# CarluerJB/3D_SIFT_CUDA

Measured on AMD Instinct MI355X. Metric: keypoints/s (.key records per second; Gauss-pyramid GB/s vs HBM roofline in `pyramid`/`roofline`), higher is better.
Workload: dtype f32; 1 GPU; 512^3 float32 blob-field volume per GPU, full featExtract path (pyramid + DoG + extrema + keypoints + SIFT-rank descriptor), all octaves; records_per_volume=185421, octaves=8, extrema=43900, keypoints=36792, parallelism=single GPU, tuning=defaults, descriptor_parity=SIFT-rank: pinned against the reference (see DESIGN.md section 2)

## Files before the change

### 3d_sift_cuda_amd/__init__.py

```python
import ctypes as C
import os
import subprocess

import numpy as np

_HERE = os.path.dirname(os.path.abspath(__file__))
CSRC = os.path.join(_HERE, "csrc")
LIB_HIP = os.path.join(CSRC, "_build", "libsift3d_hip.so")
LIB_HOST = os.path.join(CSRC, "_build", "libsift3d_host.so")
FEATEXTRACT = os.path.join(CSRC, "_build", "featExtract")
FEATRESAMPLE = os.path.join(CSRC, "_build", "featResample")
FEATCOMPOSE = os.path.join(CSRC, "_build", "featCompose")
FEATFUSE = os.path.join(CSRC, "_build", "featFuse")
FEATOVERLAP = os.path.join(CSRC, "_build", "featOverlap")

DESC_SIFT, DESC_BRIEF, DESC_RRIEF, DESC_NRRIEF = 0, 1, 2, 3
ABI_VERSION = 6
INFO_MIN0MAX1, INFO_REORIENT = 0x10, 0x20
STAGES = ("blur_x", "blur_y", "blur_z_dog", "subsample", "extrema", "keypoint", "descriptor", "blur_fused", "octave_tiny")

TUNE_BLUR_FUSED, TUNE_FUSED_CHUNKS, TUNE_FUSED_ROWS, TUNE_LAZY_LEVELS, TUNE_TINY_OCTAVE, TUNE_SAMPLER_CAP, TUNE_KP_CHUNKS, TUNE_BANDS_FIRST, TUNE_HOST_RECORDS, TUNE_FUSED_TILE, TUNE_FUSED_SUB, TUNE_SPLIT_TAIL, TUNE_DESC_SEGMENT, TUNE_FUSED_ORDER, TUNE_FUSED_STAGGER = range(15)

EXTREMUM_DTYPE = np.dtype([("x", "<i4"), ("y", "<i4"), ("z", "<i4"), ("value", "<f4")])
FEATURE_DTYPE = np.dtype([("x", "<f4"), ("y", "<f4"), ("z", "<f4"), ("scale", "<f4"), ("ori", "<f4", (9,)),
                          ("eigs", "<f4", (3,)), ("info", "<u4"), ("desc", "<f4", (64,))])
CANDIDATE_DTYPE = np.dtype([("octave", "<i4"), ("level", "<i4"), ("is_max", "<i4"), ("x", "<i4"), ("y", "<i4"),
                            ("z", "<i4"), ("value", "<f4"), ("h_value", "<f4"), ("l_value", "<f4")])


class Sift3DError(RuntimeError):
    pass


class _Timings(C.Structure):
    _fields_ = [("ms", C.c_double * len(STAGES)), ("launches", C.c_int64 * len(STAGES)), ("alg_bytes", C.c_double * len(STAGES)),
                ("n_octaves", C.c_int64), ("n_extrema", C.c_int64), ("n_keypoints", C.c_int64),
                ("n_records", C.c_int64), ("total_ms", C.c_double)]


class LevelDesc(C.Structure):
    _fields_ = [("img", C.c_void_p), ("dogc", C.c_void_p), ("nx", C.c_int64), ("ny", C.c_int64), ("nz_local", C.c_int64),
                ("nz_global", C.c_int64), ("z_offset", C.c_int64), ("sigma_h", C.c_float), ("sigma_c", C.c_float),
                ("sigma_l", C.c_float), ("octave_factor", C.c_float)]


LAUNCH_DTYPE = np.dtype([("stage", "<i4"), ("ntaps", "<i4"), ("nvox", "<i8"), ("alg_bytes", "<f8"), ("ms", "<f8"),
                         ("start_ms", "<f8")])


def build(verbose=False):
    r = subprocess.run(["make", "-C", CSRC, "-j4"], capture_output=True, text=True)
    if verbose or r.returncode != 0:
        print(r.stdout[-4000:])
        print(r.stderr[-4000:])
    if r.returncode != 0:
        raise Sift3DError("building 3d_sift_cuda_amd/csrc failed")


_hip = None
_host = None


def _sig(fn, res, *args):
    fn.restype = res
    fn.argtypes = list(args)


def hip_lib():
    global _hip
    if _hip is not None:
        return _hip
    if not os.path.exists(LIB_HIP):
        raise Sift3DError("%s is missing: run __graft_entry__.build() (there is no CPU fallback)" % LIB_HIP)
    L = C.CDLL(LIB_HIP)
    P, I64, F, I = C.c_void_p, C.c_int64, C.c_float, C.c_int
    _sig(L.sift3d_abi_version, I)
    if L.sift3d_abi_version() != ABI_VERSION:
        raise Sift3DError("%s has ABI version %d, this mirror of include/sift3d.h is version %d: rebuild (__graft_entry__.build())"
                          % (LIB_HIP, L.sift3d_abi_version(), ABI_VERSION))
    _sig(L.sift3d_device_count, I)
    _sig(L.sift3d_create, P, I, I64, I64, I64)
    _sig(L.sift3d_create_slab, P, I, I64, I64, I64)
    _sig(L.sift3d_set_tuning, I, P, I, I)
    _sig(L.sift3d_host_buffer_grows, I64, P)
    _sig(L.sift3d_zslab_set_tuning, I, P, I, I)
    _sig(L.sift3d_destroy, None, P)
    _sig(L.sift3d_last_error, C.c_char_p, P)
    _sig(L.sift3d_set_stream, I, P, P)
    _sig(L.sift3d_sync, I, P)
    _sig(L.sift3d_free, None, P)
    _sig(L.sift3d_gauss_taps, I, F, F, P)
    _sig(L.sift3d_set_libm_variant, I, I)
    _sig(L.sift3d_get_libm_variant, I)
    _sig(L.sift3d_gauss_blur, I, P, P, P, I64, I64, I64, F, F)
    _sig(L.sift3d_gauss_blur_dev, I, P, P, P, I64, I64, I64, F, F)
    _sig(L.sift3d_gauss_blur_dog_dev, I, P, P, P, P, I64, I64, I64, F, F)
    _sig(L.sift3d_gauss_blur_dog_half_dev, I, P, P, P, P, P, I64, I64, I64, F, F, C.POINTER(C.c_int))
    _sig(L.sift3d_blur_window_supported, I, I64, I64, F, F)
    _sig(L.sift3d_gauss_blur_dog_window_dev, I, P, P, P, P, I64, I64, I64, I64, I64, F, F)
    _sig(L.sift3d_dog, I, P, P, P, P, I64)
    _sig(L.sift3d_dog_dev, I, P, P, P, P, I64)
    _sig(L.sift3d_subsample2, I, P, P, I64, I64, I64, P)
    _sig(L.sift3d_subsample2_dev, I, P, P, I64, I64, I64, P)
    _sig(L.sift3d_extrema, I, P, P, P, P, I64, I64, I64, P, I64, P, P, I64, P)
    _sig(L.sift3d_double_size, I, P, P, I64, I64, I64, P)
    _sig(L.sift3d_halve_size, I, P, P, I64, I64, I64, P)
    _sig(L.sift3d_selftest_lds_add, I, P, P, P, I64, P, P)
    _sig(L.sift3d_set_volume, I, P, P, I64, I64, I64)
    _sig(L.sift3d_set_volume_dev, I, P, P, I64, I64, I64)
    _sig(L.sift3d_set_volume_resized, I, P, P, I64, I64, I64, I)
    _sig(L.sift3d_reserve, I, P, I64)
    _sig(L.sift3d_set_volume_begin, I, P, I64, I64, I64, I)
    _sig(L.sift3d_set_volume_planes, I, P, P, I64, I64)
    _sig(L.sift3d_set_volume_end, I, P)
    _sig(L.sift3d_detect, I, P, F, P, P)
    _sig(L.sift3d_extract, I, P, F, I, F, F, P, P)
    _sig(L.sift3d_extract_view, I, P, F, I, F, F, P, P)
    _sig(L.sift3d_enable_timing, I, P, I)
    _sig(L.sift3d_get_timings, I, P, P)
    _sig(L.sift3d_get_launch_log, I, P, P, I64, P)
    _sig(L.sift3d_candidates_reset, I, P)
    _sig(L.sift3d_extrema_append_dev, I, P, P, P, P, I64, I64, I64, I, I64, I64)
    _sig(L.sift3d_lazy_levels_supported, I, I64, I64, I64, F)
    _sig(L.sift3d_extrema_append_lazy_dev, I, P, P, P, P, P, P, P, F, I64, I64, I64, I, I64, I64)
    _sig(L.sift3d_candidates_dev, I, P, P, I, P, P)
    _sig(L.sift3d_describe_dev, I, P, P, I, I, F, F, P, P, P)
    _sig(L.sift3d_describe_dev_counts, I, P, P, I, I, F, F, P, P)
    _sig(L.sift3d_describe_dev_place, I, P, P, P, P, P, P)
    _sig(L.sift3d_host_register, I, P, I64)
    _sig(L.sift3d_host_unregister, I, P)
    _sig(L.sift3d_set_max_octaves, I, P, I)
    _sig(L.sift3d_extract_zslab, I, P, I, P, I64, I64, I64, F, I, F, F, P, P, P, C.c_char_p, I64)
    _sig(L.sift3d_extract_zslab_over, I, I, P, I, P, I64, I64, I64, F, I, F, F, P, P, P, C.c_char_p, I64)
    _sig(L.sift3d_zslab_set_transport_library, None, C.c_char_p)
    _sig(L.sift3d_zslab_create, P, P, I, I64, I64, I64, C.c_char_p, I64)
    _sig(L.sift3d_zslab_extract, I, P, P, F, I, F, F, P, P, P, C.c_char_p, I64)
    _sig(L.sift3d_zslab_destroy, None, P)
    _sig(L.sift3d_zslab_set_volume, I, P, P, C.c_char_p, I64)
    _sig(L.sift3d_zslab_extract_resident, I, P, F, I, F, F, P, P, P, C.c_char_p, I64)
    _sig(L.sift3d_knn64, I, I, P, I64, P, I64, I, P, P, I, P, C.c_char_p, I64)
    _sig(L.sift3d_match_ratio, I, I, P, I64, P, I64, P, P, P, P, P, C.c_char_p, I64)
    _sig(L.sift3d_hough_similarity, I, I, P, P, P, P, P, P, C.c_int32, P, P, P, P, P, C.c_char_p, I64)
    _sig(L.sift3d_match_keys, I, I, P, I64, P, I64, C.c_int32, P, C.c_char_p, I64)
    _sig(L.sift3d_get_level_slice, I, P, I, I, I64, P, P, P)
    _sig(L.sift3d_get_dog_slice, I, P, I, I, I64, P, P, P)
    _sig(L.sift3d_resample_affine, I, I, P, I64, I64, I64, P, I64, I64, I64, P, I, F, P, C.c_char_p, I64)
    _sig(L.sift3d_resample_affine_dev, I, P, P, I64, I64, I64, P, I64, I64, I64, P, I, F)
    _sig(L.sift3d_guided_search_params, I, I, P, I64, P, I64, P, F, P, P, P, P, P, P, P, C.c_char_p, I64)
    _sig(L.sift3d_refine_similarity, I, I, P, I64, P, I64, P, P, P, P, C.c_char_p, I64)
    _sig(L.sift3d_fit_field, I, I, P, P, I64, P, P, P, C.c_char_p, I64)
    _sig(L.sift3d_refine_field, I, I, P, I64, P, I64, P, P, P, P, C.c_char_p, I64)
    _sig(L.sift3d_resample_field, I, I, P, I64, I64, I64, P, I64, I64, I64, P, P, P, P, I, F, P, C.c_char_p, I64)
    _sig(L.sift3d_block_match, I, I, P, P, I64, I64, I64, P, I64, P, I, I, I, P, P, C.c_char_p, I64)
    _sig(L.sift3d_refine_field_intensity, I, I, P, I64, I64, I64, P, I64, I64, I64, P, P, P, P, P, P, P, C.c_char_p, I64)
    _sig(L.sift3d_block_match_ncc, I, I, P, P, I64, I64, I64, P, I64, P, I, I, I, P, P, C.c_char_p, I64)
    _sig(L.sift3d_refine_field_intensity_metric, I, I, P, I64, I64, I64, P, I64, I64, I64, P, P, P, P, P, I, P, P, P, C.c_char_p, I64)
    _sig(L.sift3d_invert_nodes, I, I, P, P, P, P, P, P, P, P, P, C.c_char_p, I64)
    _sig(L.sift3d_invert_field, I, I, P, P, P, P, P, P, C.c_char_p, I64)
    _sig(L.sift3d_jacobian_map, I, I, I64, I64, I64, P, P, P, P, P, I, P, C.c_char_p, I64)
    _sig(L.sift3d_compose_nodes, I, I, P, P, P, P, P, P, P, P, P, P, P, C.c_char_p, I64)
    _sig(L.sift3d_compose_field, I, I, P, P, P, P, P, P, P, P, C.c_char_p, I64)
    _sig(L.sift3d_fuse_weights, I, I, P, P, I64, I64, I64, C.c_int32, C.c_int32, P, C.c_int32, P, P, C.c_char_p, I64)
    _sig(L.sift3d_fuse_vote, I, I, C.c_int32, P, P, I64, C.c_int32, P, P, C.c_char_p, I64)
    _sig(L.sift3d_fuse_labels, I, I, P, I64, I64, I64, P, C.c_int32, P, P, P, P, C.c_char_p, I64)
    _sig(L.sift3d_fuse_search, I, I, P, P, P, I64, I64, I64, C.c_int32, C.c_int32, C.c_int32, P, C.c_int32, P, P, P, P, C.c_char_p, I64)
    _sig(L.sift3d_fuse_labels_search, I, I, P, I64, I64, I64, P, C.c_int32, P, P, C.c_int32, P, P, P, C.c_char_p, I64)
    _sig(L.sift3d_distance_map, I, I, P, I64, I64, I64, P, P, P, C.c_char_p, I64)
    _sig(L.sift3d_surface_distances, I, P, P, I64, I64, I64, P, P, P, P, P, C.c_char_p, I64)
    _hip = L
    return L


def host_lib():
    global _host
    if _host is not None:
        return _host
    if not os.path.exists(LIB_HOST):
        raise Sift3DError("%s is missing: run __graft_entry__.build()" % LIB_HOST)
    L = C.CDLL(LIB_HOST)
    P, I64, F, I = C.c_void_p, C.c_int64, C.c_float, C.c_int
    _sig(L.sift3d_synth_blobs, None, P, I64, I64, I64, C.c_uint32)
    _sig(L.sift3d_synth_blobs_slices, None, P, I64, I64, I64, C.c_uint32, I64, I64)
    _sig(L.nifti_min_read, I, C.c_char_p, P)
    _sig(L.nifti_min_free, None, P)
    _sig(L.nifti_min_write_f32, I, C.c_char_p, P, I, I, I, F, F, F)
    _sig(L.nifti_min_write_f32_ex, I, C.c_char_p, P, I, I, I, F, F, F, P, P)
    _sig(L.sift3d_write_key, I, C.c_char_p, P, I64, F, I, P)
    _sig(L.sift3d_write_key_mode, None, I)
    _sig(L.sift3d_write_key_bin, I, C.c_char_p, P, I64, F)
    _sig(L.sift3d_read_key, I, C.c_char_p, P, P)
    _sig(L.sift3d_read_key_mode, None, I)
    _sig(L.sift3d_write_pgm, I, C.c_char_p, P, I, I)
    _sig(L.sift3d_world_transform, None, P, I64, P)
    _sig(L.sift3d_match_filter, I64, P, I64, I, I)
    _sig(L.sift3d_match_descriptors, I, P, I64, P)
    _sig(L.sift3d_match_votes, I, P, P, I, P, I, P, P, I, P, P)
    _sig(L.sift3d_match_write_votes, I, C.c_char_p, C.c_char_p, C.c_char_p, P, P, I, I, I)
    _sig(L.sift3d_log_ratio_interval, I, C.c_double, P, P)
    _sig(L.sift3d_similarity_invert, None, P, P)
    _sig(L.sift3d_write_similarity, I, C.c_char_p, P)
    _sig(L.sift3d_write_alignment_matches, I, C.c_char_p, C.c_char_p, C.c_char_p, P, I64, P, I64, P)
    _sig(L.sift3d_similarity_matrix, None, P, P)
    _sig(L.sift3d_read_similarity, I, C.c_char_p, P)
    _sig(L.sift3d_resample_map, I, P, P, P, P)
    _sig(L.sift3d_key_vox2key, None, P, P, P)
    _sig(L.sift3d_fit_similarity, I, P, P, I64, P)
    _sig(L.sift3d_refine_defaults, None, P)
    _sig(L.sift3d_field_defaults, None, P)
    _sig(L.sift3d_field_size, I, P, I64, P, P)
    _sig(L.sift3d_field_samples, None, P, P, P, I64, P, P)
    _sig(L.sift3d_field_warp_terms, I, P, P, P, P)
    _sig(L.sift3d_field_eval, None, P, P, I64, P)
    _sig(L.sift3d_field_folds, I64, P, P, P)
    _sig(L.sift3d_write_field, I, C.c_char_p, P)
    _sig(L.sift3d_read_field, I, C.c_char_p, P)
    _sig(L.sift3d_blockmatch_defaults, None, P)
    _sig(L.sift3d_blockmatch_range, I, P, I64, P, P)
    _sig(L.sift3d_blockmatch_lattice, I, I64, I64, I64, P, P, P)
    _sig(L.sift3d_blockmatch_grid, I, I64, I64, I64, P, P, P)
    _sig(L.sift3d_blockmatch_samples, I64, P, I64, I64, I64, P, P, P, P, P, P, P)
    _sig(L.sift3d_blockmatch_folds, I64, P, P, P)
    _sig(L.sift3d_invert_defaults, None, P)
    _sig(L.sift3d_invert_grid, I, I64, I64, I64, P, P, P)
    _sig(L.sift3d_affine_invert, I, P, P)
    _sig(L.sift3d_affine_invert_d, I, P, P)
    _sig(L.sift3d_write_matrix, I, C.c_char_p, P)
    _sig(L.sift3d_jacobian_factor, I, P, P, P)
    _sig(L.sift3d_compose_defaults, None, P)
    _sig(L.sift3d_compose_matrix, I, P, P, P)
    _sig(L.sift3d_compose_spacing, F, P, P, P)
    _sig(L.sift3d_compose_grid, I, I64, I64, I64, P, P, P, P, P)
    _sig(L.sift3d_compose_residual, I64, P, P, P, I64, P, P)
    _sig(L.sift3d_fuse_defaults, None, P)
    _sig(L.sift3d_fuse_similarity, C.c_uint32, C.c_int32, I64, I64, I64, I64, I64, I64)
    _sig(L.sift3d_fuse_check_labels, I64, P, I64)
    _sig(L.sift3d_fuse_shift_code, C.c_uint16, C.c_int32, C.c_int32, C.c_int32, C.c_int32)
    _sig(L.sift3d_fuse_shift_of, I, C.c_int32, C.c_uint32, P)
    _sig(L.sift3d_fuse_shift_stats, I64, C.c_int32, P, I64, P, P)
    _sig(L.sift3d_label_overlap, I64, P, P, I64, P, P, P)
    _sig(L.sift3d_surface_defaults, None, P)
    _sig(L.sift3d_spacing_um, I, F, P)
    _sig(L.sift3d_surface_stats, None, P, I64, P, I64, P)
    L.free_ptr = C.CDLL(None).free
    L.free_ptr.argtypes = [C.c_void_p]
    _host = L
    return L


class ZSlabStats(C.Structure):
    _fields_ = [("n_ranks", C.c_int32), ("sharded_octaves", C.c_int32), ("exchanges", C.c_int64), ("halo_bytes_critical", C.c_int64),
                ("halo_bytes_deferred", C.c_int64), ("gather_bytes", C.c_int64), ("n_extrema", C.c_int64), ("n_keypoints", C.c_int64),
                ("n_records", C.c_int64), ("wall_ms", C.c_double), ("halo_bytes_hidden", C.c_int64), ("transport", C.c_int32),
                ("transport_fell_back", C.c_int32), ("rccl_version", C.c_int32), ("comm_sets", C.c_int32), ("resident_volume", C.c_int32),
                ("list_grown", C.c_int32), ("merge_ms", C.c_double), ("halo_bytes_subsample", C.c_int64), ("enqueue_ms", C.c_double)]


ZSLAB_TRANSPORT, TRANSPORT_PEER_COPY, TRANSPORT_RCCL = 1000, 0, 1
ZSLAB_SERIAL_CHANNELS, ZSLAB_DUPLICATE_RANKS, ZSLAB_POISON_HALO, ZSLAB_PATCH_WAIT, ZSLAB_LIST_ROOM = 1001, 1002, 1003, 1004, 1005


def zslab_set_transport_library(path):
    hip_lib().sift3d_zslab_set_transport_library(None if path is None else os.fsencode(path))


# ... 1195 lines not shown

def write_key(path, feats, eig_thres=140.0, comments=()):
    feats = np.ascontiguousarray(feats, FEATURE_DTYPE)
    arr = (C.c_char_p * max(1, len(comments)))(*[c.encode() for c in comments])
    rc = host_lib().sift3d_write_key(os.fsencode(path), feats.ctypes.data, len(feats), float(eig_thres), len(comments),
                                     C.cast(arr, C.c_void_p))
    if rc != 0:
        raise Sift3DError("could not write %s" % path)


def write_key_bin(path, feats, eig_thres=140.0):
    feats = np.ascontiguousarray(feats, FEATURE_DTYPE)
    if host_lib().sift3d_write_key_bin(os.fsencode(path), feats.ctypes.data, len(feats), float(eig_thres)) != 0:
        raise Sift3DError("could not write %s" % path)


def world_transform(feats, m44):
    out = np.ascontiguousarray(feats, FEATURE_DTYPE).copy()
    m = np.ascontiguousarray(m44, np.float32).reshape(4, 4)
    host_lib().sift3d_world_transform(out.ctypes.data, len(out), m.ctypes.data)
    return out


def write_pgm(path, slice_yx):
    a = _f32(slice_yx)
    if a.ndim != 2 or host_lib().sift3d_write_pgm(os.fsencode(path), a.ctypes.data, a.shape[0], a.shape[1]) != 0:
        raise Sift3DError("could not write %s" % path)


def read_key(path):
    L = host_lib()
    ptr, n = C.c_void_p(), C.c_int64(0)
    rc = L.sift3d_read_key(os.fsencode(path), C.byref(ptr), C.byref(n))
    if rc != 0:
        raise Sift3DError("could not read %s (%d)" % (path, rc))
    out = np.ctypeslib.as_array(C.cast(ptr, C.POINTER(C.c_uint8)), shape=(n.value * FEATURE_DTYPE.itemsize,)).view(FEATURE_DTYPE).copy()
    L.free_ptr(ptr)
    return out


def _f32(a):
    return np.ascontiguousarray(a, dtype=np.float32)


class Context:

    def __init__(self, nx, ny, nz, device=0, slab=False):
        self._L = hip_lib()
        if self._L.sift3d_device_count() <= 0:
            raise Sift3DError("no HIP device visible and there is no CPU fallback")
        make = self._L.sift3d_create_slab if slab else self._L.sift3d_create
        self._h = make(int(device), int(nx), int(ny), int(nz))
        if not self._h:
            raise Sift3DError("sift3d_create%s(device=%d, %d x %d x %d) failed" % ("_slab" if slab else "", device, nx, ny, nz))
        self.device = device
        self._shape = None

    def set_tuning(self, knob, value):
        self._chk(self._L.sift3d_set_tuning(self._h, int(knob), int(value)), "sift3d_set_tuning")

    def host_buffer_grows(self):
        return int(self._L.sift3d_host_buffer_grows(self._h))

    def close(self):
        if getattr(self, "_h", None):
            self._L.sift3d_destroy(self._h)
            self._h = None

    def __enter__(self):
        return self

    def __exit__(self, *a):
        self.close()

    def __del__(self):
        try:
            self.close()
        except Exception:
            pass

    @property
    def handle(self):
        return self._h

    def _chk(self, rc, what):
        if rc != 0:
            raise Sift3DError("%s -> %d: %s" % (what, rc, self._L.sift3d_last_error(self._h).decode()))

    def gauss_blur(self, vol, sigma, min_value=0.01):
        vol = _f32(vol)
        nz, ny, nx = vol.shape
        out = np.empty_like(vol)
        self._chk(self._L.sift3d_gauss_blur(self._h, vol.ctypes.data, out.ctypes.data, nx, ny, nz, float(sigma),
                                            float(min_value)), "sift3d_gauss_blur")
        return out

    def dog(self, a, b):
        a, b = _f32(a), _f32(b)
        out = np.empty_like(a)
        self._chk(self._L.sift3d_dog(self._h, a.ctypes.data, b.ctypes.data, out.ctypes.data, a.size), "sift3d_dog")
        return out

    def subsample2(self, vol):
        vol = _f32(vol)
        nz, ny, nx = vol.shape
        out = np.empty((nz // 2, ny // 2, nx // 2), np.float32)
        self._chk(self._L.sift3d_subsample2(self._h, vol.ctypes.data, nx, ny, nz, out.ctypes.data), "sift3d_subsample2")
        return out

    def double_size(self, vol):
        vol = _f32(vol)
        nz, ny, nx = vol.shape
        out = np.empty((2 * nz, 2 * ny, 2 * nx), np.float32)
        self._chk(self._L.sift3d_double_size(self._h, vol.ctypes.data, nx, ny, nz, out.ctypes.data), "sift3d_double_size")
        return out

    def halve_size(self, vol):
        vol = _f32(vol)
        nz, ny, nx = vol.shape
        out = np.empty((nz // 2, ny // 2, nx // 2), np.float32)
        self._chk(self._L.sift3d_halve_size(self._h, vol.ctypes.data, nx, ny, nz, out.ctypes.data), "sift3d_halve_size")
        return out

    def selftest_lds_add(self, a, b):
        a, b = _f32(a).ravel(), _f32(b).ravel()
        valu, lds = np.empty_like(a), np.empty_like(a)
        self._chk(self._L.sift3d_selftest_lds_add(self._h, a.ctypes.data, b.ctypes.data, a.size, valu.ctypes.data,
                                                  lds.ctypes.data), "sift3d_selftest_lds_add")
        return valu, lds

    def extrema(self, d_prev, d_cur, d_next=None, capacity=None):
        d_prev, d_cur = _f32(d_prev), _f32(d_cur)
        nz, ny, nx = d_cur.shape
        d_next = None if d_next is None else _f32(d_next)
        cap = int(capacity) if capacity is not None else d_cur.size // 8 + 1024
        mins = np.zeros(cap, EXTREMUM_DTYPE)
        maxs = np.zeros(cap, EXTREMUM_DTYPE)
        nmin, nmax = C.c_int64(0), C.c_int64(0)
        rc = self._L.sift3d_extrema(self._h, d_prev.ctypes.data, d_cur.ctypes.data,
                                    None if d_next is None else d_next.ctypes.data, nx, ny, nz, mins.ctypes.data, cap,
                                    C.byref(nmin), maxs.ctypes.data, cap, C.byref(nmax))
        self._chk(rc, "sift3d_extrema")
        return mins[:nmin.value].copy(), maxs[:nmax.value].copy()

    def set_volume(self, vol, resize=0):
        vol = _f32(vol)
        nz, ny, nx = vol.shape
        self._chk(self._L.sift3d_set_volume_resized(self._h, vol.ctypes.data, nx, ny, nz, int(resize)), "sift3d_set_volume_resized")
        self._shape = self._resized((nz, ny, nx), resize)

    def reserve(self, n_extrema):
        self._chk(self._L.sift3d_reserve(self._h, int(n_extrema)), "sift3d_reserve")

    def set_volume_in_runs(self, vol, runs, resize=0):
        vol = _f32(vol)
        nz, ny, nx = vol.shape
        self._chk(self._L.sift3d_set_volume_begin(self._h, nx, ny, nz, int(resize)), "sift3d_set_volume_begin")
        for z0, n in runs:
            part = vol[z0:z0 + n]
            self._chk(self._L.sift3d_set_volume_planes(self._h, part.ctypes.data, int(z0), int(n)), "sift3d_set_volume_planes")
        self._chk(self._L.sift3d_set_volume_end(self._h), "sift3d_set_volume_end")
        self._shape = self._resized((nz, ny, nx), resize)

    def set_volume_dev(self, dev_ptr, nx, ny, nz):
        self._chk(self._L.sift3d_set_volume_dev(self._h, C.c_void_p(int(dev_ptr)), nx, ny, nz), "sift3d_set_volume_dev")
        self._shape = (int(nz), int(ny), int(nx))

    @staticmethod
    def _resized(shape, resize):
        return tuple(2 * d if resize > 0 else d // 2 if resize < 0 else d for d in shape)

    def _slice(self, entry, octave, level, z, shape_yx):
        out = np.empty(shape_yx, np.float32)
        nx, ny = C.c_int64(0), C.c_int64(0)
        self._chk(getattr(self._L, entry)(self._h, int(octave), int(level), int(z), out.ctypes.data, C.byref(nx), C.byref(ny)), entry)
        assert (ny.value, nx.value) == tuple(shape_yx), (entry, octave, (ny.value, nx.value), shape_yx)
        return out

    def level_slice(self, octave, level, z, shape_yx):
        return self._slice("sift3d_get_level_slice", octave, level, z, shape_yx)

    def dog_slice(self, octave, level, z, shape_yx):
        return self._slice("sift3d_get_dog_slice", octave, level, z, shape_yx)

    def pyramid(self):
        out = []
        shape = self._shape
        for o in range(int(self.timings()["n_octaves"])):
            assert min(shape) > 2, (o, shape)
            lv = {"L": [], "D": []}
            for j in range(5):
                lv["L"].append(np.stack([self.level_slice(o, j, z, shape[1:]) for z in range(shape[0])]))
                try:
                    lv["D"].append(np.stack([self.dog_slice(o, j, z, shape[1:]) for z in range(shape[0])]))
                except Sift3DError as e:
                    if "not stored" not in str(e):
                        raise
                    lv["D"].append(None)
            out.append(lv)
            shape = tuple(d // 2 for d in shape)
        return out

    def detect(self, initial_image_scale=1.0):
        out, n = C.c_void_p(), C.c_int64(0)
        self._chk(self._L.sift3d_detect(self._h, float(initial_image_scale), C.byref(out), C.byref(n)), "sift3d_detect")
        try:
            buf = (C.c_char * (n.value * CANDIDATE_DTYPE.itemsize)).from_address(out.value) if n.value else b""
            return np.frombuffer(buf, CANDIDATE_DTYPE, n.value).copy()
        finally:
            self._L.sift3d_free(out)

    def extract(self, initial_image_scale=1.0, desc_mode=DESC_SIFT, eig_thres=140.0, size_factor=1.0, copy=True):
        out, n = C.c_void_p(), C.c_int64(0)
        self._chk(self._L.sift3d_extract_view(self._h, float(initial_image_scale), int(desc_mode), float(eig_thres),
                                              float(size_factor), C.byref(out), C.byref(n)), "sift3d_extract_view")
        if n.value == 0:
            return np.zeros(0, FEATURE_DTYPE)
        buf = (C.c_char * (n.value * FEATURE_DTYPE.itemsize)).from_address(out.value)
        a = np.frombuffer(buf, FEATURE_DTYPE, n.value)
        return a.copy() if copy else a

    def gauss_blur_dog_dev(self, d_in, d_out, d_dog, nx, ny, nz, sigma, min_value=0.01):
        self._chk(self._L.sift3d_gauss_blur_dog_dev(self._h, C.c_void_p(int(d_in)), C.c_void_p(int(d_out)) if d_out else None,
                                                    C.c_void_p(int(d_dog)) if d_dog else None, nx, ny, nz, float(sigma),
                                                    float(min_value)), "sift3d_gauss_blur_dog_dev")

    def gauss_blur_dog_half_dev(self, d_in, d_out, d_dog, d_half, nx, ny, nz, sigma, min_value=0.01):
        one = C.c_int(0)
        self._chk(self._L.sift3d_gauss_blur_dog_half_dev(self._h, C.c_void_p(int(d_in)), C.c_void_p(int(d_out)),
                                                         C.c_void_p(int(d_dog)) if d_dog else None, C.c_void_p(int(d_half)), nx, ny, nz,
                                                         float(sigma), float(min_value), C.byref(one)), "sift3d_gauss_blur_dog_half_dev")
        return bool(one.value)

    def gauss_blur_dev(self, d_in, d_out, nx, ny, nz, sigma, min_value=0.01):
        self._chk(self._L.sift3d_gauss_blur_dev(self._h, C.c_void_p(int(d_in)), C.c_void_p(int(d_out)), nx, ny, nz,
                                                float(sigma), float(min_value)), "sift3d_gauss_blur_dev")

    def blur_window_supported(self, nx, ny, sigma, min_value=0.01):
        return bool(self._L.sift3d_blur_window_supported(nx, ny, float(sigma), float(min_value)))

    def gauss_blur_dog_window_dev(self, d_in, d_out, d_dog, nx, ny, nz, z_lo, z_hi, sigma, min_value=0.01):
        self._chk(self._L.sift3d_gauss_blur_dog_window_dev(self._h, C.c_void_p(int(d_in)), C.c_void_p(int(d_out)) if d_out else None,
                                                           C.c_void_p(int(d_dog)) if d_dog else None, nx, ny, nz, int(z_lo), int(z_hi),
                                                           float(sigma), float(min_value)), "sift3d_gauss_blur_dog_window_dev")

    def dog_dev(self, d_a, d_b, d_out, n):
        self._chk(self._L.sift3d_dog_dev(self._h, C.c_void_p(int(d_a)), C.c_void_p(int(d_b)), C.c_void_p(int(d_out)), n),
                  "sift3d_dog_dev")

    def resample_affine_dev(self, d_src, src_shape, d_dst, out_shape, map, interp="linear", fill=0.0):
        nz, ny, nx = (int(d) for d in src_shape)
        oz, oy, ox = (int(d) for d in out_shape)
        m = _map12(map)
        self._chk(self._L.sift3d_resample_affine_dev(self._h, C.c_void_p(int(d_src)), nx, ny, nz, C.c_void_p(int(d_dst)), ox, oy, oz,
                                                     m.ctypes.data, INTERP[interp], float(fill)), "sift3d_resample_affine_dev")

    def subsample2_dev(self, d_in, nx, ny, nz, d_out):
        self._chk(self._L.sift3d_subsample2_dev(self._h, C.c_void_p(int(d_in)), nx, ny, nz, C.c_void_p(int(d_out))),
                  "sift3d_subsample2_dev")

    def candidates_reset(self):
        self._chk(self._L.sift3d_candidates_reset(self._h), "sift3d_candidates_reset")

    def extrema_append_dev(self, d_prev, d_cur, d_next, nx, ny, nz_local, level_id, z_lo, z_hi):
        self._chk(self._L.sift3d_extrema_append_dev(self._h, C.c_void_p(int(d_prev)), C.c_void_p(int(d_cur)),
                                                    C.c_void_p(int(d_next)), nx, ny, nz_local, int(level_id), int(z_lo),
                                                    int(z_hi)), "sift3d_extrema_append_dev")

    def lazy_levels_supported(self, nx, ny, nz_local, next_sigma):
        return bool(self._L.sift3d_lazy_levels_supported(nx, ny, nz_local, float(next_sigma)))

    def extrema_append_lazy_dev(self, d_prev, g_prev_a, g_prev_b, d_cur, d_next, g_next, next_sigma, nx, ny, nz_local, level_id,
                                z_lo, z_hi):
        vp = lambda v: C.c_void_p(int(v)) if v else None
        self._chk(self._L.sift3d_extrema_append_lazy_dev(self._h, vp(d_prev), vp(g_prev_a), vp(g_prev_b), vp(d_cur), vp(d_next),
                                                         vp(g_next), float(next_sigma), nx, ny, nz_local, int(level_id), int(z_lo),
                                                         int(z_hi)), "sift3d_extrema_append_lazy_dev")

    @staticmethod
    def _level_array(levels):
        arr = (LevelDesc * len(levels))()
        for i, lv in enumerate(levels):
            arr[i] = LevelDesc(int(lv["img"]), int(lv["dogc"]), lv["nx"], lv["ny"], lv["nz_local"], lv["nz_global"],
                               lv["z_offset"], lv["sigma_h"], lv["sigma_c"], lv["sigma_l"], lv["octave_factor"])
        return arr

    def candidates_dev(self, levels):
        arr = self._level_array(levels)
        out, n = C.c_void_p(), C.c_int64(0)
        self._chk(self._L.sift3d_candidates_dev(self._h, arr, len(levels), C.byref(out), C.byref(n)), "sift3d_candidates_dev")
        try:
            buf = (C.c_char * (n.value * CANDIDATE_DTYPE.itemsize)).from_address(out.value) if n.value else b""
            return np.frombuffer(buf, CANDIDATE_DTYPE, n.value).copy()
        finally:
            self._L.sift3d_free(out)

    def describe_dev(self, levels, desc_mode=DESC_SIFT, eig_thres=140.0, size_factor=1.0, copy=True):
        arr = self._level_array(levels)
        view, grp, n = C.c_void_p(), C.c_void_p(), C.c_int64(0)
        self._chk(self._L.sift3d_describe_dev(self._h, arr, len(levels), int(desc_mode), float(eig_thres), float(size_factor),
                                              C.byref(view), C.byref(grp), C.byref(n)), "sift3d_describe_dev")
        if n.value == 0:
            return np.zeros(0, FEATURE_DTYPE), np.zeros(0, np.int32)
        rb = (C.c_char * (n.value * FEATURE_DTYPE.itemsize)).from_address(view.value)
        gb = (C.c_char * (n.value * 4)).from_address(grp.value)
        recs, grp = np.frombuffer(rb, FEATURE_DTYPE, n.value), np.frombuffer(gb, np.int32, n.value)
# ... 51 lines not shown
```

### 3d_sift_cuda_amd/csrc/api_context.hip

```cpp
#include <algorithm>
#include <chrono>
#include <cmath>
#include <cstdarg>
#include <cstdio>
#include <cstdlib>
#include <cstring>
#include <vector>

#include "sift3d_internal.h"

#include "pipeline.h"

int set_err(sift3d_ctx *c, int code, const char *fmt, ...)
{
    if (c) {
        va_list ap;
        va_start(ap, fmt);
        vsnprintf(c->err, sizeof(c->err), fmt, ap);
        va_end(ap);
    }
    return code;
}

extern "C" int sift3d_abi_version(void) { return SIFT3D_ABI_VERSION; }

extern "C" int sift3d_device_count(void)
{
    int n = 0;
    if (hipGetDeviceCount(&n) != hipSuccess) return 0;
    return n;
}

extern "C" void sift3d_free(void *p) { free(p); }

extern "C" const char *sift3d_last_error(const sift3d_ctx *ctx) { return ctx ? ctx->err : "no context"; }

static void free_dev(sift3d_ctx *c)
{
    hipFree(c->vol);
    for (int i = 0; i < 6; i++) hipFree(c->L[i]);
    for (int i = 0; i < 5; i++) hipFree(c->D[i]);
    hipFree(c->D4tiny);
    hipFree(c->T[0]);
    hipFree(c->T[1]);
    hipFree(c->d_taps);
    hipFree(c->keys_a);
    hipFree(c->keys_b);
    hipFree(c->vals_a);
    hipFree(c->vals_b);
    hipFree(c->d_count);
    hipFree(c->surv);
    hipFree(c->surv2);
    hipFree(c->list2[0]);
    hipFree(c->list2[1]);
    hipFree(c->list2_counts);
    hipFree(c->surv_counts);
    hipFree(c->sort_tmp);
    hipFree(c->scan_tmp);
    hipFree(c->d_levels);
    hipFree(c->kps);
    hipFree(c->patch0);
    hipFree(c->sampler_tokens);
    hipFree(c->d_rec_base);
    hipFree(c->nrec);
    hipFree(c->offs);
    hipFree(c->rec_kp);
    hipFree(c->rec_frame);
    if (c->h_recs) hipHostFree(c->h_recs);
    if (c->h_group) hipHostFree(c->h_group);
    hipFree(c->place.d_counts);
    hipFree(c->place.d_shift);
    if (c->place.h_counts) hipHostFree(c->place.h_counts);
}


std::vector<octave_dims> octave_list(int64_t X, int64_t Y, int64_t Z)
{
    std::vector<octave_dims> v;
    int64_t off = 0;
    while (X > 2 && Y > 2 && Z > 2 && v.size() < 32) {
        const int64_t XP = pitch_of(X);
        v.push_back({X, Y, Z, off, XP});
        off += ((XP * Y * Z + 63) / 64) * 64;
        X /= 2; Y /= 2; Z /= 2;
    }
    return v;
}

int alloc_cands(sift3d_ctx *c, int64_t cap)
{
    unsigned long long *ka = nullptr, *kb = nullptr;
    sift3d_cval *va = nullptr, *vb = nullptr;
    void *tmp = nullptr;
    const size_t tmp_bytes = sift3d_sort_temp_bytes(cap) + 256;
    const bool ok = hipMalloc((void **)&ka, sizeof(unsigned long long) * (size_t)cap) == hipSuccess &&
                    hipMalloc((void **)&kb, sizeof(unsigned long long) * (size_t)cap) == hipSuccess &&
                    hipMalloc((void **)&va, sizeof(sift3d_cval) * (size_t)cap) == hipSuccess &&
                    hipMalloc((void **)&vb, sizeof(sift3d_cval) * (size_t)cap) == hipSuccess && hipMalloc(&tmp, tmp_bytes) == hipSuccess;
    if (!ok) {
        (void)hipGetLastError();
        hipFree(ka); hipFree(kb); hipFree(va); hipFree(vb); hipFree(tmp);
        return SIFT3D_ERR_MEMORY;
    }
    hipFree(c->keys_a); hipFree(c->keys_b); hipFree(c->vals_a); hipFree(c->vals_b); hipFree(c->sort_tmp);
    c->keys_a = ka; c->keys_b = kb;
    c->vals_a = va; c->vals_b = vb;
    c->sort_tmp = tmp;
    c->sort_tmp_bytes = tmp_bytes;
    c->cand_cap = cap;
    return SIFT3D_OK;
}

static void destroy_sync_objects(sift3d_ctx *c)
{
    hipStream_t streams[] = {c->ex_stream, c->ex_stream2, c->kp_stream};
    for (hipStream_t st : streams)
        if (st) {
            hipStreamSynchronize(st);
            hipStreamDestroy(st);
        }
    hipEvent_t events[] = {c->ev_ex2[0], c->ev_ex2[1], c->ev_reset, c->ev_desc, c->ev_oct[0], c->ev_oct[1], c->ev_fence[0], c->ev_fence[1],
                           c->ev_split[0], c->ev_split[1], c->ev_split[2]};
    for (hipEvent_t e : events)
        if (e) hipEventDestroy(e);
    for (hipEvent_t e : c->ev_kpc)
        if (e) hipEventDestroy(e);
    if (c->h_cnt0) hipHostFree(c->h_cnt0);
    if (c->own_stream && c->stream) hipStreamDestroy(c->stream);
}

sift3d_ctx *ctx_create(int device, int64_t nx, int64_t ny, int64_t nz, bool lean)
{
    if (nx <= 0 || ny <= 0 || nz <= 0) return nullptr;
    int n = sift3d_device_count();
    if (device < 0 || device >= n) return nullptr;
    if (hipSetDevice(device) != hipSuccess) return nullptr;
    sift3d_ctx *c = new sift3d_ctx();
    c->device = device;
    c->own_stream = true;
    c->lean = lean;
    c->capN = pitch_of(nx) * ny * nz;
    c->surv_div = 64;
    c->tune[SIFT3D_TUNE_BLUR_FUSED] = 1;
    c->tune[SIFT3D_TUNE_LAZY_LEVELS] = 1;
    c->tune[SIFT3D_TUNE_TINY_OCTAVE] = 1;
    c->tune[SIFT3D_TUNE_SAMPLER_CAP] = 4;
    c->tune[SIFT3D_TUNE_BANDS_FIRST] = 1;
    c->tune[SIFT3D_TUNE_HOST_RECORDS] = 5;
    c->tune[SIFT3D_TUNE_FUSED_SUB] = 1;
    c->tune[SIFT3D_TUNE_SPLIT_TAIL] = 1;
    c->tune[SIFT3D_TUNE_DESC_SEGMENT] = 32;
    c->capTot = c->capN + c->capN / 7 + 4 * ny * nz + 64 * 34;
    bool ok = hipStreamCreateWithFlags(&c->stream, hipStreamNonBlocking) == hipSuccess;
    hipStream_t *streams[] = {&c->ex_stream, &c->ex_stream2, &c->kp_stream};
    for (hipStream_t *st : streams) ok = ok && hipStreamCreateWithFlags(st, hipStreamNonBlocking) == hipSuccess;
    hipEvent_t *events[] = {&c->ev_ex2[0], &c->ev_ex2[1], &c->ev_reset, &c->ev_desc, &c->ev_oct[0], &c->ev_oct[1], &c->ev_fence[0], &c->ev_fence[1],
                            &c->ev_split[0], &c->ev_split[1], &c->ev_split[2]};
    for (hipEvent_t *e : events) ok = ok && hipEventCreateWithFlags(e, hipEventDisableTiming) == hipSuccess;
    for (hipEvent_t &e : c->ev_kpc) ok = ok && hipEventCreateWithFlags(&e, hipEventDisableTiming) == hipSuccess;
    ok = ok && hipHostMalloc((void **)&c->h_cnt0, sizeof(unsigned long long) * (16 + SIFT3D_KP_MAX_CHUNKS), hipHostMallocDefault) == hipSuccess;
    const size_t vb = sizeof(float) * (size_t)c->capN;
    const size_t tb = sizeof(float) * (size_t)c->capTot;
    if (!lean) {
        ok = ok && hipMalloc((void **)&c->vol, vb) == hipSuccess && hipMemsetAsync(c->vol, 0, vb, c->stream) == hipSuccess;
        for (int i = 0; i < 5 && ok; i++) ok = hipMalloc((void **)&c->L[i], tb) == hipSuccess && hipMemsetAsync(c->L[i], 0, tb, c->stream) == hipSuccess;
        for (int i = 0; i < 4 && ok; i++) ok = hipMalloc((void **)&c->D[i], tb) == hipSuccess && hipMemsetAsync(c->D[i], 0, tb, c->stream) == hipSuccess;
        ok = ok && hipMalloc((void **)&c->D4tiny, sizeof(float) * SIFT3D_D4TINY_FLOATS) == hipSuccess &&
             hipMemsetAsync(c->D4tiny, 0, sizeof(float) * SIFT3D_D4TINY_FLOATS, c->stream) == hipSuccess;
    }
    if (c->capN <= SIFT3D_EAGER_T_FLOATS)
        for (int i = 0; i < 2 && ok; i++) {
            ok = hipMalloc((void **)&c->T[i], vb) == hipSuccess;
            if (ok) c->capT = c->capN;
        }
    ok = ok && hipMalloc((void **)&c->d_taps, sizeof(float) * SIFT3D_MAX_TAPS) == hipSuccess;
    ok = ok && hipMalloc((void **)&c->d_count, sizeof(unsigned long long) * 8) == hipSuccess;
    ok = ok && hipMalloc((void **)&c->d_levels, sizeof(sift3d_level) * 96) == hipSuccess;
    ok = ok && hipMalloc((void **)&c->sampler_tokens, sizeof(int) * SIFT3D_CU_SLOTS) == hipSuccess &&
         hipMemsetAsync(c->sampler_tokens, 0, sizeof(int) * SIFT3D_CU_SLOTS, c->stream) == hipSuccess;
    ok = ok && hipMalloc((void **)&c->d_rec_base, sizeof(int) * (SIFT3D_KP_MAX_CHUNKS + 1)) == hipSuccess;
    ok = ok && alloc_cands(c, c->capN / 32 + 8192) == SIFT3D_OK;
    c->surv_cap = c->capN / 8 + 65536;
    ok = ok && hipMalloc((void **)&c->surv, sizeof(sift3d_survivor) * (size_t)c->surv_cap) == hipSuccess;
    ok = ok && hipMalloc((void **)&c->surv_counts, sizeof(unsigned long long) * SIFT3D_SURV_COUNTERS * SIFT3D_SURV_SETS) == hipSuccess;
    ok = ok && hipMalloc((void **)&c->list2_counts, sizeof(unsigned long long) * SIFT3D_LIST2_COUNTERS * SIFT3D_SURV_SETS) == hipSuccess;
    ok = ok && hipStreamSynchronize(c->stream) == hipSuccess;
    if (!ok) {
        free_dev(c);
        destroy_sync_objects(c);
        delete c;
        return nullptr;
    }
    return c;
}

extern "C" sift3d_ctx *sift3d_create(int device, int64_t nx, int64_t ny, int64_t nz) { return ctx_create(device, nx, ny, nz, false); }

extern "C" sift3d_ctx *sift3d_create_slab(int device, int64_t nx, int64_t ny, int64_t nz_local) { return ctx_create(device, nx, ny, nz_local, true); }

extern "C" void sift3d_destroy(sift3d_ctx *c)
{
    if (!c) return;
    hipSetDevice(c->device);
    hipStreamSynchronize(c->stream);
    free_dev(c);
    for (hipEvent_t e : c->pool) hipEventDestroy(e);
    destroy_sync_objects(c);
    delete c;
}

extern "C" int sift3d_set_tuning(sift3d_ctx *c, int knob, int value)
{
    if (!c) return SIFT3D_ERR_ARG;
    static const int lo[SIFT3D_TUNE_COUNT] = {0, 0, 0, 0, 0, 0, 0, 0, 1, 0, 0, 0, 0, 0, 0},
                     hi[SIFT3D_TUNE_COUNT] = {2, 4096, 2, 1, 1, 64, SIFT3D_KP_MAX_CHUNKS, 1, 1 + SIFT3D_MAX_FRAMES, 2, 1, 2, 1 << 20, 3, 2};
    if (knob < 0 || knob >= SIFT3D_TUNE_COUNT || value < lo[knob] || value > hi[knob])
        return set_err(c, SIFT3D_ERR_ARG, "sift3d_set_tuning: knob %d does not take %d", knob, value);
    c->tune[knob] = value;
    return SIFT3D_OK;
}

extern "C" int64_t sift3d_host_buffer_grows(const sift3d_ctx *c) { return c ? c->host_grows : 0; }

#ifdef SIFT3D_DEV
extern "C" int sift3d_dev_set_stop(sift3d_ctx *c, int n)
{
    if (!c) return SIFT3D_ERR_ARG;
    c->dev_stop = n;
    return SIFT3D_OK;
}
#endif

extern "C" int sift3d_set_stream(sift3d_ctx *c, void *s)
{
    if (!c) return SIFT3D_ERR_ARG;
    HIPCHK(c, hipSetDevice(c->device));
    HIPCHK(c, hipStreamSynchronize(c->stream));
    if (s) {
        if (c->own_stream) hipStreamDestroy(c->stream);
        c->stream = (hipStream_t)s;
        c->own_stream = false;
    } else if (!c->own_stream) {
        HIPCHK(c, hipStreamCreateWithFlags(&c->stream, hipStreamNonBlocking));
        c->own_stream = true;
    }
    return SIFT3D_OK;
}

extern "C" int sift3d_set_max_octaves(sift3d_ctx *c, int n)
{
    if (!c || n < 0) return c ? set_err(c, SIFT3D_ERR_ARG, "max_octaves must be >= 0") : SIFT3D_ERR_ARG;
    c->max_octaves = n;
    return SIFT3D_OK;
}

extern "C" int sift3d_sync(sift3d_ctx *c)
{
    if (!c) return SIFT3D_ERR_ARG;
    HIPCHK(c, hipSetDevice(c->device));
    HIPCHK(c, hipStreamSynchronize(c->stream));
    return SIFT3D_OK;
}

__global__ void selftest_lds_add_kernel(const float *__restrict__ a, const float *__restrict__ b, long long n,
                                        float *__restrict__ valu, float *__restrict__ lds)
{
    __shared__ float cell[256];
    const long long i = (long long)blockIdx.x * 256 + threadIdx.x;
    const float x = i < n ? a[i] : 0.0f, y = i < n ? b[i] : 0.0f;
    cell[threadIdx.x] = x;
    __syncthreads();
    __hip_atomic_fetch_add(&cell[threadIdx.x], y, __ATOMIC_RELAXED, __HIP_MEMORY_SCOPE_WORKGROUP);
    __syncthreads();
    if (i < n) {
        valu[i] = x + y;
        lds[i] = cell[threadIdx.x];
    }
}

extern "C" int sift3d_selftest_lds_add(sift3d_ctx *c, const float *a, const float *b, int64_t n, float *valu, float *lds)
{
    NEED_LEVELS(c);
    if (!c || !a || !b || !valu || !lds || n <= 0 || 4 * n > c->capTot) return c ? set_err(c, SIFT3D_ERR_ARG, "bad self-test arguments") : SIFT3D_ERR_ARG;
    HIPCHK(c, hipSetDevice(c->device));
    float *da = c->L[0], *db = c->L[0] + n, *dv = c->L[0] + 2 * n, *dl = c->L[0] + 3 * n;
    HIPCHK(c, hipMemcpyAsync(da, a, sizeof(float) * (size_t)n, hipMemcpyHostToDevice, c->stream));
    HIPCHK(c, hipMemcpyAsync(db, b, sizeof(float) * (size_t)n, hipMemcpyHostToDevice, c->stream));
    hipLaunchKernelGGL(selftest_lds_add_kernel, dim3((unsigned)((n + 255) / 256)), dim3(256), 0, c->stream, da, db, (long long)n, dv, dl);
    HIPCHK(c, hipGetLastError());
    HIPCHK(c, hipMemcpyAsync(valu, dv, sizeof(float) * (size_t)n, hipMemcpyDeviceToHost, c->stream));
    HIPCHK(c, hipMemcpyAsync(lds, dl, sizeof(float) * (size_t)n, hipMemcpyDeviceToHost, c->stream));
    HIPCHK(c, hipStreamSynchronize(c->stream));
    c->has_volume = false;
    c->pad_nx = 0;
    return SIFT3D_OK;
}

int ensure_T(sift3d_ctx *c, int64_t floats)
{
    if (floats <= c->capT) return SIFT3D_OK;
    if (floats > c->capN) return set_err(c, SIFT3D_ERR_ARG, "pass intermediates of %lld floats asked of a context of %lld", (long long)floats, (long long)c->capN);
    HIPCHK(c, hipStreamSynchronize(c->stream));
    hipFree(c->T[0]);
    hipFree(c->T[1]);
    c->T[0] = c->T[1] = nullptr;
    c->capT = 0;
    int64_t want = c->capN / 8 + c->capN / 64 + 4096;
    if (want < floats) want = floats;
    if (want > c->capN) want = c->capN;
    for (int i = 0; i < 2; i++)
        if (hipMalloc((void **)&c->T[i], sizeof(float) * (size_t)want) != hipSuccess) {
            (void)hipGetLastError();
            return set_err(c, SIFT3D_ERR_MEMORY, "out of device memory for the pass intermediates (%lld floats)", (long long)want);
        }
    c->capT = want;
    return SIFT3D_OK;
}
```

### 3d_sift_cuda_amd/csrc/api_ops.hip

```cpp
#include <algorithm>
#include <chrono>
#include <cmath>
#include <cstdarg>
#include <cstdio>
#include <cstdlib>
#include <cstring>
#include <vector>

#include "sift3d_internal.h"

#include "pipeline.h"

static sift3d_blur_tuning blur_tuning(const sift3d_ctx *c)
{
    return {c->tune[SIFT3D_TUNE_FUSED_CHUNKS], c->tune[SIFT3D_TUNE_FUSED_ROWS], c->tune[SIFT3D_TUNE_FUSED_TILE], c->tune[SIFT3D_TUNE_FUSED_ORDER], c->tune[SIFT3D_TUNE_FUSED_STAGGER]};
}

int blur_dev(sift3d_ctx *c, const float *in, float *out, float *dog, int64_t X, int64_t Y, int64_t Z, float sigma,
                    float min_value, float *sub, bool *sub_done)
{
    if (sub_done) *sub_done = false;
    float taps[SIFT3D_MAX_TAPS];
    hipStream_t ws = c->stream;
    int n = sift3d_gauss_taps(sigma, min_value, taps);
// ... 240 lines not shown

extern "C" int sift3d_halve_size(sift3d_ctx *c, const float *in, int64_t nx, int64_t ny, int64_t nz, float *out)
{
    NEED_LEVELS(c);
    int rc = check_shape(c, nx, ny, nz);
    if (rc) return rc;
    if (!in || !out || nx < 2 || ny < 2 || nz < 2) return set_err(c, SIFT3D_ERR_ARG, "halve_size needs every dimension >= 2");
    HIPCHK(c, hipSetDevice(c->device));
    HIPCHK(c, hipMemcpyAsync(c->L[0], in, sizeof(float) * (size_t)(nx * ny * nz), hipMemcpyHostToDevice, c->stream));
    HIPCHK(c, sift3d_launch_halve_size(c->stream, c->L[0], nx, ny, nz, c->L[1]));
    const size_t ob = sizeof(float) * (size_t)((nx / 2) * (ny / 2) * (nz / 2));
    HIPCHK(c, hipMemcpyAsync(out, c->L[1], ob, hipMemcpyDeviceToHost, c->stream));
    HIPCHK(c, hipStreamSynchronize(c->stream));
    c->has_volume = false;
    c->pad_nx = 0;
    return SIFT3D_OK;
}

int cand_reset(sift3d_ctx *c, hipStream_t on)
{
    if (!on) on = c->stream;
    c->jobs.clear();
    c->cand_split_at = 0;
    HIPCHK(c, hipMemsetAsync(c->d_count, 0, sizeof(unsigned long long) * 8, on));
    HIPCHK(c, hipMemsetAsync(c->surv_counts, 0, sizeof(unsigned long long) * SIFT3D_SURV_COUNTERS * SIFT3D_SURV_SETS, on));
    HIPCHK(c, hipMemsetAsync(c->list2_counts, 0, sizeof(unsigned long long) * SIFT3D_LIST2_COUNTERS * SIFT3D_SURV_SETS, on));
    HIPCHK(c, hipMemsetAsync(c->d_rec_base, 0, sizeof(int), on));
    c->surv_set = 0;
    return SIFT3D_OK;
}

int cand_append(sift3d_ctx *c, const level_job &j, const cand_where &w, bool record)
{
    c->count_queued = false;
    if (record) c->jobs.push_back(j);
    hipStream_t st = w.stream ? w.stream : c->stream;
    stage_scope sc(c, SIFT3D_STAGE_EXTREMA, 4.0 * (double)j.X * j.Y * j.Z, 0, j.X * j.Y * j.Z, st);
    int64_t cover = j.X * j.Y * j.Z / c->surv_div + 64 * 1024;
    if (cover > c->surv_cap) cover = c->surv_cap;
    sift3d_survivor *surv = c->surv;
    if (w.list > 0) {
        if (c->surv2_cap < cover) {
            HIPCHK(c, hipStreamSynchronize(st));
            hipFree(c->surv2);
            c->surv2 = nullptr;
            c->surv2_cap = 0;
            HIPCHK(c, hipMalloc((void **)&c->surv2, sizeof(sift3d_survivor) * (size_t)cover));
            c->surv2_cap = cover;
        }
        surv = c->surv2;
    }
    const bool fresh = c->surv_set < SIFT3D_SURV_SETS;
    const int set = fresh ? c->surv_set++ : SIFT3D_SURV_SETS - 1;
    unsigned long long *counters = c->surv_counts + (size_t)set * SIFT3D_SURV_COUNTERS;
    sift3d_extrema_lazy lz;
    memset(&lz, 0, sizeof(lz));
    const bool lazy = j.prev_b || j.next_g;
    if (lazy) {
        lz.prev_b = j.prev_b;
        lz.next_g = j.next_g;
        if (j.next_g) {
            const int li = w.list > 0 ? 1 : 0;
            if (c->list2_cap[li] < cover) {
                HIPCHK(c, hipStreamSynchronize(st));
                hipFree(c->list2[li]);
                c->list2[li] = nullptr;
                c->list2_cap[li] = 0;
                HIPCHK(c, hipMalloc((void **)&c->list2[li], sizeof(sift3d_survivor2) * (size_t)cover));
                c->list2_cap[li] = cover;
            }
            lz.ntaps = j.next_ntaps;
            memcpy(lz.taps, j.next_taps, sizeof(lz.taps));
            lz.list2 = c->list2[li];
            lz.list2_count = c->list2_counts + (size_t)set * SIFT3D_LIST2_COUNTERS;
            lz.list2_cap = c->list2_cap[li];
            if (!fresh) HIPCHK(c, hipMemsetAsync(lz.list2_count, 0, sizeof(unsigned long long) * SIFT3D_LIST2_COUNTERS, st));
        }
    }
    HIPCHK(c, sift3d_launch_extrema(st, {j.dp, j.dc, j.dn, j.X, j.Xl ? j.Xl : j.X, j.Y, j.Z, j.z_lo, j.z_hi, j.lvl_id, cand_target_of(c, w.group),
                                         surv, counters, c->d_count + 2, cover, !fresh, lazy ? &lz : nullptr, c->strict_extrema}));
    return SIFT3D_OK;
}

int cand_append_octave_small(sift3d_ctx *c, const level_job jobs[3], const float *const D[5], int64_t XP, int64_t X, int64_t Y, int64_t Z,
                             const cand_where &w)
{
    hipStream_t st = w.stream ? w.stream : c->stream;
    stage_scope sc(c, SIFT3D_STAGE_EXTREMA, 12.0 * (double)XP * Y * Z, 0, XP * Y * Z, st);
    HIPCHK(c, sift3d_launch_extrema_octave_small(st, D, XP, X, Y, Z, jobs[0].lvl_id, cand_target_of(c, w.group)));
    c->count_queued = false;
    for (int l = 0; l < 3; l++) c->jobs.push_back(jobs[l]);
    return SIFT3D_OK;
}

int cand_replay(sift3d_ctx *c)
{
    c->cand_split_at = 0;
    HIPCHK(c, hipMemsetAsync(c->d_count, 0, sizeof(unsigned long long) * 8, c->stream));
    HIPCHK(c, hipMemsetAsync(c->surv_counts, 0, sizeof(unsigned long long) * SIFT3D_SURV_COUNTERS * SIFT3D_SURV_SETS, c->stream));
    HIPCHK(c, hipMemsetAsync(c->list2_counts, 0, sizeof(unsigned long long) * SIFT3D_LIST2_COUNTERS * SIFT3D_SURV_SETS, c->stream));
    c->surv_set = 0;
    for (const level_job &j : c->jobs) {
        int rc = cand_append(c, j, cand_where(), false);
        if (rc) return rc;
    }
    return SIFT3D_OK;
}

int surv_make_room(sift3d_ctx *c, unsigned long long high_water)
{
    c->surv_div = 1;
    if ((int64_t)high_water > c->surv_cap) {
        hipFree(c->surv);
        c->surv = nullptr;
        c->surv_cap = (int64_t)high_water + (int64_t)high_water / 4 + 4096;
        HIPCHK(c, hipMalloc((void **)&c->surv, sizeof(sift3d_survivor) * (size_t)c->surv_cap));
    }
    return SIFT3D_OK;
}

int cand_count_queue(sift3d_ctx *c)
{
    unsigned long long *cnt = c->h_cnt0 + 4;
    cnt[0] = cnt[1] = cnt[2] = 0;
    HIPCHK(c, hipMemcpyAsync(cnt, c->d_count, sizeof(unsigned long long) * 3, hipMemcpyDeviceToHost, c->stream));
    c->count_queued = true;
    return SIFT3D_OK;
}

int cand_finalize(sift3d_ctx *c, int64_t *count_out)
{
    for (int attempt = 0; attempt < 4; attempt++) {
        const unsigned long long *cnt = c->h_cnt0 + 4;
        if (!c->count_queued) {
            int rc = cand_count_queue(c);
            if (rc) return rc;
        }
        c->count_queued = false;
        HIPCHK(c, hipStreamSynchronize(c->stream));
        if (cnt[2] > 0) {
            int rc = surv_make_room(c, cnt[2]);
            if (rc) return rc;
            rc = cand_replay(c);
            if (rc) return rc;
            continue;
        }
        if ((int64_t)cnt[0] > c->cand_cap) {
            if (alloc_cands(c, (int64_t)cnt[0] + (int64_t)cnt[0] / 4 + 4096) != SIFT3D_OK)
                return set_err(c, SIFT3D_ERR_MEMORY, "candidate buffer could not be grown to %llu entries", cnt[0]);
            int rc = cand_replay(c);
            if (rc) return rc;
            continue;
        }
        if (cnt[0] > 0)
            HIPCHK(c, sift3d_sort_candidates(c->stream, c->sort_tmp, c->sort_tmp_bytes, c->keys_a, c->keys_b, c->vals_a, c->vals_b, (int64_t)cnt[0]));
        *count_out = (int64_t)cnt[0];
        return SIFT3D_OK;
    }
    return set_err(c, SIFT3D_ERR_MEMORY, "extrema buffers could not be grown");
}

extern "C" int sift3d_extrema(sift3d_ctx *c, const float *d_prev, const float *d_cur, const float *d_next, int64_t nx,
                              int64_t ny, int64_t nz, sift3d_extremum *minima, int64_t cap_min, int64_t *n_min,
                              sift3d_extremum *maxima, int64_t cap_max, int64_t *n_max)
{
    NEED_LEVELS(c);
    int rc = check_shape(c, nx, ny, nz);
    if (rc) return rc;
    if (!d_prev || !d_cur || !n_min || !n_max) return set_err(c, SIFT3D_ERR_ARG, "null pointer");
    HIPCHK(c, hipSetDevice(c->device));
    const size_t b = sizeof(float) * (size_t)(nx * ny * nz);
    HIPCHK(c, hipMemcpyAsync(c->D[0], d_prev, b, hipMemcpyHostToDevice, c->stream));
    HIPCHK(c, hipMemcpyAsync(c->D[1], d_cur, b, hipMemcpyHostToDevice, c->stream));
    if (d_next) HIPCHK(c, hipMemcpyAsync(c->D[2], d_next, b, hipMemcpyHostToDevice, c->stream));
    c->has_volume = false;
    c->pad_nx = 0;
    c->strict_extrema = sift3d_volume_needs_strict(d_cur, nx * ny * nz);
    int64_t cnt = 0;
    rc = cand_reset(c);
    if (!rc) rc = cand_append(c, {c->D[0], c->D[1], d_next ? c->D[2] : nullptr, nx, ny, nz, 0, (int)nz, 0}, cand_where(), true);
    if (!rc) rc = cand_finalize(c, &cnt);
    if (rc) return rc;
    std::vector<unsigned long long> keys((size_t)cnt);
    std::vector<sift3d_cval> vals((size_t)cnt);
    if (cnt) {
        HIPCHK(c, hipMemcpyAsync(keys.data(), c->keys_b, sizeof(unsigned long long) * (size_t)cnt, hipMemcpyDeviceToHost, c->stream));
        HIPCHK(c, hipMemcpyAsync(vals.data(), c->vals_b, sizeof(sift3d_cval) * (size_t)cnt, hipMemcpyDeviceToHost, c->stream));
    }
    HIPCHK(c, hipStreamSynchronize(c->stream));
    int64_t a = 0, m = 0;
    bool over = false;
    for (int64_t i = 0; i < cnt; i++) {
        const int64_t idx = (int64_t)(keys[(size_t)i] & SIFT3D_KEY_IDX_MASK);
        sift3d_extremum e;
        e.x = (int32_t)(idx % nx);
        e.y = (int32_t)((idx / nx) % ny);
        e.z = (int32_t)(idx / (nx * ny));
        e.value = vals[(size_t)i].value;
        if ((keys[(size_t)i] >> SIFT3D_KEY_MAX_SHIFT) & 1ull) {
            if (m < cap_max && maxima) maxima[m] = e; else over = true;
            m++;
        } else {
            if (a < cap_min && minima) minima[a] = e; else over = true;
            a++;
        }
    }
    *n_min = a;
    *n_max = m;
    return over ? set_err(c, SIFT3D_ERR_CAPACITY, "extrema lists need %lld + %lld entries", (long long)a, (long long)m)
                : SIFT3D_OK;
}
```

### 3d_sift_cuda_amd/csrc/api_pipeline.hip

```cpp
#include <algorithm>
#include <chrono>
#include <cmath>
#include <cstdarg>
#include <cstdio>
#include <cstdlib>
#include <cstring>
#include <vector>

#include "sift3d_internal.h"

#include "pipeline.h"

static int ensure_level_buffer(sift3d_ctx *c, float **buf)
{
    if (*buf) return SIFT3D_OK;
    if (hipMalloc((void **)buf, sizeof(float) * (size_t)c->capTot) != hipSuccess) {
        *buf = nullptr;
        return set_err(c, SIFT3D_ERR_MEMORY, "a level buffer of %lld floats could not be allocated", (long long)c->capTot);
    }
    HIPCHK(c, hipMemsetAsync(*buf, 0, sizeof(float) * (size_t)c->capTot, c->stream));
    return SIFT3D_OK;
}

static int load_volume_prepare(sift3d_ctx *c, int64_t nx, int64_t ny, int64_t nz)
// ... 57 lines not shown
    return SIFT3D_OK;
}

extern "C" int sift3d_set_volume_dev(sift3d_ctx *c, const float *d_vol, int64_t nx, int64_t ny, int64_t nz)
{
    NEED_LEVELS(c);
    int rc = check_shape(c, nx, ny, nz);
    if (rc) return rc;
    if (!d_vol) return set_err(c, SIFT3D_ERR_ARG, "null volume");
    if (nz <= 1) return set_err(c, SIFT3D_ERR_ARG, "Could not read volume (z <= 1)");
    HIPCHK(c, hipSetDevice(c->device));
    rc = fence_in(c);
    if (rc) return rc;
    rc = load_volume(c, d_vol, false, nx, ny, nz);
    if (rc) return rc;
    rc = scan_volume(c, nx, ny, nz);
    if (rc) return rc;
    c->nx = nx; c->ny = ny; c->nz = nz;
    c->has_volume = true;
    return fence_out(c);
}

extern "C" int sift3d_set_volume_resized(sift3d_ctx *c, const float *vol, int64_t nx, int64_t ny, int64_t nz, int resize)
{
    NEED_LEVELS(c);
    if (resize == 0) return sift3d_set_volume(c, vol, nx, ny, nz);
    if (!c || !vol || nx < 2 || ny < 2 || nz < 2 || nx * ny * nz > c->capN)
        return set_err(c, SIFT3D_ERR_ARG, "set_volume_resized: bad shape or null volume");
    const int64_t ox = resize > 0 ? 2 * nx : nx / 2, oy = resize > 0 ? 2 * ny : ny / 2, oz = resize > 0 ? 2 * nz : nz / 2;
    int rc = check_shape(c, ox, oy, oz);
    if (rc) return rc;
    if (oz <= 1) return set_err(c, SIFT3D_ERR_ARG, "Could not read volume (z <= 1)");
    HIPCHK(c, hipSetDevice(c->device));
    rc = ensure_T(c, ox * oy * oz > nx * ny * nz ? ox * oy * oz : nx * ny * nz);
    if (rc) return rc;
    HIPCHK(c, hipMemcpyAsync(c->T[0], vol, sizeof(float) * (size_t)(nx * ny * nz), hipMemcpyHostToDevice, c->stream));
    if (resize > 0) HIPCHK(c, sift3d_launch_double_size(c->stream, c->T[0], nx, ny, nz, c->T[1]));
    else HIPCHK(c, sift3d_launch_halve_size(c->stream, c->T[0], nx, ny, nz, c->T[1]));
    rc = load_volume(c, c->T[1], false, ox, oy, oz);
    if (rc) return rc;
    rc = scan_volume(c, ox, oy, oz);
    if (rc) return rc;
    c->nx = ox; c->ny = oy; c->nz = oz;
    c->has_volume = true;
    return SIFT3D_OK;
}

extern "C" int sift3d_set_volume_begin(sift3d_ctx *c, int64_t nx, int64_t ny, int64_t nz, int resize)
{
    NEED_LEVELS(c);
    if (!c || nx < 1 || ny < 1 || nz < 1 || nx * ny * nz > c->capN) return set_err(c, SIFT3D_ERR_ARG, "set_volume_begin: bad shape");
    if (resize != 0 && (nx < 2 || ny < 2 || nz < 2)) return set_err(c, SIFT3D_ERR_ARG, "set_volume_begin: bad shape for a resize");
    const int64_t ox = resize > 0 ? 2 * nx : (resize < 0 ? nx / 2 : nx), oy = resize > 0 ? 2 * ny : (resize < 0 ? ny / 2 : ny),
                  oz = resize > 0 ? 2 * nz : (resize < 0 ? nz / 2 : nz);
    int rc = check_shape(c, ox, oy, oz);
    if (rc) return rc;
    if (oz <= 1) return set_err(c, SIFT3D_ERR_ARG, "Could not read volume (z <= 1)");
    HIPCHK(c, hipSetDevice(c->device));
    c->has_volume = false;
    if (resize != 0) {
        rc = ensure_T(c, ox * oy * oz > nx * ny * nz ? ox * oy * oz : nx * ny * nz);
        if (rc) return rc;
    } else {
        rc = load_volume_prepare(c, nx, ny, nz);
        if (rc) return rc;
    }
    c->up.open = true;
    c->up.nx = nx; c->up.ny = ny; c->up.nz = nz;
    c->up.got = 0;
    c->up.resize = resize;
    c->up.seen.assign((size_t)nz, false);
    return SIFT3D_OK;
}

extern "C" int sift3d_set_volume_planes(sift3d_ctx *c, const float *planes, int64_t z0, int64_t n)
{
    if (!c || !c->up.open) return set_err(c, SIFT3D_ERR_ARG, "set_volume_planes without set_volume_begin");
    if (!planes || z0 < 0 || n < 1 || z0 + n > c->up.nz) {
        c->up.open = false;
        return set_err(c, SIFT3D_ERR_ARG, "set_volume_planes: planes [%lld, %lld) of %lld", (long long)z0, (long long)(z0 + n), (long long)c->up.nz);
    }
    for (int64_t z = z0; z < z0 + n; z++)
        if (c->up.seen[(size_t)z]) {
            c->up.open = false;
            return set_err(c, SIFT3D_ERR_ARG, "set_volume_planes: plane %lld arrived twice", (long long)z);
        }
    for (int64_t z = z0; z < z0 + n; z++) c->up.seen[(size_t)z] = true;
    HIPCHK(c, hipSetDevice(c->device));
    const int64_t nx = c->up.nx, ny = c->up.ny, xp = pitch_of(nx);
    if (c->up.resize != 0) {
        HIPCHK(c, hipMemcpyAsync(c->T[0] + z0 * nx * ny, planes, sizeof(float) * (size_t)(n * nx * ny), hipMemcpyHostToDevice, c->stream));
    } else if (xp == nx) {
        HIPCHK(c, hipMemcpyAsync(c->vol + z0 * nx * ny, planes, sizeof(float) * (size_t)(n * nx * ny), hipMemcpyHostToDevice, c->stream));
    } else {
        HIPCHK(c, hipMemcpy2DAsync(c->vol + z0 * xp * ny, sizeof(float) * (size_t)xp, planes, sizeof(float) * (size_t)nx, sizeof(float) * (size_t)nx,
                                   (size_t)(ny * n), hipMemcpyHostToDevice, c->stream));
    }
    c->up.got += n;
    return SIFT3D_OK;
}

extern "C" int sift3d_set_volume_end(sift3d_ctx *c)
{
    if (!c || !c->up.open) return set_err(c, SIFT3D_ERR_ARG, "set_volume_end without set_volume_begin");
    c->up.open = false;
    if (c->up.got != c->up.nz) return set_err(c, SIFT3D_ERR_ARG, "set_volume_end: %lld of %lld planes arrived", (long long)c->up.got, (long long)c->up.nz);
    HIPCHK(c, hipSetDevice(c->device));
    int64_t nx = c->up.nx, ny = c->up.ny, nz = c->up.nz;
    if (c->up.resize != 0) {
        const int64_t ox = c->up.resize > 0 ? 2 * nx : nx / 2, oy = c->up.resize > 0 ? 2 * ny : ny / 2, oz = c->up.resize > 0 ? 2 * nz : nz / 2;
        if (c->up.resize > 0) HIPCHK(c, sift3d_launch_double_size(c->stream, c->T[0], nx, ny, nz, c->T[1]));
        else HIPCHK(c, sift3d_launch_halve_size(c->stream, c->T[0], nx, ny, nz, c->T[1]));
        const int rc = load_volume(c, c->T[1], false, ox, oy, oz);
        if (rc) return rc;
        nx = ox; ny = oy; nz = oz;
    }
    const int rs = scan_volume(c, nx, ny, nz);
    if (rs) return rs;
    c->nx = nx; c->ny = ny; c->nz = nz;
    c->has_volume = true;
    return SIFT3D_OK;
}

static int ensure_host_records(sift3d_ctx *c, int64_t need, int64_t keep)
{
    if (need <= c->hrecs_cap) return SIFT3D_OK;
    sift3d_feature *nr = nullptr;
    int *ng = nullptr;
    const int64_t cap = need + need / 8 + 1024;
    HIPCHK(c, hipHostMalloc((void **)&nr, sizeof(sift3d_feature) * (size_t)cap, hipHostMallocDefault));
    if (hipHostMalloc((void **)&ng, sizeof(int) * (size_t)cap, hipHostMallocDefault) != hipSuccess) {
        hipHostFree(nr);
        return set_err(c, SIFT3D_ERR_MEMORY, "out of pinned host memory for %lld records", (long long)cap);
    }
    if (keep > 0 && c->h_recs) {
        memcpy(nr, c->h_recs, sizeof(sift3d_feature) * (size_t)keep);
        memcpy(ng, c->h_group, sizeof(int) * (size_t)keep);
    }
    if (c->h_recs) hipHostFree(c->h_recs);
    if (c->h_group) hipHostFree(c->h_group);
    c->h_recs = nr;
    c->h_group = ng;
    c->hrecs_cap = cap;
    HIPCHK(c, hipHostGetDevicePointer((void **)&c->d_hrecs, c->h_recs, 0));
    HIPCHK(c, hipHostGetDevicePointer((void **)&c->d_hgroup, c->h_group, 0));
    return SIFT3D_OK;
}

static int ensure_kp_buffers(sift3d_ctx *c, int64_t ncand, int64_t host_for = -1)
{
    if (ncand > c->kps_cap) {
        HIPCHK(c, hipStreamSynchronize(c->stream));
        HIPCHK(c, hipStreamSynchronize(c->kp_stream));
        hipFree(c->kps); hipFree(c->nrec); hipFree(c->offs); hipFree(c->scan_tmp); hipFree(c->patch0);
        hipFree(c->rec_kp); hipFree(c->rec_frame);
        c->kps = nullptr;
        c->patch0 = nullptr;
        c->nrec = c->offs = c->rec_kp = c->rec_frame = nullptr;
        c->scan_tmp = nullptr;
        c->kps_cap = 0;
        const int64_t cap = ncand + ncand / 2 + 1024, rcap = cap * (1 + SIFT3D_MAX_FRAMES);
        c->scan_tmp_bytes = sift3d_scan_temp_bytes(cap) + 256;
        HIPCHK(c, hipMalloc((void **)&c->kps, sizeof(sift3d_dkp) * (size_t)cap));
        HIPCHK(c, hipMalloc((void **)&c->patch0, sizeof(float) * SIFT3D_PATCH_VOX * (size_t)cap));
        HIPCHK(c, hipMalloc((void **)&c->nrec, sizeof(int) * (size_t)cap));
        HIPCHK(c, hipMalloc((void **)&c->offs, sizeof(int) * (size_t)cap));
        HIPCHK(c, hipMalloc(&c->scan_tmp, c->scan_tmp_bytes));
        HIPCHK(c, hipMalloc((void **)&c->rec_kp, sizeof(int) * (size_t)rcap));
        HIPCHK(c, hipMalloc((void **)&c->rec_frame, sizeof(int) * (size_t)rcap));
        c->kps_cap = cap;
        c->recs_cap = rcap;
    }
    int per = c->tune[SIFT3D_TUNE_HOST_RECORDS];
    if (per < 1) per = 1;
    if (per > 1 + SIFT3D_MAX_FRAMES) per = 1 + SIFT3D_MAX_FRAMES;
    if (host_for < 0 || host_for > ncand) host_for = ncand;
    if (c->hrecs_cap < host_for * per) {
        HIPCHK(c, hipStreamSynchronize(c->stream));
        HIPCHK(c, hipStreamSynchronize(c->kp_stream));
        int rc = ensure_host_records(c, host_for * per, 0);
        if (rc) return rc;
    }
    return SIFT3D_OK;
}

extern "C" int sift3d_reserve(sift3d_ctx *c, int64_t n_extrema)
{
    if (!c || n_extrema < 0) return set_err(c, SIFT3D_ERR_ARG, "sift3d_reserve: bad arguments");
    HIPCHK(c, hipSetDevice(c->device));
    if (n_extrema > c->cand_cap && alloc_cands(c, n_extrema + n_extrema / 4 + 4096) != SIFT3D_OK)
        return set_err(c, SIFT3D_ERR_MEMORY, "candidate buffer could not be grown to %lld entries", (long long)n_extrema);
    return ensure_kp_buffers(c, n_extrema, n_extrema);
}

int candidates_to_host(sift3d_ctx *c, const std::vector<sift3d_level> &levels, int64_t ncand,
                              sift3d_candidate **cands_out, int64_t *n_out)
{
    std::vector<unsigned long long> keys((size_t)ncand);
    std::vector<sift3d_cval> vals((size_t)ncand);
    if (ncand) {
        HIPCHK(c, hipMemcpyAsync(keys.data(), c->keys_b, sizeof(unsigned long long) * (size_t)ncand, hipMemcpyDeviceToHost, c->stream));
        HIPCHK(c, hipMemcpyAsync(vals.data(), c->vals_b, sizeof(sift3d_cval) * (size_t)ncand, hipMemcpyDeviceToHost, c->stream));
    }
    timing_end(c);
    HIPCHK(c, hipStreamSynchronize(c->stream));
    sift3d_candidate *out = (sift3d_candidate *)malloc(sizeof(sift3d_candidate) * (size_t)(ncand ? ncand : 1));
    if (!out) return set_err(c, SIFT3D_ERR_MEMORY, "out of host memory");
    for (int64_t i = 0; i < ncand; i++) {
        const unsigned long long k = keys[(size_t)i];
        const int id = (int)(k >> SIFT3D_KEY_LVL_SHIFT);
        const int64_t idx = (int64_t)(k & SIFT3D_KEY_IDX_MASK);
        if (id < 0 || id >= (int)levels.size()) {
            free(out);
            return set_err(c, SIFT3D_ERR_ARG, "candidate with level id %d outside the level table", id);
        }
        const sift3d_level &lv = levels[(size_t)id];
        sift3d_candidate &o = out[i];
        o.octave = id / 3;
        o.level = id % 3 + 1;
        o.is_max = (int)((k >> SIFT3D_KEY_MAX_SHIFT) & 1ull);
        o.x = (int32_t)(idx % lv.XP);
        o.y = (int32_t)((idx / lv.XP) % lv.Y);
        o.z = (int32_t)(idx / ((int64_t)lv.XP * lv.Y)) + lv.z_off;
        o.value = vals[(size_t)i].value;
        o.h_value = vals[(size_t)i].h;
        o.l_value = vals[(size_t)i].l;
    }
    *cands_out = out;
    *n_out = ncand;
    return SIFT3D_OK;
}

static void kp_params_of(sift3d_ctx *c, int desc_mode, float eig_thres, float size_factor, sift3d_kp_params &p)
{
    p.levels = c->d_levels;
    p.eig_thres = eig_thres;
    p.size_factor = size_factor;
    p.desc_mode = desc_mode;
    p.debug_stop = c->dev_stop;
    p.patch0 = c->patch0;
    p.sampler_tokens = c->sampler_tokens;
    p.sampler_cap = c->tune[SIFT3D_TUNE_SAMPLER_CAP];
    p.desc_seg = c->tune[SIFT3D_TUNE_DESC_SEGMENT] * 8;
    p.rec_shift = nullptr;
}

static int kp_chunks_for(const sift3d_ctx *c, int64_t ncand)
{
    int n = c->tune[SIFT3D_TUNE_KP_CHUNKS];
    if (n <= 0) n = SIFT3D_KP_DEFAULT_CHUNKS;
    if (n > SIFT3D_KP_MAX_CHUNKS) n = SIFT3D_KP_MAX_CHUNKS;
    if (n > ncand) n = ncand > 0 ? (int)ncand : 1;
    return n;
}

static int describe_begin(sift3d_ctx *c, size_t nlevels, float *taps3)
{
    if (sift3d_gauss_taps(0.5f, 0.01f, taps3) != 3 || sift3d_gauss_taps((float)0.95, (float)0.01, c->kp.taps5) != 5)
        return set_err(c, SIFT3D_ERR_ARG, "unexpected patch tap counts");
    if (nlevels > 96) return set_err(c, SIFT3D_ERR_ARG, "too many levels");
    c->kp.ncand = 0;
    c->kp.nchunks = 0;
    c->kp.launched = 0;
    c->kp.nrec = 0;
    c->kp.split = false;
    c->place.dst = nullptr;
    return SIFT3D_OK;
}

void describe_want_group_counts(sift3d_ctx *c, bool on) { c->place.counts = on; }

static int ensure_place_buffers(sift3d_ctx *c)
{
    if (c->place.d_counts) return SIFT3D_OK;
    HIPCHK(c, hipMalloc((void **)&c->place.d_counts, sizeof(int) * SIFT3D_GROUPS));
    HIPCHK(c, hipMalloc((void **)&c->place.d_shift, sizeof(int) * SIFT3D_GROUPS));
    HIPCHK(c, hipHostMalloc((void **)&c->place.h_counts, sizeof(int) * SIFT3D_GROUPS, hipHostMallocDefault));
    return SIFT3D_OK;
}

int describe_group_counts(sift3d_ctx *c, const int **counts, int64_t *total)
{
    if (!c->place.counts) return set_err(c, SIFT3D_ERR_ARG, "describe_group_counts: not asked for before describe_queue");
    {
        const int rc = ensure_place_buffers(c);
        if (rc) return rc;
    }
    *total = 0;
    if (c->kp.ncand <= 0 || c->kp.nchunks != 1) {
        memset(c->place.h_counts, 0, sizeof(int) * SIFT3D_GROUPS);
        *counts = c->place.h_counts;
        return c->kp.nchunks > 1 ? set_err(c, SIFT3D_ERR_ARG, "describe_group_counts: the stage runs in chunks") : SIFT3D_OK;
    }
    HIPCHK(c, hipEventSynchronize(c->ev_kpc[0]));
    for (int g = 0; g < SIFT3D_GROUPS; g++) *total += c->place.h_counts[g];
    *counts = c->place.h_counts;
    return SIFT3D_OK;
}

int describe_placement(sift3d_ctx *c, sift3d_feature *shared_list, const int *shift)
{
    if (!shared_list || !shift || !c->place.d_shift) return set_err(c, SIFT3D_ERR_ARG, "describe_placement: bad arguments");
    HIPCHK(c, hipMemcpyAsync(c->place.d_shift, shift, sizeof(int) * SIFT3D_GROUPS, hipMemcpyHostToDevice, c->stream));
    c->place.dst = shared_list;
    return SIFT3D_OK;
}

static int describe_queue_chunk(sift3d_ctx *c, int i, int64_t a, int64_t b, hipStream_t ks, const float *taps3)
{
    int *h_end = reinterpret_cast<int *>(c->h_cnt0 + 8);
    c->kp.first[i] = a;
    c->kp.first[i + 1] = b;
    h_end[i] = 0;
    {
        sift3d_kp_params q = c->kp.p;
        q.patch0 = c->patch0 + (size_t)a * SIFT3D_PATCH_VOX;
        stage_scope sc(c, SIFT3D_STAGE_KEYPOINT, 0.0, 0, b - a, ks);
        HIPCHK(c, sift3d_launch_keypointsA(ks, q, c->keys_b + a, c->vals_b + a, b - a, c->kps + a, c->nrec + a, taps3));
    }
    HIPCHK(c, sift3d_scan_counts(ks, c->scan_tmp, c->scan_tmp_bytes, c->nrec + a, c->offs + a, b - a));
    HIPCHK(c, sift3d_launch_recmap(ks, c->nrec + a, c->offs + a, b - a, (int)a, c->d_rec_base + i, c->rec_kp, c->rec_frame, c->d_count + 3));
    HIPCHK(c, hipMemcpyAsync(&h_end[i], c->d_rec_base + i + 1, sizeof(int), hipMemcpyDeviceToHost, ks));
    if (c->place.counts && i == 0) {
        int rc = ensure_place_buffers(c);
        if (rc) return rc;
        HIPCHK(c, hipMemsetAsync(c->place.d_counts, 0, sizeof(int) * SIFT3D_GROUPS, ks));
        HIPCHK(c, sift3d_launch_group_counts(ks, c->keys_b + a, c->nrec + a, b - a, c->place.d_counts));
        HIPCHK(c, hipMemcpyAsync(c->place.h_counts, c->place.d_counts, sizeof(int) * SIFT3D_GROUPS, hipMemcpyDeviceToHost, ks));
    }
    HIPCHK(c, hipEventRecord(c->ev_kpc[i], ks));
    return SIFT3D_OK;
}

int describe_queue(sift3d_ctx *c, const std::vector<sift3d_level> &levels, int64_t ncand, int desc_mode, float eig_thres,
                          float size_factor, bool levels_on_device)
{
    float taps3[SIFT3D_MAX_TAPS];
    int rc0 = describe_begin(c, levels.size(), taps3);
    if (rc0) return rc0;
    c->kp.ncand = ncand;
    if (ncand <= 0) return SIFT3D_OK;
    int rc = ensure_kp_buffers(c, ncand);
    if (rc) return rc;
    if (!levels_on_device)
        HIPCHK(c, hipMemcpyAsync(c->d_levels, levels.data(), sizeof(sift3d_level) * levels.size(), hipMemcpyHostToDevice, c->stream));
    kp_params_of(c, desc_mode, eig_thres, size_factor, c->kp.p);
    const int nch = kp_chunks_for(c, ncand);
    c->kp.nchunks = nch;
    HIPCHK(c, hipMemsetAsync(c->d_count + 3, 0, sizeof(unsigned long long), c->stream));
    HIPCHK(c, hipMemsetAsync(c->d_rec_base, 0, sizeof(int), c->stream));
    for (int i = 0; i < nch; i++) {
        rc = describe_queue_chunk(c, i, ncand * i / nch, ncand * (i + 1) / nch, c->stream, taps3);
        if (rc) return rc;
    }
    return SIFT3D_OK;
}

int describe_launch(sift3d_ctx *c)
{
    const int nch = c->kp.nchunks;
    if (nch <= 0) return SIFT3D_OK;
    const int *h_end = reinterpret_cast<const int *>(c->h_cnt0 + 8);
    const bool split = c->kp.split && nch > 1;
    const bool beside = split || (!c->kp.split && nch > 1 && !(c->timing == 1 || c->timing == 3));
    int64_t base = 0;
    for (int i = 0; i < nch; i++) {
        hipStream_t ds = (split ? i > 0 : beside) ? c->kp_stream : c->stream;
        HIPCHK(c, hipEventSynchronize(c->ev_kpc[i]));
        const int64_t end = h_end[i], m = end - base;
        if (end < base || end > c->recs_cap) return set_err(c, SIFT3D_ERR_DEVICE, "record map out of range (%lld of %lld)", (long long)end, (long long)c->recs_cap);
        if (end > c->hrecs_cap && !c->place.dst) {
            HIPCHK(c, hipStreamSynchronize(ds));
            if (split) HIPCHK(c, hipStreamSynchronize(c->stream));
            const int64_t done_cand = c->kp.first[i + 1], need = done_cand > 0 && i + 1 < nch ? (int64_t)((double)end * (double)c->kp.ncand / (double)done_cand) + 1 : end;
            int rc = ensure_host_records(c, need > end ? need : end, base);
            if (rc) return rc;
            c->host_grows++;
        }
        if (m > 0) {
            stage_scope sc(c, SIFT3D_STAGE_DESCRIPTOR, 0.0, 0, m, ds);
            if (c->kp.p.sampler_cap > 0 && !(split && i > 0))
                HIPCHK(c, hipMemsetAsync(c->sampler_tokens, 0, sizeof(int) * SIFT3D_CU_SLOTS, ds));
            sift3d_kp_params q = c->kp.p;
            q.rec_shift = c->place.dst ? c->place.d_shift : nullptr;
            if (c->place.dst && end > c->hrecs_cap) {
                HIPCHK(c, hipStreamSynchronize(ds));
                int rc = ensure_host_records(c, end, 0);
                if (rc) return rc;
                c->host_grows++;
            }
            HIPCHK(c, sift3d_launch_descriptors(ds, q, c->kps, c->rec_kp + base, c->rec_frame + base, m,
                                                (c->place.dst ? c->place.dst : c->d_hrecs) + base, c->d_hgroup + base, c->kp.taps5));
        }
        base = end;
    }
    c->kp.nrec = base;
    c->kp.launched = 1;
    if (beside) {
        HIPCHK(c, hipEventRecord(c->ev_desc, c->kp_stream));
        HIPCHK(c, hipStreamWaitEvent(c->stream, c->ev_desc, 0));
    }
    return SIFT3D_OK;
}

int describe_finish(sift3d_ctx *c, int64_t *n_out)
{
    unsigned long long &nkp = c->h_cnt0[6];
    nkp = 0;
    if (c->kp.nrec) HIPCHK(c, hipMemcpyAsync(&nkp, c->d_count + 3, sizeof(nkp), hipMemcpyDeviceToHost, c->stream));
    HIPCHK(c, hipStreamSynchronize(c->stream));
    timing_end(c);
    c->last.n_records = c->kp.nrec;
    c->last.n_keypoints = (int64_t)nkp;
    *n_out = c->kp.nrec;
    return SIFT3D_OK;
}

#ifdef SIFT3D_DEV
extern "C" int sift3d_dev_overlap_probe(sift3d_ctx *c, int kslice, int dslice, double *out_ms)
{
    if (!c || !out_ms || kslice < 1 || dslice < 1 || c->kp.ncand <= 0 || c->kp.nrec <= 0) return SIFT3D_ERR_ARG;
    HIPCHK(c, hipSetDevice(c->device));
    float taps3[SIFT3D_MAX_TAPS];
    sift3d_gauss_taps(0.5f, 0.01f, taps3);
    const int64_t ncand = c->kp.ncand, nrec = c->kp.nrec;
    hipEvent_t ev[6];
    for (hipEvent_t &e : ev) HIPCHK(c, hipEventCreate(&e));
    hipStream_t s1 = c->stream, s2 = c->kp_stream;
    HIPCHK(c, hipStreamSynchronize(s1));
    HIPCHK(c, hipStreamSynchronize(s2));
    auto launch_k = [&](hipStream_t st, int64_t a, int64_t n) -> hipError_t {
        sift3d_kp_params q = c->kp.p;
        q.patch0 = c->patch0 + (size_t)a * SIFT3D_PATCH_VOX;
        return sift3d_launch_keypointsA(st, q, c->keys_b + a, c->vals_b + a, n, c->kps + a, c->nrec + a, taps3);
    };
    auto launch_d = [&](hipStream_t st, int64_t b, int64_t m) -> hipError_t {
        return sift3d_launch_descriptors(st, c->kp.p, c->kps, c->rec_kp + b, c->rec_frame + b, m, c->d_hrecs + b, c->d_hgroup + b, c->kp.taps5);
    };
    HIPCHK(c, hipEventRecord(ev[0], s1));
    HIPCHK(c, launch_k(s1, 0, ncand));
    HIPCHK(c, hipMemsetAsync(c->sampler_tokens, 0, sizeof(int) * SIFT3D_CU_SLOTS, s1));
    HIPCHK(c, launch_d(s1, 0, nrec));
    HIPCHK(c, hipEventRecord(ev[1], s1));
    HIPCHK(c, hipStreamSynchronize(s1));
    HIPCHK(c, hipMemsetAsync(c->sampler_tokens, 0, sizeof(int) * SIFT3D_CU_SLOTS, s1));
    HIPCHK(c, hipEventRecord(ev[2], s1));
    HIPCHK(c, hipStreamWaitEvent(s2, ev[2], 0));
    enum { NS = 4 };
    hipStream_t ks[NS], ds[NS];
    hipEvent_t done[2 * NS];
    for (int i = 0; i < NS; i++) {
        HIPCHK(c, hipStreamCreateWithFlags(&ks[i], hipStreamNonBlocking));
        HIPCHK(c, hipStreamCreateWithFlags(&ds[i], hipStreamNonBlocking));
        HIPCHK(c, hipEventCreateWithFlags(&done[i], hipEventDisableTiming));
        HIPCHK(c, hipEventCreateWithFlags(&done[NS + i], hipEventDisableTiming));
        HIPCHK(c, hipStreamWaitEvent(ks[i], ev[2], 0));
        HIPCHK(c, hipStreamWaitEvent(ds[i], ev[2], 0));
    }
    (void)s2;
    int64_t a = 0, b = 0;
    int ki = 0, di = 0;
    while (a < ncand || b < nrec) {
        if (a < ncand) {
            const int64_t n = ncand - a < kslice ? ncand - a : kslice;
            HIPCHK(c, launch_k(ks[ki++ % NS], a, n));
            a += n;
        }
        const int64_t b_to = ncand > 0 ? (int64_t)((double)nrec * (double)a / (double)ncand) : nrec;
        while (b < nrec && (b < b_to || a >= ncand)) {
            const int64_t m = nrec - b < dslice ? nrec - b : dslice;
            HIPCHK(c, launch_d(ds[di++ % NS], b, m));
            b += m;
        }
    }
    for (int i = 0; i < NS; i++) {
        HIPCHK(c, hipEventRecord(done[i], ks[i]));
        HIPCHK(c, hipEventRecord(done[NS + i], ds[i]));
        HIPCHK(c, hipStreamWaitEvent(s1, done[i], 0));
        HIPCHK(c, hipStreamWaitEvent(s1, done[NS + i], 0));
    }
    HIPCHK(c, hipEventRecord(ev[4], s1));
    HIPCHK(c, hipStreamSynchronize(s1));
    for (int i = 0; i < NS; i++) {
        hipStreamDestroy(ks[i]);
        hipStreamDestroy(ds[i]);
        hipEventDestroy(done[i]);
        hipEventDestroy(done[NS + i]);
    }
    float m0 = 0, m1 = 0;
    HIPCHK(c, hipEventElapsedTime(&m0, ev[0], ev[1]));
    HIPCHK(c, hipEventElapsedTime(&m1, ev[2], ev[4]));
    out_ms[0] = m0;
    out_ms[1] = m1;
    for (hipEvent_t e : ev) hipEventDestroy(e);
    return SIFT3D_OK;
}
#endif

int describe_sorted(sift3d_ctx *c, const std::vector<sift3d_level> &levels, int64_t ncand, int desc_mode,
                           float eig_thres, float size_factor, int64_t *n_out, bool levels_on_device)
{
    int rc = describe_queue(c, levels, ncand, desc_mode, eig_thres, size_factor, levels_on_device);
    if (!rc) rc = describe_launch(c);
    if (!rc) rc = describe_finish(c, n_out);
    return rc;
}

static int finish_split_tail(sift3d_ctx *c, const std::vector<sift3d_level> &levels, bool levels_on_device, int desc_mode, float eig_thres,
                             float size_factor, int64_t *n_out, bool *done)
{
    *done = false;
    unsigned long long *const h_split = c->h_cnt0 + 8 + SIFT3D_KP_MAX_CHUNKS;
    const int64_t capA = c->cand_split_at, capB = c->cand_cap - capA;
    hipStream_t ks = c->kp_stream;
    float taps3[SIFT3D_MAX_TAPS];
    auto fall_back = [&](unsigned long long overflow_mark) -> int {
        HIPCHK(c, hipStreamSynchronize(ks));
        HIPCHK(c, hipStreamSynchronize(c->stream));
        if (overflow_mark > 0) {
            const int rc = surv_make_room(c, overflow_mark);
            if (rc) return rc;
        }
        return cand_replay(c);
    };
    h_split[3] = h_split[5] = h_split[7] = 0;
    HIPCHK(c, hipMemcpyAsync(h_split + 3, c->d_count, sizeof(unsigned long long) * 5, hipMemcpyDeviceToHost, c->stream));
    HIPCHK(c, hipEventSynchronize(c->ev_split[2]));
    const int64_t nA = (int64_t)h_split[0];
    if (h_split[2] > 0 || nA > capA) return fall_back(h_split[2]);
    int rc = describe_begin(c, levels.size(), taps3);
    if (rc) return rc;
    rc = ensure_kp_buffers(c, nA + nA / 8 + 4096, nA);
    if (rc) return rc;
    kp_params_of(c, desc_mode, eig_thres, size_factor, c->kp.p);
    c->kp.split = true;
    if (!levels_on_device)
        HIPCHK(c, hipMemcpyAsync(c->d_levels, levels.data(), sizeof(sift3d_level) * levels.size(), hipMemcpyHostToDevice, ks));
    int nch = 0;
    if (nA > 0) {
        HIPCHK(c, sift3d_sort_candidates(ks, c->sort_tmp, c->sort_tmp_bytes, c->keys_a, c->keys_b, c->vals_a, c->vals_b, nA));
        rc = describe_queue_chunk(c, nch++, 0, nA, ks, taps3);
        if (rc) return rc;
    }
    c->kp.nchunks = nch;
    HIPCHK(c, hipStreamSynchronize(c->stream));
    const int64_t nB = (int64_t)h_split[7];
    if (h_split[5] > 0 || nB > capB || nA + nB > c->kps_cap || (int64_t)h_split[3] != nA) return fall_back(h_split[5]);
    if (nB > 0) {
        HIPCHK(c, sift3d_sort_candidates(ks, c->sort_tmp, c->sort_tmp_bytes, c->keys_a + capA, c->keys_b + nA, c->vals_a + capA, c->vals_b + nA, nB));
        rc = describe_queue_chunk(c, nch++, nA, nA + nB, ks, taps3);
        if (rc) return rc;
    }
    c->kp.nchunks = nch;
    c->kp.ncand = nA + nB;
    c->last.n_extrema = nA + nB;
    rc = describe_launch(c);
    if (!rc) rc = describe_finish(c, n_out);
    if (rc) return rc;
    *done = true;
    return SIFT3D_OK;
}

static int run_pipeline(sift3d_ctx *c, float init_scale, bool extract, int desc_mode, float eig_thres, float size_factor,
                        sift3d_candidate **cands_out, sift3d_feature **feats_out, int64_t *n_out)
{
    if (!c) return SIFT3D_ERR_ARG;
    if (c->lean) return set_err(c, SIFT3D_ERR_ARG, "a slab context holds no pyramid (sift3d_create_slab)");
    if (!c->has_volume) return set_err(c, SIFT3D_ERR_ARG, "no volume set (sift3d_set_volume)");
    HIPCHK(c, hipSetDevice(c->device));
    timing_begin(c);
    c->last_run.clear();
    std::vector<octave_dims> oct = octave_list(c->nx, c->ny, c->nz);
    if (c->max_octaves > 0 && oct.size() > (size_t)c->max_octaves) oct.resize((size_t)c->max_octaves);

    const octave_sigmas s = sigma_schedule(init_scale);
    const int64_t xp0 = pitch_of(c->nx);
    int rc = blur_dev(c, c->vol, c->L[0], nullptr, xp0, c->ny, c->nz, s.extra0, 0.01f);
    if (rc) return rc;
    if (xp0 != c->nx) HIPCHK(c, sift3d_launch_zero_pad(c->stream, c->L[0], nullptr, xp0, c->nx, c->ny * c->nz));
    rc = cand_reset(c, c->ex_stream);
    if (rc) return rc;
    HIPCHK(c, hipEventRecord(c->ev_reset, c->ex_stream));
    const bool split_tail = extract && oct.size() >= 3 && c->tune[SIFT3D_TUNE_SPLIT_TAIL] && c->timing != 3 && c->tune[SIFT3D_TUNE_KP_CHUNKS] == 0;
    if (split_tail) {
        int64_t second = c->cand_cap / 16 + 1024 < c->cand_cap / 2 ? c->cand_cap / 16 + 1024 : c->cand_cap / 2;
        if (c->tune[SIFT3D_TUNE_SPLIT_TAIL] == 2) second = 8;
        c->cand_split_at = c->cand_cap - second;
    }
    unsigned long long *const h_split = c->h_cnt0 + 8 + SIFT3D_KP_MAX_CHUNKS;

    int64_t tiny_base = -1;
    for (const octave_dims &d : oct)
        if (tiny_base < 0 && d.X * d.Y * d.Z <= SIFT3D_TINY_VOX) tiny_base = d.off;
    auto octave_buffers = [&](const octave_dims &d, const float *L[5], const float *D[5]) {
        for (int j = 0; j < 5; j++) {
            L[j] = c->L[j] + d.off;
            D[j] = c->D[j] ? c->D[j] + d.off : nullptr;
        }
    };
    std::vector<sift3d_level> levels(oct.size() * 3);
    {
        float fscale = 1;
        for (size_t o = 0; o < oct.size(); o++) {
            const octave_dims &d = oct[o];
            const float *L[5], *D[5];
            octave_buffers(d, L, D);
            octave_level_rows(&levels[o * 3], L, D, d.X, d.XP, d.Y, d.Z, d.Z, 0, s, fscale);
            fscale *= 2.0f;
        }
    }
    if (split_tail && levels.size() <= 96)
        HIPCHK(c, hipMemcpyAsync(c->d_levels, levels.data(), sizeof(sift3d_level) * levels.size(), hipMemcpyHostToDevice, c->kp_stream));
    float next_taps[SIFT3D_MAX_TAPS];
    const int next_ntaps = sift3d_gauss_taps(s.extras[4], 0.01f, next_taps);
    std::vector<octave_run> runs(oct.size());
    bool used_second = false;
    auto enqueue_extrema = [&](size_t o, int which) -> int {
        const octave_dims &d = oct[o];
        const octave_run &ru = runs[o];
        hipStream_t exs = c->timing == 3 ? c->stream : (which == 0 ? c->ex_stream : c->ex_stream2);
        if (exs != c->ex_stream) HIPCHK(c, hipStreamWaitEvent(exs, c->ev_reset, 0));
        if (exs != c->stream) {
            hipEvent_t ev = which == 0 ? c->ev_oct[0] : c->ev_ex2[0];
            HIPCHK(c, hipEventRecord(ev, c->stream));
            HIPCHK(c, hipStreamWaitEvent(exs, ev, 0));
            if (which == 1) used_second = true;
        }
        const cand_where where = {exs, (exs != c->stream && which == 1) ? 1 : 0, o >= 2 ? 1 : 0};
        const float *L[5], *D[5];
        octave_buffers(d, L, D);
        if (ru.lazy) D[0] = D[4] = nullptr;
        if (ru.tiny_done) D[4] = ru.d4tiny;
        level_job jobs[3];
        octave_jobs(jobs, L, D, d.XP, d.X, d.Y, d.Z, 0, (int)d.Z, (int)o * 3, next_taps, next_ntaps);
        if (ru.tiny_done) return cand_append_octave_small(c, jobs, D, d.XP, d.X, d.Y, d.Z, where);
        int rc_ = SIFT3D_OK;
        for (int l = 0; l < 3 && !rc_; l++) rc_ = cand_append(c, jobs[l], where, true);
        return rc_;
    };
    for (size_t o = 0; o < oct.size(); o++) {
        const octave_dims &d = oct[o];
        const double N = (double)d.X * d.Y * d.Z;
        hipStream_t ws = c->stream;
        octave_run &ru = runs[o];
        ru.tiny_done = false;
        ru.d4tiny = (tiny_base >= 0 && d.off >= tiny_base && d.off - tiny_base + d.XP * d.Y * d.Z <= SIFT3D_D4TINY_FLOATS)
                        ? c->D4tiny + (d.off - tiny_base) : nullptr;
        if (d.X * d.Y * d.Z <= SIFT3D_TINY_VOX && ru.d4tiny && c->tune[SIFT3D_TUNE_TINY_OCTAVE]) {
            sift3d_octave_taps ot;
            sift3d_octave_out oo;
            bool ok = true;
            for (int j = 1; j < 6 && ok; j++) {
                float taps[SIFT3D_MAX_TAPS];
                const int n = sift3d_gauss_taps(s.extras[j - 1], 0.01f, taps);
                ok = n >= 3 && n <= 2 * SIFT3D_FAST_MAX_R + 1;
                for (int q = 0; ok && q < n; q++) ot.f[j - 1][q] = taps[q];
                ot.n[j - 1] = n;
                oo.L[j - 1] = j < 5 ? c->L[j] + d.off : nullptr;
                oo.D[j - 1] = j < 5 ? c->D[j - 1] + d.off : ru.d4tiny;
            }
            if (ok) {
                stage_scope sc(c, SIFT3D_STAGE_OCTAVE_TINY, 40.0 * N, 0, (int64_t)N, ws);
                hipError_t e = sift3d_launch_tiny_octave(ws, c->L[0] + d.off, oo, d.X, d.XP, d.Y, d.Z, ot);
                if (e == hipSuccess) ru.tiny_done = true;
                else if (e != hipErrorNotSupported) HIPCHK(c, e);
                else sc.cancel();
            }
        }
        ru.lazy = !ru.tiny_done && lazy_shape_ok(d.XP, d.Y, d.Z) && c->tune[SIFT3D_TUNE_LAZY_LEVELS] && next_ntaps == 2 * SIFT3D_FAST_MAX_R + 1;
        const bool more = o + 1 < oct.size();
        for (int j = 1; j < 6; j++) {
            bool sub_done = false;
            if (!ru.tiny_done && !(ru.lazy && j == 5)) {
                if (j == 5) {
                    rc = ensure_level_buffer(c, &c->D[4]);
                    if (rc) return rc;
                }
                float *dst_dog = (ru.lazy && j == 1) ? nullptr : c->D[j - 1] + d.off;
                float *sub = nullptr;
                if (j == 3 && more && d.XP % 8 == 0 && oct[o + 1].XP == d.XP / 2) sub = c->L[0] + oct[o + 1].off;
                rc = blur_dev(c, c->L[j - 1] + d.off, j < 5 ? c->L[j] + d.off : nullptr, dst_dog, d.XP, d.Y, d.Z, s.extras[j - 1], 0.01f, sub, &sub_done);
                if (rc) return rc;
                if (d.XP != d.X)
                    HIPCHK(c, sift3d_launch_zero_pad(ws, j < 5 ? c->L[j] + d.off : nullptr, dst_dog, d.XP, d.X, d.Y * d.Z));
            }
            if (j == 3 && more) {
                const octave_dims &dn = oct[o + 1];
                if (!sub_done) {
                    stage_scope sc(c, SIFT3D_STAGE_SUBSAMPLE, 4.5 * N, 0, (int64_t)N, ws);
                    HIPCHK(c, sift3d_launch_subsample(ws, c->L[3] + d.off, d.XP, d.X, d.Y, d.Z, c->L[0] + dn.off, dn.XP));
                }
                if (dn.XP != dn.X) HIPCHK(c, sift3d_launch_zero_pad(ws, c->L[0] + dn.off, nullptr, dn.XP, dn.X, dn.Y * dn.Z));
            }
        }
        if (o == 0 && oct.size() == 1) {
            rc = enqueue_extrema(0, 0);
            if (rc) return rc;
        } else if (o >= 1) {
            if (o == 1) {
                rc = enqueue_extrema(0, 0);
                if (rc) return rc;
            }
            rc = enqueue_extrema(o, 1);
// ... 75 lines not shown
```

### 3d_sift_cuda_amd/csrc/kernels_keypoint.hip

```cpp
#include <cstddef>
#include <type_traits>

#include "desc_bins.h"
#include "sift3d_internal.h"

#define PD SIFT3D_PATCH_DIM
#define PV SIFT3D_PATCH_VOX



__device__ __forceinline__ float trilinear(const float *__restrict__ img, int X, int XP, int Y, int Z, int Zl, int z_off,
                                           float x, float y, float z)
{
    float wx, wy, wz;
    int ix, iy, iz;
    interp_coord(x, 0, (float)X, ix, wx);
    interp_coord(y, 0, (float)Y, iy, wy);
    interp_coord(z, 0, (float)Z, iz, wz);
    iz -= z_off;
    iz = iz < 0 ? 0 : (iz > Zl - 2 ? Zl - 2 : iz);
    const long long XY = (long long)XP * Y;
    const float *p = img + (long long)iz * XY + (long long)iy * XP + ix;
    typedef float f2u __attribute__((ext_vector_type(2), aligned(4)));
    const f2u q00 = *reinterpret_cast<const f2u *>(p), q10 = *reinterpret_cast<const f2u *>(p + XP);
// ... 464 lines not shown
            float n[9];
#pragma unroll
            for (int k = 0; k < 9; k++) n[k] = g[rb + ((k / 3 - 1) * PD + (k % 3 - 1)) * PD + x + 1];
            const float c = b[4];
            bool pk = true;
#pragma unroll
            for (int k = 0; k < 9; k++) {
                pk = pk && (a[k] < c) && (n[k] < c);
                if (k != 4) pk = pk && (b[k] < c);
            }
            flags[rb + x] = pk ? 1 : 0;
#pragma unroll
            for (int k = 0; k < 9; k++) {
                a[k] = b[k];
                b[k] = n[k];
            }
        }
        flags[rb + PD - 1] = 0;
    } else if (t < 81 + PD * PD) {
        const int q = t - 81, y = q % PD, z = q / PD;
        if (y == 0 || y == PD - 1 || z == 0 || z == PD - 1) {
#pragma unroll
            for (int x = 0; x < PD; x++) flags[(z * PD + y) * PD + x] = 0;
        }
    }
    __syncthreads();
    if (threadIdx.x < 64) {
        int n = 0;
        for (int base = 0; base < PV; base += 64) {
            const int s = base + threadIdx.x;
            const bool pk = s < PV && flags[s] != 0;
            const unsigned long long m = __ballot(pk);
            if (pk) {
                const int pos = n + __popcll(m & ((1ull << threadIdx.x) - 1ull));
                raw_idx[pos] = (short)s;
                raw_val[pos] = g[s];
            }
            n += __popcll(m);
        }
        if (threadIdx.x == 0) *n_lds = n;
    }
    __syncthreads();
    const int n = *n_lds;
    for (int i = threadIdx.x; i < n; i += NT) {
        const float vi = raw_val[i];
        int rank = 0;
        for (int j = 0; j < n; j++) {
            const float vj = raw_val[j];
            rank += (vj > vi || (vj == vi && j < i)) ? 1 : 0;
        }
        pk_idx[rank] = raw_idx[i];
        pk_val[rank] = vi;
    }
    __syncthreads();
    return n;
}

__device__ __forceinline__ void interp_point_patch(const float *g, int s, float *o)
{
    const int ix = s % PD, iy = (s / PD) % PD, iz = s / (PD * PD);
    const float c = g[s];
    o[0] = (float)interp_quadratic(ix - 1, ix, ix + 1, g[s - 1], c, g[s + 1]);
    o[1] = (float)interp_quadratic(iy - 1, iy, iy + 1, g[s - PD], c, g[s + PD]);
    o[2] = (float)interp_quadratic(iz - 1, iz, iz + 1, g[s - PD * PD], c, g[s + PD * PD]);
}

__device__ __forceinline__ void splat_params(float x, float y, float z, short &base, float &wx, float &wy, float &wz)
{
    int ix, iy, iz;
    interp_coord(x, 0, (float)PD, ix, wx);
    interp_coord(y, 0, (float)PD, iy, wy);
    interp_coord(z, 0, (float)PD, iz, wz);
    base = (short)(ix | (iy << 4) | (iz << 8));
}

__device__ __forceinline__ void wave_splat_sequence(float *grid, int n, const short *sp_base, const v4f *sp4)
{
    const int lane = threadIdx.x;
    const int slot = lane >> 3;
    const int a = lane & 1, b = (lane >> 1) & 1, c = (lane >> 2) & 1;
    float *g = grid;
    if (lane < 64) {
        int packed = 0;
        float wx = 0, wy = 0, wz = 0, v = 0;
        if (slot < n) {
            packed = sp_base[slot];
            const v4f q = sp4[slot];
            wx = q.x; wy = q.y; wz = q.z; v = q.w;
        }
        for (int g0 = 0; g0 < n; g0 += 8) {
            const int i = g0 + slot;
            const bool ok = i < n;
            const int ix = packed & 15, iy = (packed >> 4) & 15, iz = packed >> 8;
            const int cell = ((iz + c) * PD + (iy + b)) * PD + (ix + a);
            const float ux = a ? (1.0f - wx) : wx;
            const float uy = b ? (1.0f - wy) : wy;
            const float uz = c ? (1.0f - wz) : wz;
            const float contrib = v * ux * uy * uz;
            const int in = i + 8;
            if (in < n) {
                packed = sp_base[in];
                const v4f q = sp4[in];
                wx = q.x; wy = q.y; wz = q.z; v = q.w;
            }
#pragma unroll
            for (int j = 0; j < 8; j++) {
                if (slot == j && ok) __hip_atomic_fetch_add(&g[cell], contrib, __ATOMIC_RELAXED, __HIP_MEMORY_SCOPE_WORKGROUP);
                __builtin_amdgcn_wave_barrier();
            }
        }
    }
    __syncthreads();
}

__device__ __forceinline__ long long xcd_contiguous_item(long long n, int seg)
{
    const long long b = blockIdx.x;
    if (seg <= 0) {
        const long long per = (n + 7) / 8;
        return (b % 8) * per + b / 8;
    }
    const long long s0 = b / seg * seg, local = b - s0;
    return s0 + (local % 8) * (seg / 8) + local / 8;
}

struct kpA_smem {
    float A[PV + 1];
    union {
        float sp_tail[2 * NRAD_PAD];
        struct {
            unsigned char flags[PV + 13];
            short raw_idx[128], pk2_idx[128];
            float raw_val[128], pk2_val[128];
        } pk;
    } C;
    float B[PV + 1];
    float gx[NRAD_PAD], gy[NRAD_PAD], gz[NRAD_PAD];
    union {
        unsigned short rlist[NRAD_PAD];
        short sp_base[NRAD_PAD];
    } r;
    short pk_idx[128];
    float pk_val[128];
    float ori_data[PD * 3 + 3];
    float sc[16];
    float taps[8];
    int cnt[4];
};
static_assert(sizeof(kpA_smem) * 7 <= 160 * 1024, "seven workgroups per CU");
static_assert(offsetof(kpA_smem, C) == sizeof(float) * (PV + 1) && sizeof(float) * (PV + 1) + sizeof(float) * 2 * NRAD_PAD >= 16 * NRAD_PAD,
              "the splat parameters span A and C");

__global__ __launch_bounds__(KP_NT, 7) void keypoint_kernel(sift3d_kp_params p, const unsigned long long *__restrict__ keys,
                                                      const sift3d_cval *__restrict__ vals, long long ncand,
                                                      sift3d_dkp *__restrict__ kps, int *__restrict__ nrec_out,
                                                      sift3d_taps taps3)
{
    __shared__ __attribute__((aligned(16))) kpA_smem sm;
    const long long k = blockIdx.x;
    if (k >= ncand) return;
    const int lane = threadIdx.x;
    if (lane < 3) sm.taps[lane] = taps3.f[lane];
    const unsigned long long key = keys[k];
    const sift3d_cval cvl = vals[k];
    const int lvl = (int)(key >> SIFT3D_KEY_LVL_SHIFT);
    const int is_max = (int)((key >> SIFT3D_KEY_MAX_SHIFT) & 1ull);
    const long long cidx = (long long)(key & SIFT3D_KEY_IDX_MASK);
    const sift3d_level lv = p.levels[lvl];
    sift3d_dkp *kp = kps + k;
    const int X = lv.X, Y = lv.Y, Z = lv.Z, XP = lv.XP;
    const long long XY = (long long)XP * Y;
    const int ix = (int)(cidx % XP), iy = (int)((cidx / XP) % Y), iz = (int)(cidx / XY) + lv.z_off;

    const float *C = lv.dogc;
    const float cv = C[cidx];
    float fx = (float)interp_quadratic(ix - 1, ix, ix + 1, C[cidx - 1], cv, C[cidx + 1]);
    float fy = (float)interp_quadratic(iy - 1, iy, iy + 1, C[cidx - XP], cv, C[cidx + XP]);
    float fz = (float)interp_quadratic(iz - 1, iz, iz + 1, C[cidx - XY], cv, C[cidx + XY]);
    float scale = (float)(2 * interp_quadratic(lv.sigma_h, lv.sigma_c, lv.sigma_l, cvl.h, cv, cvl.l));
    fx += 0.5f; fy += 0.5f; fz += 0.5f;

    const float rad = 2.0f * scale;
    const int rmax = (int)(rad + 2);
    if (fx - rmax < 0 || fy - rmax < 0 || fz - rmax < 0 || fx + rmax >= X || fy + rmax >= Y || fz + rmax >= Z) {
        if (lane == 0) nrec_out[k] = 0;
        return;
    }
    float *patch = sm.A;
    const float ident[9] = {1, 0, 0, 0, 1, 0, 0, 0, 1};
    wave_sample_patch<KP_NT>(patch, lv.img, X, lv.XP, Y, Z, lv.Zl, lv.z_off, fx, fy, fz, scale, ident);
#ifdef SIFT3D_DEV
    if (p.debug_stop == 1) { if (lane == 0) nrec_out[k] = 0; return; }
#endif
    wave_normalize_patch<KP_NT>(patch, sm.sc);
#ifdef SIFT3D_DEV
    if (p.debug_stop == 2) { if (lane == 0) nrec_out[k] = 0; return; }
#endif
    const int nrad = wave_build_radius_list(sm.r.rlist, &sm.cnt[0]);

    for (int i = lane; i < NRAD_PAD; i += KP_NT) {
        float a = 0, b = 0, c = 0;
        if (i < nrad) {
            const int s = sm.r.rlist[i];
            a = patch[s + 1] - patch[s - 1];
            b = patch[s + PD] - patch[s - PD];
            c = patch[s + PD * PD] - patch[s - PD * PD];
        }
        sm.gx[i] = a; sm.gy[i] = b; sm.gz[i] = c;
    }
    __syncthreads();
    if (lane < 9) {
        const float *ei = lane / 3 == 0 ? sm.gx : (lane / 3 == 1 ? sm.gy : sm.gz);
        const float *ej = lane % 3 == 0 ? sm.gx : (lane % 3 == 1 ? sm.gy : sm.gz);
        float acc = 0;
        int i = 0;
        for (; i + 16 <= nrad; i += 16) {
            v4f a[4], b[4];
#pragma unroll
            for (int q = 0; q < 4; q++) {
                a[q] = *reinterpret_cast<const v4f *>(ei + i + 4 * q);
                b[q] = *reinterpret_cast<const v4f *>(ej + i + 4 * q);
            }
#pragma unroll
            for (int q = 0; q < 4; q++) {
                acc += a[q].x * b[q].x; acc += a[q].y * b[q].y; acc += a[q].z * b[q].z; acc += a[q].w * b[q].w;
            }
        }
        for (; i < nrad; i++) acc += ei[i] * ej[i];
        sm.sc[lane] = acc;
    }
    __syncthreads();
#ifdef SIFT3D_DEV
    if (p.debug_stop == 3) { if (lane == 0) nrec_out[k] = 0; return; }
#endif
    auto svd_and_eigen_test = [&]() {
        float mat[3][3], w[3], v[3][3];
        for (int i = 0; i < 3; i++)
            for (int j = 0; j < 3; j++) {
                mat[i][j] = sm.sc[i * 3 + j];
                v[i][j] = 0;
            }
        w[0] = w[1] = w[2] = 0;
        svd3(mat, w, v);
        sort_eig(w, v);
        float es = w[0] + w[1] + w[2];
        float ep = w[0] * w[1] * w[2];
        float esp = es * es * es;
        int keep = (esp < p.eig_thres * ep || p.eig_thres < 0) ? 1 : 0;
        sm.sc[15] = keep ? 1.0f : 0.0f;
        if (keep) {
            kp->x = fx; kp->y = fy; kp->z = fz; kp->scale = scale;
            kp->eigs[0] = w[0]; kp->eigs[1] = w[1]; kp->eigs[2] = w[2];
            for (int i = 0; i < 3; i++)
                for (int j = 0; j < 3; j++) kp->ori0[i * 3 + j] = v[i][j];
            kp->info = is_max ? SIFT3D_INFO_MIN0MAX1 : 0u;
            kp->lvl = lvl;
        } else {
            nrec_out[k] = 0;
        }
    };
#ifdef SIFT3D_DEV
    const bool svd_first = p.debug_stop == 40;
    if (svd_first) {
        if (lane == KP_NT - 64) svd_and_eigen_test();
        __syncthreads();
        if (sm.sc[15] == 0.0f) return;
    }
#else
    constexpr bool svd_first = false;
#endif
    for (int s = lane; s < PV; s += KP_NT) p.patch0[(long long)k * PV + s] = patch[s];
    __syncthreads();

    float *t0 = sm.B;
    float *ta = sm.A;
    v4f *sp4 = reinterpret_cast<v4f *>(sm.A);
    const float radius = (float)(PD / 2);
    for (int s = lane; s < PV; s += KP_NT) t0[s] = 0;
    for (int i = lane; i < nrad; i += KP_NT) {
        float e[3] = {sm.gx[i], sm.gy[i], sm.gz[i]};
        float m2 = e[0] * e[0] + e[1] * e[1] + e[2] * e[2];
        float mg = 0, wx = 0, wy = 0, wz = 0;
        short base = 0;
        if (m2 != 0) {
            mg = sqrtf(m2);
            float u[3];
            for (int q = 0; q < 3; q++) u[q] = e[q] * radius / mg;
            for (int q = 0; q < 3; q++) u[q] += radius;
            splat_params((float)(u[0] + 0.5), (float)(u[1] + 0.5), (float)(u[2] + 0.5), base, wx, wy, wz);
        }
        sm.r.sp_base[i] = base;
        v4f q; q.x = wx; q.y = wy; q.z = wz; q.w = mg;
        sp4[i] = q;
    }
    __syncthreads();
    if (!svd_first && lane == KP_NT - 64) svd_and_eigen_test();
    wave_splat_sequence(t0, nrad, sm.r.sp_base, sp4);
    if (sm.sc[15] == 0.0f) return;
#ifdef SIFT3D_DEV
    if (p.debug_stop == 4 || p.debug_stop == 5) { if (lane == 0) nrec_out[k] = 0; return; }
#endif
#ifdef SIFT3D_DEV
    if (p.debug_stop == 6) { if (lane == 0) nrec_out[k] = 0; return; }
#endif
    wave_blur_patch<KP_NT>(t0, ta, t0, sm.taps, 3);
#ifdef SIFT3D_DEV
    if (p.debug_stop == 7) { if (lane == 0) nrec_out[k] = 0; return; }
#endif
    const int npk = wave_peaks_sorted<KP_NT>(ta, sm.C.pk.flags, &sm.cnt[1], sm.C.pk.raw_idx, sm.C.pk.raw_val, sm.pk_idx, sm.pk_val);
#ifdef SIFT3D_DEV
    if (p.debug_stop == 8) { if (lane == 0) nrec_out[k] = 0; return; }
#endif

// ... 153 lines not shown
        if (p.debug_stop == 21) return;
    } else
#endif
    if (fr < 0) {
        const float *src = p.patch0 + (long long)rec_kp[r] * PV;
        for (int s = lane; s < PV; s += DESC_NT) sm.patch[s] = src[s];
        __syncthreads();
    } else {
        int *tok = nullptr;
        if (p.sampler_cap > 0) {
            unsigned hw, xcc;
            asm volatile("s_getreg_b32 %0, hwreg(HW_REG_HW_ID)" : "=s"(hw));
            asm volatile("s_getreg_b32 %0, hwreg(HW_REG_XCC_ID)" : "=s"(xcc));
            tok = p.sampler_tokens + ((((xcc & 7u) * 8u + ((hw >> 13) & 7u)) * 2u + ((hw >> 12) & 1u)) * 16u + ((hw >> 8) & 15u));
            if (lane == 0) {
                for (int tries = 0;; tries++) {
                    if (atomicAdd(tok, 1) < p.sampler_cap || tries > 50000) break;
                    atomicSub(tok, 1);
                    __builtin_amdgcn_s_sleep(64);
                }
            }
            __syncthreads();
        }
        wave_sample_patch<DESC_NT>(sm.patch, lv.img, lv.X, lv.XP, lv.Y, lv.Z, lv.Zl, lv.z_off, kp->x, kp->y, kp->z, kp->scale, ori);
        if (tok && lane == 0) atomicSub(tok, 1);
    }
#ifdef SIFT3D_DEV
    if (p.debug_stop == 11) return;
#endif
    wave_normalize_patch<DESC_NT>(sm.patch, sm.sc);
#ifdef SIFT3D_DEV
    if (p.debug_stop == 12 || p.debug_stop == 23) return;
#endif

    const bool w0 = lane < 64;
    float myval = 0.0f;
    if constexpr (SIFT) {
        for (int q = lane; q < NINT; q += DESC_NT) {
            const int x = q % 9 + 1, y = (q / 9) % 9 + 1, z = q / 81 + 1;
            const int s = (z * PD + y) * PD + x;
            float e[3] = {sm.patch[s + 1] - sm.patch[s - 1], sm.patch[s + PD] - sm.patch[s - PD],
                          sm.patch[s + PD * PD] - sm.patch[s - PD * PD]};
            float mg = v3_mag(e);
            int best = 8;
            if (mg > 0) {
                v3_norm(e);
                const float oa[8][3] = {{1, 1, 1},  {1, 1, -1},  {1, -1, 1},  {1, -1, -1},
                                        {-1, 1, 1}, {-1, 1, -1}, {-1, -1, 1}, {-1, -1, -1}};
                best = 0;
                float bd = v3_dot(oa[0], e);
#pragma unroll
                for (int t = 1; t < 8; t++) {
                    float d = v3_dot(oa[t], e);
                    if (d > bd) {
                        bd = d;
                        best = t;
                    }
                }
            }
            const int en = desc_bins_entry(x, y, z);
            sm.u.v.mag[en] = mg;
            sm.u.v.bin[en] = (unsigned char)best;
            if (desc_bins_needs_all(mg)) sm.u.v.all = 1;
        }
        __syncthreads();
#ifdef SIFT3D_DEV
        if (p.debug_stop == 13 || p.debug_stop == 24) return;
#endif
        if (w0) {
            const float acc = sm.u.v.all ? desc_bins_walk_all(sm.u.v.mag, sm.u.v.bin, lane) : desc_bins_walk(sm.u.v.mag, sm.u.v.bin, lane);
#ifdef SIFT3D_DEV
            if (p.debug_stop == 26) return;
#endif
            float mn = 100000;
#pragma unroll
            for (int i = 0; i < 64; i++) {
                float vi = lane_value(acc, i);
                if (vi < mn) mn = vi;
            }
            float v = acc - mn;
            float ss = 0;
#pragma unroll
            for (int i = 0; i < 64; i++) {
                float vi = lane_value(v, i);
                ss += vi * vi;
            }
            float div = 1.0f / sqrtf(ss);
            myval = v * div;
        }
    } else {
        wave_blur_patch<DESC_NT>(sm.patch, sm.u.v.t1, sm.patch, sm.taps, 5);
        if (w0) {
            const float *bl = sm.u.v.t1;
            const int x1 = c_brief_x[3 * lane], y1 = c_brief_x[3 * lane + 1], z1 = c_brief_x[3 * lane + 2];
            const int x2 = c_brief_y[3 * lane], y2 = c_brief_y[3 * lane + 1], z2 = c_brief_y[3 * lane + 2];
            float d = bl[x1 + y1 * PD + z1 * PD * PD] - bl[x2 + y2 * PD + z2 * PD * PD];
            if (p.desc_mode == SIFT3D_DESC_BRIEF) {
                myval = (d < 0) ? 1.0f : 0.0f;
            } else if (p.desc_mode == SIFT3D_DESC_RRIEF) {
                myval = d;
            } else {
                float fdx = x1 - x2, fdy = y1 - y2, fdz = z1 - z2;
                int dist = (int)sqrtf(fdx * fdx + fdy * fdy + fdz * fdz);
                myval = d / dist;
            }
        }
    }
    if (!w0) return;
    int rank = 0;
    const unsigned long long nans = __ballot(myval != myval);
    if (nans == 0) {
#pragma unroll
        for (int j = 0; j < 64; j++) {
            float vj = lane_value(myval, j);
            rank += (vj < myval || (vj == myval && j < lane)) ? 1 : 0;
        }
    } else {
        const unsigned long long below = nans & ((1ull << lane) - 1ull), above = lane == 63 ? 0ull : nans & ~((2ull << lane) - 1ull);
        const int lo = below ? 64 - __clzll((long long)below) : 0;
        const int hi = above ? __ffsll((long long)above) - 1 : 64;
        rank = lo;
        for (int j = 0; j < 64; j++) {
            float vj = lane_value(myval, j);
            rank += (j >= lo && j < hi && (vj < myval || (vj == myval && j < lane))) ? 1 : 0;
        }
        if (myval != myval) rank = lane;
    }
    const int grp = kp->lvl * 2 + ((kp->info & SIFT3D_INFO_MIN0MAX1) ? 1 : 0);
    sift3d_feature *out = recs + r + (p.rec_shift ? (long long)p.rec_shift[grp] : 0ll);
    out->desc[lane] = (float)rank;
    static_assert(offsetof(sift3d_feature, desc) == 17 * 4 && offsetof(sift3d_feature, ori) == 16 && offsetof(sift3d_feature, eigs) == 52 &&
                      offsetof(sift3d_feature, info) == 64, "record layout: x y z scale ori[9] eigs[3] info desc[64]");
    if (lane < 17) {
        const float fac = lv.octave_factor, add = 0;
        unsigned word;
        if (lane < 4) {
            float v = lane == 0 ? kp->x : (lane == 1 ? kp->y : (lane == 2 ? kp->z : kp->scale));
            if (lane == 3) v *= fac;
            else v = v * fac + add;
            v *= p.size_factor;
            word = __builtin_bit_cast(unsigned, v);
        } else if (lane < 13) {
            word = __builtin_bit_cast(unsigned, fr < 0 ? kp->ori0[lane - 4] : kp->frames[fr * 9 + lane - 4]);
        } else if (lane < 16) {
            word = __builtin_bit_cast(unsigned, kp->eigs[lane - 13]);
        } else {
            word = kp->info | (fr < 0 ? 0u : SIFT3D_INFO_REORIENT);
        }
        reinterpret_cast<unsigned *>(out)[lane] = word;
        if (lane == 0) rec_group[r] = grp;
    }
}

__global__ void group_count_kernel(const unsigned long long *__restrict__ keys, const int *__restrict__ nrec, long long ncand, int *__restrict__ counts)
{
    const long long k = (long long)blockIdx.x * blockDim.x + threadIdx.x;
    if (k >= ncand) return;
    const int n = nrec[k];
    if (n <= 0) return;
    int g = (int)(keys[k] >> SIFT3D_KEY_LVL_SHIFT) * 2 + (int)((keys[k] >> SIFT3D_KEY_MAX_SHIFT) & 1ull);
    if (g < 0 || g >= SIFT3D_GROUPS - 1) g = SIFT3D_GROUPS - 1;
    atomicAdd(counts + g, n);
}

hipError_t sift3d_launch_group_counts(hipStream_t s, const unsigned long long *keys, const int *nrec, int64_t ncand, int *counts)
{
    if (ncand <= 0) return hipSuccess;
    hipLaunchKernelGGL(group_count_kernel, dim3((unsigned)((ncand + 255) / 256)), dim3(256), 0, s, keys, nrec, (long long)ncand, counts);
    return hipGetLastError();
}

__global__ void recmap_kernel(const int *__restrict__ nrec, const int *__restrict__ offs, long long ncand, int cand_off,
                              int *rec_base, int *__restrict__ rec_kp, int *__restrict__ rec_frame, unsigned long long *kp_count)
{
    const long long k = (long long)blockIdx.x * blockDim.x + threadIdx.x;
    if (k >= ncand) return;
    const int n = nrec[k], o = rec_base[0] + offs[k];
    if (k == ncand - 1) rec_base[1] = o + n;
    if (n > 0) atomicAdd(kp_count, 1ull);
    for (int f = 0; f < n; f++) {
        rec_kp[o + f] = cand_off + (int)k;
        rec_frame[o + f] = f - 1;
    }
}

hipError_t sift3d_launch_keypointsA(hipStream_t s, const sift3d_kp_params &p, const unsigned long long *keys,
                                    const sift3d_cval *vals, int64_t ncand, sift3d_dkp *kps, int *nrec, const float *taps3)
{
    if (ncand <= 0) return hipSuccess;
    sift3d_taps t;
    for (int i = 0; i < 17; i++) t.f[i] = i < 3 ? taps3[i] : 0.0f;
    hipLaunchKernelGGL(keypoint_kernel, dim3((unsigned)ncand), dim3(KP_NT), 0, s, p, keys, vals, (long long)ncand, kps, nrec, t);
    return hipGetLastError();
}

hipError_t sift3d_launch_recmap(hipStream_t s, const int *nrec, const int *offs, int64_t ncand, int cand_off, int *rec_base,
                                int *rec_kp, int *rec_frame, unsigned long long *kp_count)
{
    if (ncand <= 0) return hipSuccess;
    hipLaunchKernelGGL(recmap_kernel, dim3((unsigned)((ncand + 255) / 256)), dim3(256), 0, s, nrec, offs, (long long)ncand,
                       cand_off, rec_base, rec_kp, rec_frame, kp_count);
    return hipGetLastError();
}

hipError_t sift3d_launch_descriptors(hipStream_t s, const sift3d_kp_params &p, const sift3d_dkp *kps, const int *rec_kp,
                                     const int *rec_frame, int64_t nrec, sift3d_feature *recs, int *rec_group,
                                     const float *taps5)
{
    if (nrec <= 0) return hipSuccess;
    sift3d_taps t;
    for (int i = 0; i < 17; i++) t.f[i] = i < 5 ? taps5[i] : 0.0f;
    const int seg = p.desc_seg;
    const dim3 grid((unsigned)(seg > 0 ? (nrec + seg - 1) / seg * seg : ((nrec + 7) / 8) * 8));
    if (p.desc_mode == SIFT3D_DESC_SIFT)
        hipLaunchKernelGGL(descriptor_kernel<true>, grid, dim3(DESC_NT), 0, s, p, kps, rec_kp, rec_frame, (long long)nrec, recs,
                           rec_group, t);
    else
        hipLaunchKernelGGL(descriptor_kernel<false>, grid, dim3(DESC_NT), 0, s, p, kps, rec_kp, rec_frame, (long long)nrec, recs,
                           rec_group, t);
    return hipGetLastError();
}
```

### 3d_sift_cuda_amd/csrc/pipeline.h

```cpp
#ifndef SIFT3D_PIPELINE_H
#define SIFT3D_PIPELINE_H
#include <cmath>
#include <cstdint>
#include <cstring>
#include <vector>

#include "sift3d_internal.h"

#define SIFT3D_KP_MAX_CHUNKS 16
#define SIFT3D_KP_DEFAULT_CHUNKS 1
#define SIFT3D_D4TINY_FLOATS 32768

struct timed_launch {
    int stage;
    hipEvent_t e0, e1;
    int ntaps;
    int64_t nvox;
    double bytes;
    float ms;
    float start_ms;
};

struct level_job {
    const float *dp, *dc, *dn;
    int64_t X, Y, Z;
    int z_lo, z_hi;
    int lvl_id;
    int64_t Xl;
    const float *prev_b = nullptr, *next_g = nullptr;
    float next_taps[2 * SIFT3D_FAST_MAX_R + 1] = {};
    int next_ntaps = 0;
};

struct octave_dims {
    int64_t X, Y, Z, off;
    int64_t XP;
};

struct octave_sigmas {
    float extra0;
    float extras[5];
    float sig[6];
};
static inline octave_sigmas sigma_schedule(float initial_image_scale)
{
    octave_sigmas s;
    float sigma_init = 0.5f;
    if (initial_image_scale > 0) sigma_init /= initial_image_scale;
    const float factor = (float)pow(2.0, 1.0 / (double)3);
    s.extra0 = sqrtf(1.6f * 1.6f - sigma_init * sigma_init);
    float sg = 1.6f;
    s.sig[0] = sg;
    for (int j = 0; j < 5; j++) {
        s.extras[j] = sg * sqrtf(factor * factor - 1.0f);
        sg *= factor;
        s.sig[j + 1] = sg;
    }
    return s;
}

static inline void octave_jobs(level_job jobs[3], const float *const L[5], const float *const D[5], int64_t XP, int64_t Xl, int64_t Y,
                               int64_t Zl, int z_lo, int z_hi, int first_id, const float *next_taps, int next_ntaps)
{
    for (int l = 0; l < 3; l++) jobs[l] = {D[l], D[l + 1], D[l + 2], XP, Y, Zl, z_lo, z_hi, first_id + l, Xl};
    if (!D[0]) {
        jobs[0].dp = L[0];
        jobs[0].prev_b = L[1];
    }
    if (!D[4]) {
        jobs[2].next_g = L[4];
        jobs[2].next_ntaps = next_ntaps;
        for (int q = 0; q < next_ntaps; q++) jobs[2].next_taps[q] = next_taps[q];
    }
}

static inline void octave_level_rows(sift3d_level rows[3], const float *const L[5], const float *const D[5], int64_t X, int64_t XP, int64_t Y,
                                     int64_t Z, int64_t Zl, int64_t z_off, const octave_sigmas &s, float octave_factor)
{
    for (int l = 0; l < 3; l++) {
        sift3d_level &lv = rows[l];
        memset(&lv, 0, sizeof lv);
        lv.img = L[l + 1];
        lv.dogc = D[l + 1];
        lv.X = (int)X; lv.Y = (int)Y; lv.Z = (int)Z;
        lv.XP = (int)XP;
        lv.sigma_h = s.sig[l]; lv.sigma_c = s.sig[l + 1]; lv.sigma_l = s.sig[l + 2];
        lv.octave_factor = octave_factor;
        lv.Zl = (int)Zl;
        lv.z_off = (int)z_off;
    }
}

struct octave_run {
    bool tiny_done;
    bool lazy;
    float *d4tiny;
};

struct sift3d_ctx {
    int device;
    hipStream_t stream;
    hipStream_t ex_stream;
    hipStream_t ex_stream2;
    hipEvent_t ev_ex2[2];
    hipEvent_t ev_reset;
    sift3d_survivor *surv2;
    int64_t surv2_cap;
    hipStream_t kp_stream;
    hipEvent_t ev_kpc[SIFT3D_KP_MAX_CHUNKS];
    hipEvent_t ev_desc;
    hipEvent_t ev_split[3];
    unsigned long long *h_cnt0;
    hipEvent_t ev_oct[2];
    hipEvent_t ev_fence[2];
    bool own_stream;
    int64_t capN;
    int64_t capTot;
    float *vol;
    float *L[6];
    float *D[5];
    float *D4tiny;
    float *T[2];
    float *d_taps;
    unsigned long long *keys_a, *keys_b;
    sift3d_cval *vals_a, *vals_b;
    int64_t cand_cap;
    unsigned long long *d_count;
    int64_t cand_split_at;
    sift3d_survivor *surv;
    sift3d_survivor2 *list2[2];
    int64_t list2_cap[2];
    unsigned long long *list2_counts;
    unsigned long long *surv_counts;
    int surv_set;
    int64_t surv_cap;
    int surv_div;
    void *sort_tmp;
    size_t sort_tmp_bytes;
    void *scan_tmp;
    size_t scan_tmp_bytes;
    sift3d_level *d_levels;
    sift3d_dkp *kps;
    float *patch0;
    int *sampler_tokens;
    int *d_rec_base;
    int *nrec, *offs;
    int64_t kps_cap;
    int *rec_kp, *rec_frame;
    int64_t recs_cap;
    int64_t capT;
    int64_t hrecs_cap;
    sift3d_feature *h_recs;
    int *h_group;
    sift3d_feature *d_hrecs;
    int *d_hgroup;
    struct {
        sift3d_kp_params p;
        float taps5[SIFT3D_MAX_TAPS];
        int64_t ncand, nrec;
        int nchunks, launched;
        int64_t first[SIFT3D_KP_MAX_CHUNKS + 1];
        bool split;
    } kp;
    struct {
        bool counts;
        int *d_counts, *h_counts, *d_shift;
        sift3d_feature *dst;
    } place;
    int dev_stop;
    bool count_queued;
    std::vector<struct level_job> jobs;
    int64_t nx, ny, nz;
    int64_t pad_nx, pad_ny, pad_nz;
    bool has_volume;
    std::vector<octave_run> last_run;
    bool strict_extrema;
    struct {
        bool open;
        int64_t nx, ny, nz, got;
        int resize;
        std::vector<bool> seen;
    } up;
    int max_octaves;
    int tune[SIFT3D_TUNE_COUNT];
    int64_t host_grows;
    int staged = 0;
    bool lean;
    int timing;
    std::vector<timed_launch> launches;
    std::vector<hipEvent_t> pool;
    size_t pool_used;
    size_t resolved;
    sift3d_timings last;
    char err[512];
};

#pragma GCC visibility push(hidden)
int set_err(sift3d_ctx *c, int code, const char *fmt, ...);

#define HIPCHK(c, call)                                                                                        \
    do {                                                                                                       \
        hipError_t e_ = (call);                                                                                \
        if (e_ != hipSuccess)                                                                                  \
            return set_err((c), SIFT3D_ERR_DEVICE, "%s failed: %s (%s:%d)", #call, hipGetErrorString(e_), __FILE__, \
                           __LINE__);                                                                          \
    } while (0)

static inline int64_t pitch_of(int64_t X) { return (X + 3) / 4 * 4; }

#define NEED_LEVELS(c)                                                                                                  \
    do {                                                                                                                \
        if ((c) && (c)->lean) return set_err((c), SIFT3D_ERR_ARG, "%s needs a full context (sift3d_create), not a slab context", __func__); \
    } while (0)

#define FENCED(c, op)                 \
    do {                              \
        int rc_ = fence_in(c);        \
        if (rc_) return rc_;          \
        rc_ = (op);                   \
        if (rc_) return rc_;          \
        return fence_out(c);          \
    } while (0)


sift3d_ctx *ctx_create(int device, int64_t nx, int64_t ny, int64_t nz, bool lean);
void timing_begin(sift3d_ctx *c);
int blur_dev(sift3d_ctx *c, const float *in, float *out, float *dog, int64_t X, int64_t Y, int64_t Z, float sigma, float min_value,
             float *sub = nullptr, bool *sub_done = nullptr);
bool blur_window_supported(int64_t X, int64_t Y, float sigma, float min_value);
int blur_window_dev(sift3d_ctx *c, const float *in, float *out, float *dog, int64_t X, int64_t Y, int64_t Z, int64_t zo0, int64_t zo1, float sigma,
                    float min_value);
int cand_reset(sift3d_ctx *c, hipStream_t on = nullptr);
struct cand_where {
    hipStream_t stream = nullptr;
    int list = 0;
    int group = 0;
};
int cand_append(sift3d_ctx *c, const level_job &j, const cand_where &w, bool record);
int cand_append_octave_small(sift3d_ctx *c, const level_job jobs[3], const float *const D[5], int64_t XP, int64_t X, int64_t Y, int64_t Z,
                             const cand_where &w);
int cand_count_queue(sift3d_ctx *c);
int cand_finalize(sift3d_ctx *c, int64_t *count_out);
int describe_queue(sift3d_ctx *c, const std::vector<sift3d_level> &levels, int64_t ncand, int desc_mode, float eig_thres, float size_factor,
                   bool levels_on_device);
void describe_want_group_counts(sift3d_ctx *c, bool on);
int describe_group_counts(sift3d_ctx *c, const int **counts, int64_t *total);
int describe_placement(sift3d_ctx *c, sift3d_feature *shared_list, const int *shift);
int describe_launch(sift3d_ctx *c);
int describe_finish(sift3d_ctx *c, int64_t *n_out);

static inline hipEvent_t get_event(sift3d_ctx *c)
{
    if (c->pool_used == c->pool.size()) {
        hipEvent_t e;
        hipEventCreate(&e);
        c->pool.push_back(e);
    }
    return c->pool[c->pool_used++];
}

struct stage_scope {
    sift3d_ctx *c;
    int stage;
    hipEvent_t e0, e1;
    int ntaps;
    int64_t nvox;
    double bytes;
    hipStream_t st;
    bool timed;
    stage_scope(sift3d_ctx *c_, int stage_, double bytes_, int ntaps_ = 0, int64_t nvox_ = 0, hipStream_t st_ = nullptr)
        : c(c_), stage(stage_), e0(nullptr), e1(nullptr), ntaps(ntaps_), nvox(nvox_), bytes(bytes_), st(st_ ? st_ : c_->stream)
    {
        c->last.launches[stage] += 1;
        c->last.alg_bytes[stage] += bytes;
        timed = c->timing == 1 || c->timing == 3 ||
                (c->timing == 2 && nvox == pitch_of(c->nx) * c->ny * c->nz &&
                 (stage == SIFT3D_STAGE_BLUR_FUSED || stage == SIFT3D_STAGE_BLUR_X || stage == SIFT3D_STAGE_BLUR_Y ||
                  stage == SIFT3D_STAGE_BLUR_Z_DOG));
        if (timed) {
            e0 = get_event(c);
            e1 = get_event(c);
            hipEventRecord(e0, st);
        }
    }
    void add_bytes(double more)
    {
        c->last.alg_bytes[stage] += more;
        bytes += more;
    }
    void cancel()
    {
        c->last.launches[stage] -= 1;
        c->last.alg_bytes[stage] -= bytes;
        if (timed) c->pool_used -= 2;
        stage = -1;
    }
    ~stage_scope()
    {
        if (stage < 0) return;
        if (timed) {
            hipEventRecord(e1, st);
            c->launches.push_back({stage, e0, e1, ntaps, nvox, bytes, 0.0f, 0.0f});
        }
    }
};

static inline cand_target cand_target_of(const sift3d_ctx *c, int group)
{
    if (c->cand_split_at <= 0) return {c->keys_a, c->vals_a, c->d_count, c->cand_cap};
    if (group == 0) return {c->keys_a, c->vals_a, c->d_count, c->cand_split_at};
    return {c->keys_a + c->cand_split_at, c->vals_a + c->cand_split_at, c->d_count + 4, c->cand_cap - c->cand_split_at};
}

std::vector<octave_dims> octave_list(int64_t X, int64_t Y, int64_t Z);
int alloc_cands(sift3d_ctx *c, int64_t cap);
int ensure_T(sift3d_ctx *c, int64_t floats);
void timing_end(sift3d_ctx *c);
int check_shape(sift3d_ctx *c, int64_t nx, int64_t ny, int64_t nz);
int fence_in(sift3d_ctx *c);
int fence_out(sift3d_ctx *c);
int cand_replay(sift3d_ctx *c);
int surv_make_room(sift3d_ctx *c, unsigned long long high_water);
int describe_sorted(sift3d_ctx *c, const std::vector<sift3d_level> &levels, int64_t ncand, int desc_mode, float eig_thres, float size_factor, int64_t *n_out, bool levels_on_device = false);
int candidates_to_host(sift3d_ctx *c, const std::vector<sift3d_level> &levels, int64_t ncand, sift3d_candidate **cands_out, int64_t *n_out);
#pragma GCC visibility pop
#endif
```

### 3d_sift_cuda_amd/csrc/sift3d_internal.h

```cpp
#ifndef SIFT3D_INTERNAL_H
#define SIFT3D_INTERNAL_H

#include <hip/hip_runtime.h>
#include <stdint.h>

#include "blur_plan.h"
#include "extrema_plan.h"
#include "sift3d.h"
#include "sift3d_dev.h"

#define SIFT3D_MAX_TAPS 129
#define SIFT3D_FAST_MAX_R 8
#define SIFT3D_PATCH_DIM 11
#define SIFT3D_PATCH_VOX 1331

struct sift3d_taps {
    float f[2 * SIFT3D_FAST_MAX_R + 1];
};

typedef float v4f __attribute__((ext_vector_type(4)));
template <int VEC>
struct vecT;
template <> struct vecT<4> { typedef v4f type; };
template <> struct vecT<1> { typedef float type; };
template <int VEC>
__device__ __forceinline__ typename vecT<VEC>::type vload(const float *p)
{
    return *reinterpret_cast<const typename vecT<VEC>::type *>(p);
}
template <int VEC>
__device__ __forceinline__ void vstore(float *p, typename vecT<VEC>::type v)
{
    *reinterpret_cast<typename vecT<VEC>::type *>(p) = v;
}

#define SIFT3D_KEY_LVL_SHIFT 40
#define SIFT3D_KEY_MAX_SHIFT 39
#define SIFT3D_KEY_IDX_MASK ((1ull << 39) - 1ull)
struct sift3d_survivor {
    long long idx;
    float value;
    int is_max;
};
struct sift3d_survivor2 {
    int x, y, z;
    int is_max;
    float value;
    float h;
};
struct sift3d_cval {
    float value, h, l, pad;
};

struct sift3d_level {
    const float *img;
    const float *dogc;
    int X, Y, Z;
    int XP;
    float sigma_h, sigma_c, sigma_l;
    float octave_factor;
    int Zl;
    int z_off;
    int pad;
};

hipError_t sift3d_launch_blur_x(hipStream_t s, const float *in, float *out, int64_t X, int64_t Y, int64_t Z,
                                const float *taps, int ntaps, const float *d_taps);
hipError_t sift3d_launch_blur_y(hipStream_t s, const float *in, float *out, int64_t X, int64_t Y, int64_t Z,
                                const float *taps, int ntaps, const float *d_taps);
hipError_t sift3d_launch_blur_z(hipStream_t s, const float *in, float *out, const float *prev, float *dog, int64_t X,
                                int64_t Y, int64_t Z, const float *taps, int ntaps, const float *d_taps);
hipError_t sift3d_launch_blur_fused(hipStream_t s, const float *in, float *out, float *dog, int64_t X, int64_t Y, int64_t Z,
                                    const float *taps, int ntaps, const sift3d_blur_tuning &tune, int64_t zo0 = 0, int64_t zo1 = -1,
                                    float *sub = nullptr, int *sub_done = nullptr);
hipError_t sift3d_launch_dog(hipStream_t s, const float *a, const float *b, float *out, int64_t n);
hipError_t sift3d_launch_subsample(hipStream_t s, const float *in, int64_t X, int64_t Xl, int64_t Y, int64_t Z, float *out,
                                   int64_t XPout);
hipError_t sift3d_launch_zero_pad(hipStream_t s, float *a, float *b, int64_t X, int64_t Xl, int64_t rows);
#define SIFT3D_TINY_VOX 4096
#define SIFT3D_EAGER_T_FLOATS (1ll << 31)
struct sift3d_octave_out {
    float *L[5];
    float *D[5];
};
struct sift3d_octave_taps {
    float f[5][2 * SIFT3D_FAST_MAX_R + 1];
    int n[5];
};
hipError_t sift3d_launch_tiny_octave(hipStream_t s, const float *L0, const sift3d_octave_out &o, int64_t X, int64_t XP, int64_t Y,
                                     int64_t Z, const sift3d_octave_taps &t);
hipError_t sift3d_launch_double_size(hipStream_t s, const float *in, int64_t X, int64_t Y, int64_t Z, float *out);
hipError_t sift3d_launch_halve_size(hipStream_t s, const float *in, int64_t X, int64_t Y, int64_t Z, float *out);
struct sift3d_extrema_lazy {
    const float *prev_b;
    const float *next_g;
    float taps[2 * SIFT3D_FAST_MAX_R + 1];
    int ntaps;
    sift3d_survivor2 *list2;
    unsigned long long *list2_count;
    int64_t list2_cap;
};
static_assert(EX_LAZY_NTAPS == 2 * SIFT3D_FAST_MAX_R + 1, "the third phase is built for the widest filter of the templated kernels");
struct cand_target {
    unsigned long long *keys;
    sift3d_cval *vals;
    unsigned long long *count;
    int64_t cap;
};
struct sift3d_extrema_pass {
    const float *dprev, *dcur, *dnext;
    int64_t X, Xl, Y, Z;
    int z_lo, z_hi, lvl_id;
    cand_target out;
    sift3d_survivor *surv;
    unsigned long long *surv_count;
    unsigned long long *surv_overflow;
    int64_t surv_cap;
    bool zero_counters;
    const sift3d_extrema_lazy *lazy;
    bool strict;
};
hipError_t sift3d_launch_extrema(hipStream_t s, const sift3d_extrema_pass &p);
hipError_t sift3d_launch_scan_strict(hipStream_t s, const float *v, int64_t n, unsigned *flag);
bool sift3d_volume_needs_strict(const float *v, int64_t n);
hipError_t sift3d_launch_extrema_octave_small(hipStream_t s, const float *const d[5], int64_t X, int64_t Xl, int64_t Y, int64_t Z,
                                              int lvl_id0, const cand_target &out);
#define SIFT3D_SURV_SETS 96
#define SIFT3D_SURV_COUNTERS (EX_SEGS * EX_SEG_STRIDE)
#define SIFT3D_LIST2_COUNTERS EX_SEGS

struct sift3d_kp_params {
    const sift3d_level *levels;
    float eig_thres;
    float size_factor;
    int desc_mode;
    int debug_stop;
    float *patch0;
    int *sampler_tokens;
    int sampler_cap;
    int desc_seg;
    const int *rec_shift;
};
hipError_t sift3d_launch_group_counts(hipStream_t s, const unsigned long long *keys, const int *nrec, int64_t ncand, int *counts);
#define SIFT3D_CU_SLOTS 2048
#define SIFT3D_MAX_FRAMES 11
struct sift3d_dkp {
    float x, y, z, scale;
    float eigs[3];
    float ori0[9];
    int nframes;
    float frames[SIFT3D_MAX_FRAMES * 9];
    int lvl;
    unsigned info;
};
hipError_t sift3d_launch_keypointsA(hipStream_t s, const sift3d_kp_params &p, const unsigned long long *keys,
                                    const sift3d_cval *vals, int64_t ncand, sift3d_dkp *kps, int *nrec, const float *taps3);
hipError_t sift3d_launch_recmap(hipStream_t s, const int *nrec, const int *offs, int64_t ncand, int cand_off, int *rec_base,
                                int *rec_kp, int *rec_frame, unsigned long long *kp_count);
hipError_t sift3d_launch_descriptors(hipStream_t s, const sift3d_kp_params &p, const sift3d_dkp *kps, const int *rec_kp,
                                     const int *rec_frame, int64_t nrec, sift3d_feature *recs, int *rec_group,
                                     const float *taps5);
size_t sift3d_sort_temp_bytes(int64_t n);
hipError_t sift3d_sort_candidates(hipStream_t s, void *temp, size_t temp_bytes, const unsigned long long *keys_in,
                                  unsigned long long *keys_out, const sift3d_cval *vals_in, sift3d_cval *vals_out, int64_t n);
size_t sift3d_scan_temp_bytes(int64_t n);
hipError_t sift3d_scan_counts(hipStream_t s, void *temp, size_t temp_bytes, const int *in, int *out, int64_t n);

hipError_t sift3d_launch_knn_norms(hipStream_t s, const signed char *v, int64_t n, int *norms, unsigned long long *stats);
hipError_t sift3d_launch_knn(hipStream_t s, const signed char *db, const int *db_norm, int64_t n_db, const signed char *q, const int *q_norm,
                             int64_t n_q, int k, int const_norm, int groups, int segments, int *part_d, int *part_i, int *out_i, int *out_d);
int sift3d_knn_list_length(int k);
void sift3d_knn_plan(int64_t n_db, int64_t n_q, int k, int *groups, int *segments);

hipError_t sift3d_launch_ratio(hipStream_t s, const signed char *db, const int *db_norm, int64_t n_db, const signed char *q, const int *q_norm,
                               int64_t n_q, const float *geo, const unsigned *info, float lo, float hi, int *i1, int *d1, int *i2, int *d2);
hipError_t sift3d_launch_hough(hipStream_t s, const float *p0, const float *p1, const float *s0, const float *s1, const float *o0, const float *o1,
                               int M, float lo, float hi, int one, int *counts, int *flags, float *hyp);
hipError_t sift3d_launch_resample(hipStream_t s, const float *src, int64_t nx, int64_t ny, int64_t nz, float *dst, int64_t ox, int64_t oy,
                                  int64_t oz, const float *map, int nearest, float fill);
hipError_t sift3d_launch_guided(hipStream_t s, const void *f_rows, const int *f_norm, const float *f_pos, const unsigned *f_info, const int *f_idx,
                                int n_f, const int *cell_start, const long long *keys, const double grid_o[3], double edge, const long long grid_n[3],
                                int dense, const void *m_rows, const float *m_pos, const unsigned *m_info, const int *order, int n_m,
                                const float c0[3], const float c1[3], const float rot[9], float scale, float radius, float lo, float hi, int *i1,
                                int *d1, int *i2, int *d2, int *visited);

#pragma GCC visibility push(hidden)
struct sift3d_scale_intervals {
    float lo[2], hi[2];
    int ok[2];
};
const sift3d_scale_intervals &sift3d_scale_ivs();
int sift3d_put_pairs(sift3d_similarity *out, int32_t n, const int32_t *moving, const int32_t *fixed, const int32_t *inlier, const int32_t *dist2,
                     const char *what, char *err, int64_t err_len);
#pragma GCC visibility pop

#endif
```

### 3d_sift_cuda_amd/csrc/sort_scan.hip

```cpp
#include <cstring>

#include <rocprim/rocprim.hpp>

#include "sift3d_internal.h"

static const unsigned SORT_END_BIT = 48;

size_t sift3d_sort_temp_bytes(int64_t n)
{
    size_t bytes = 0;
    (void)rocprim::radix_sort_pairs(nullptr, bytes, (const unsigned long long *)nullptr, (unsigned long long *)nullptr,
                                    (const float4 *)nullptr, (float4 *)nullptr, (size_t)n, 0, SORT_END_BIT, (hipStream_t)0);
    return bytes;
}

hipError_t sift3d_sort_candidates(hipStream_t s, void *temp, size_t temp_bytes, const unsigned long long *keys_in,
                                  unsigned long long *keys_out, const sift3d_cval *vals_in, sift3d_cval *vals_out, int64_t n)
{
    if (n <= 0) return hipSuccess;
    return rocprim::radix_sort_pairs(temp, temp_bytes, keys_in, keys_out, (const float4 *)vals_in, (float4 *)vals_out,
                                     (size_t)n, 0, SORT_END_BIT, s);
}

size_t sift3d_scan_temp_bytes(int64_t n)
{
    size_t bytes = 0;
    (void)rocprim::exclusive_scan(nullptr, bytes, (const int *)nullptr, (int *)nullptr, 0, (size_t)n, rocprim::plus<int>(),
                                  (hipStream_t)0);
    return bytes;
}

hipError_t sift3d_scan_counts(hipStream_t s, void *temp, size_t temp_bytes, const int *in, int *out, int64_t n)
{
    if (n <= 0) return hipSuccess;
    return rocprim::exclusive_scan(temp, temp_bytes, in, out, 0, (size_t)n, rocprim::plus<int>(), s);
}
```

### include/sift3d.h

```cpp
#ifndef SIFT3D_H
#define SIFT3D_H

#include <stdint.h>

#ifdef __cplusplus
extern "C" {
#endif

#define SIFT3D_ABI_VERSION 6
int sift3d_abi_version(void);

#define SIFT3D_DESC_LEN 64
#define SIFT3D_INFO_MIN0MAX1 0x00000010u
#define SIFT3D_INFO_REORIENT 0x00000020u

typedef enum {
    SIFT3D_OK = 0,
    SIFT3D_ERR_ARG = -1,
    SIFT3D_ERR_DEVICE = -2,
    SIFT3D_ERR_MEMORY = -3,
    SIFT3D_ERR_CAPACITY = -4,
    SIFT3D_ERR_COMM = -5
} sift3d_status;

typedef enum { SIFT3D_DESC_SIFT = 0, SIFT3D_DESC_BRIEF = 1, SIFT3D_DESC_RRIEF = 2, SIFT3D_DESC_NRRIEF = 3 } sift3d_desc_mode;

typedef struct {
    int32_t x, y, z;
    float value;
} sift3d_extremum;

typedef struct {
    float x, y, z, scale;
    float ori[9];
    float eigs[3];
    uint32_t info;
    float desc[SIFT3D_DESC_LEN];
} sift3d_feature;

typedef struct {
    int32_t octave, level;
    int32_t is_max;
    int32_t x, y, z;
    float value, h_value, l_value;
} sift3d_candidate;

typedef struct sift3d_ctx sift3d_ctx;

int sift3d_device_count(void);
sift3d_ctx *sift3d_create(int device, int64_t nx, int64_t ny, int64_t nz);
sift3d_ctx *sift3d_create_slab(int device, int64_t nx, int64_t ny, int64_t nz_local);
void sift3d_destroy(sift3d_ctx *ctx);
const char *sift3d_last_error(const sift3d_ctx *ctx);
int sift3d_set_stream(sift3d_ctx *ctx, void *hip_stream);
int sift3d_sync(sift3d_ctx *ctx);
void sift3d_free(void *p);

int sift3d_gauss_taps(float sigma, float min_value, float *taps);
#define SIFT3D_LIBM_CURRENT 0
#define SIFT3D_LIBM_GCC5 1
int sift3d_set_libm_variant(int which);
int sift3d_get_libm_variant(void);


int sift3d_gauss_blur(sift3d_ctx *ctx, const float *in, float *out, int64_t nx, int64_t ny, int64_t nz, float sigma,
                      float min_value);
int sift3d_gauss_blur_dev(sift3d_ctx *ctx, const float *d_in, float *d_out, int64_t nx, int64_t ny, int64_t nz,
                          float sigma, float min_value);
int sift3d_gauss_blur_dog_dev(sift3d_ctx *ctx, const float *d_in, float *d_out, float *d_dog, int64_t nx, int64_t ny,
                              int64_t nz, float sigma, float min_value);
int sift3d_gauss_blur_dog_half_dev(sift3d_ctx *ctx, const float *d_in, float *d_out, float *d_dog, float *d_half, int64_t nx,
                                   int64_t ny, int64_t nz, float sigma, float min_value, int *in_one_launch);
int sift3d_blur_window_supported(int64_t nx, int64_t ny, float sigma, float min_value);
int sift3d_gauss_blur_dog_window_dev(sift3d_ctx *ctx, const float *d_in, float *d_out, float *d_dog, int64_t nx, int64_t ny,
                                     int64_t nz, int64_t z_lo, int64_t z_hi, float sigma, float min_value);
int sift3d_dog(sift3d_ctx *ctx, const float *a, const float *b, float *out, int64_t n);
int sift3d_dog_dev(sift3d_ctx *ctx, const float *d_a, const float *d_b, float *d_out, int64_t n);
int sift3d_subsample2(sift3d_ctx *ctx, const float *in, int64_t nx, int64_t ny, int64_t nz, float *out);
int sift3d_subsample2_dev(sift3d_ctx *ctx, const float *d_in, int64_t nx, int64_t ny, int64_t nz, float *d_out);
int sift3d_extrema(sift3d_ctx *ctx, const float *d_prev, const float *d_cur, const float *d_next, int64_t nx, int64_t ny,
                   int64_t nz, sift3d_extremum *minima, int64_t cap_min, int64_t *n_min, sift3d_extremum *maxima,
                   int64_t cap_max, int64_t *n_max);
int sift3d_double_size(sift3d_ctx *ctx, const float *in, int64_t nx, int64_t ny, int64_t nz, float *out);
int sift3d_halve_size(sift3d_ctx *ctx, const float *in, int64_t nx, int64_t ny, int64_t nz, float *out);

int sift3d_set_volume(sift3d_ctx *ctx, const float *vol, int64_t nx, int64_t ny, int64_t nz);
int sift3d_set_volume_dev(sift3d_ctx *ctx, const float *d_vol, int64_t nx, int64_t ny, int64_t nz);
int sift3d_set_volume_resized(sift3d_ctx *ctx, const float *vol, int64_t nx, int64_t ny, int64_t nz, int resize);
int sift3d_set_volume_begin(sift3d_ctx *ctx, int64_t nx, int64_t ny, int64_t nz, int resize);
int sift3d_set_volume_planes(sift3d_ctx *ctx, const float *planes, int64_t z0, int64_t n);
int sift3d_set_volume_end(sift3d_ctx *ctx);
int sift3d_reserve(sift3d_ctx *ctx, int64_t n_extrema);
int sift3d_detect(sift3d_ctx *ctx, float initial_image_scale, sift3d_candidate **out, int64_t *n_out);
int sift3d_extract(sift3d_ctx *ctx, float initial_image_scale, int desc_mode, float eig_thres, float size_factor,
                   sift3d_feature **out, int64_t *n_out);
int sift3d_get_level_slice(sift3d_ctx *ctx, int octave, int level, int64_t z, float *out, int64_t *nx_out, int64_t *ny_out);
int sift3d_get_dog_slice(sift3d_ctx *ctx, int octave, int level, int64_t z, float *out, int64_t *nx_out, int64_t *ny_out);
int sift3d_set_max_octaves(sift3d_ctx *ctx, int n);
typedef enum {
    SIFT3D_TUNE_BLUR_FUSED = 0,
    SIFT3D_TUNE_FUSED_CHUNKS,
    SIFT3D_TUNE_FUSED_ROWS,
    SIFT3D_TUNE_LAZY_LEVELS,
    SIFT3D_TUNE_TINY_OCTAVE,
    SIFT3D_TUNE_SAMPLER_CAP,
    SIFT3D_TUNE_KP_CHUNKS,
    SIFT3D_TUNE_BANDS_FIRST,
    SIFT3D_TUNE_HOST_RECORDS,
    SIFT3D_TUNE_FUSED_TILE,
    SIFT3D_TUNE_FUSED_SUB,
    SIFT3D_TUNE_SPLIT_TAIL,
    SIFT3D_TUNE_DESC_SEGMENT,
    SIFT3D_TUNE_FUSED_ORDER,
    SIFT3D_TUNE_FUSED_STAGGER,
    SIFT3D_TUNE_COUNT
} sift3d_tuning;
int sift3d_set_tuning(sift3d_ctx *ctx, int knob, int value);
int64_t sift3d_host_buffer_grows(const sift3d_ctx *ctx);

int sift3d_extract_view(sift3d_ctx *ctx, float initial_image_scale, int desc_mode, float eig_thres, float size_factor,
                        const sift3d_feature **view, int64_t *n_out);

typedef struct {
    const float *img;
    const float *dogc;
    int64_t nx, ny, nz_local, nz_global, z_offset;
    float sigma_h, sigma_c, sigma_l;
    float octave_factor;
} sift3d_level_desc;
int sift3d_candidates_reset(sift3d_ctx *ctx);
int sift3d_extrema_append_dev(sift3d_ctx *ctx, const float *d_prev, const float *d_cur, const float *d_next, int64_t nx,
                              int64_t ny, int64_t nz_local, int level_id, int64_t z_lo, int64_t z_hi);
int sift3d_lazy_levels_supported(int64_t nx, int64_t ny, int64_t nz_local, float next_sigma);
int sift3d_extrema_append_lazy_dev(sift3d_ctx *ctx, const float *d_prev, const float *g_prev_a, const float *g_prev_b,
                                   const float *d_cur, const float *d_next, const float *g_next, float next_sigma, int64_t nx,
                                   int64_t ny, int64_t nz_local, int level_id, int64_t z_lo, int64_t z_hi);
int sift3d_candidates_dev(sift3d_ctx *ctx, const sift3d_level_desc *levels, int n_levels, sift3d_candidate **out,
                          int64_t *n_out);
int sift3d_describe_dev(sift3d_ctx *ctx, const sift3d_level_desc *levels, int n_levels, int desc_mode, float eig_thres,
                        float size_factor, const sift3d_feature **view, const int32_t **group_view, int64_t *n_out);

#define SIFT3D_GROUPS 193
int sift3d_describe_dev_counts(sift3d_ctx *ctx, const sift3d_level_desc *levels, int n_levels, int desc_mode, float eig_thres,
                               float size_factor, const int32_t **group_counts, int64_t *n_records);
int sift3d_describe_dev_place(sift3d_ctx *ctx, sift3d_feature *list, const int32_t *shift, const sift3d_feature **own_view,
                              const int32_t **group_view, int64_t *n_out);
int sift3d_host_register(void *p, int64_t bytes);
int sift3d_host_unregister(void *p);

typedef struct {
    int32_t n_ranks, sharded_octaves;
    int64_t exchanges;
    int64_t halo_bytes_critical;
    int64_t halo_bytes_deferred;
    int64_t gather_bytes;
    int64_t n_extrema, n_keypoints, n_records;
    double wall_ms;
    int64_t halo_bytes_hidden;
    int32_t transport;
    int32_t transport_fell_back;
    int32_t rccl_version;
    int32_t comm_sets;
    int32_t resident_volume;
    int32_t list_grown;
    double merge_ms;
    int64_t halo_bytes_subsample;
    double enqueue_ms;
} sift3d_zslab_stats;
#define SIFT3D_ZSLAB_TRANSPORT 1000
#define SIFT3D_TRANSPORT_PEER_COPY 0
#define SIFT3D_TRANSPORT_RCCL 1
#define SIFT3D_ZSLAB_SERIAL_CHANNELS 1001
#define SIFT3D_ZSLAB_DUPLICATE_RANKS 1002
#define SIFT3D_ZSLAB_POISON_HALO 1003
#define SIFT3D_ZSLAB_PATCH_WAIT 1004
#define SIFT3D_ZSLAB_LIST_ROOM 1005
void sift3d_zslab_set_transport_library(const char *path);
int sift3d_extract_zslab(const int *devices, int n_devices, const float *vol, int64_t nx, int64_t ny, int64_t nz,
                         float initial_image_scale, int desc_mode, float eig_thres, float size_factor, sift3d_feature **out,
                         int64_t *n_out, sift3d_zslab_stats *stats, char *err, int64_t err_len);
int sift3d_extract_zslab_over(int transport, const int *devices, int n_devices, const float *vol, int64_t nx, int64_t ny, int64_t nz,
                              float initial_image_scale, int desc_mode, float eig_thres, float size_factor, sift3d_feature **out,
                              int64_t *n_out, sift3d_zslab_stats *stats, char *err, int64_t err_len);
typedef struct sift3d_zslab sift3d_zslab;
sift3d_zslab *sift3d_zslab_create(const int *devices, int n_devices, int64_t nx, int64_t ny, int64_t nz, char *err, int64_t err_len);
int sift3d_zslab_extract(sift3d_zslab *h, const float *vol, float initial_image_scale, int desc_mode, float eig_thres,
                         float size_factor, sift3d_feature **out, int64_t *n_out, sift3d_zslab_stats *stats, char *err,
                         int64_t err_len);
void sift3d_zslab_destroy(sift3d_zslab *h);
int sift3d_zslab_set_volume(sift3d_zslab *h, const float *vol, char *err, int64_t err_len);
int sift3d_zslab_extract_resident(sift3d_zslab *h, float initial_image_scale, int desc_mode, float eig_thres, float size_factor,
                                  const sift3d_feature **view, int64_t *n_out, sift3d_zslab_stats *stats, char *err, int64_t err_len);
int sift3d_zslab_set_tuning(sift3d_zslab *h, int knob, int value);

int sift3d_knn64(int device, const int8_t *db, int64_t n_db, const int8_t *queries, int64_t n_q, int k, int32_t *idx,
                 int32_t *dist2, int repeats, double *kernel_ms, char *err, int64_t err_len);


int sift3d_match_ratio(int device, const sift3d_feature *db, int64_t n_db, const sift3d_feature *q, int64_t n_q, int32_t *i1, int32_t *d1,
                       int32_t *i2, int32_t *d2, double *kernel_ms, char *err, int64_t err_len);

int sift3d_hough_similarity(int device, const float *p0, const float *p1, const float *s0, const float *s1, const float *o0, const float *o1,
                            int32_t m, int32_t *counts, int32_t *winner, float *rot, float *scale, int32_t *flags, char *err,
                            int64_t err_len);

typedef struct {
    float scale;
    float rot[9];
    float trans[3];
    float center0[3];
    float center1[3];
    int32_t n_matches;
    int32_t inliers;
    int32_t winner;
    int32_t capacity;
    int32_t *moving_idx;
    int32_t *fixed_idx;
    int32_t *inlier;
    int32_t *dist2;
} sift3d_similarity;

int sift3d_match_keys(int device, const sift3d_feature *fixed, int64_t n_fixed, const sift3d_feature *moving, int64_t n_moving,
                      int32_t max_matches, sift3d_similarity *out, char *err, int64_t err_len);

int sift3d_log_ratio_interval(double t, float *lo, float *hi);
void sift3d_similarity_invert(const sift3d_similarity *in, sift3d_similarity *out);
int sift3d_write_similarity(const char *path, const sift3d_similarity *t);
int sift3d_write_alignment_matches(const char *base, const char *fixed_name, const char *moving_name, const sift3d_feature *fixed,
                                   int64_t n_fixed, const sift3d_feature *moving, int64_t n_moving, const sift3d_similarity *t);

int sift3d_guided_search(int device, const sift3d_feature *fixed, int64_t n_fixed, const sift3d_feature *moving, int64_t n_moving,
                         const sift3d_similarity *t, float radius, int32_t *i1, int32_t *d1, int32_t *i2, int32_t *d2, int32_t *visited,
                         double *kernel_ms, char *err, int64_t err_len);

int sift3d_fit_similarity(const float *p_moving, const float *p_fixed, int64_t n, sift3d_similarity *out);

typedef struct {
    int32_t max_rounds;
    float min_radius;
    float max_radius;
    int32_t ratio_num;
    int32_t ratio_den;
    float stop_shift;
    int64_t index_cells_max;
} sift3d_refine_params;
void sift3d_refine_defaults(sift3d_refine_params *p);
int sift3d_guided_search_params(int device, const sift3d_feature *fixed, int64_t n_fixed, const sift3d_feature *moving, int64_t n_moving,
                                const sift3d_similarity *t, float radius, const sift3d_refine_params *p, int32_t *i1, int32_t *d1, int32_t *i2,
                                int32_t *d2, int32_t *visited, double *kernel_ms, char *err, int64_t err_len);

#define SIFT3D_REFINE_MAX_ROUNDS 16
typedef enum {
    SIFT3D_REFINE_STOP_ROUNDS = 0,
    SIFT3D_REFINE_STOP_CONVERGED = 1,
    SIFT3D_REFINE_STOP_FIT = 2,
    SIFT3D_REFINE_STOP_NONE = 3
} sift3d_refine_stop;
typedef struct {
    float radius;
    int64_t visited;
    int32_t accepted;
    int32_t kept;
    double rms;
    double shift;
    double kernel_ms;
} sift3d_refine_round;
typedef struct {
    int32_t rounds;
    int32_t stop;
    sift3d_refine_round round[SIFT3D_REFINE_MAX_ROUNDS];
} sift3d_refine_report;

int sift3d_refine_similarity(int device, const sift3d_feature *fixed, int64_t n_fixed, const sift3d_feature *moving, int64_t n_moving,
                             const sift3d_similarity *init, const sift3d_refine_params *p, sift3d_similarity *out, sift3d_refine_report *rep,
                             char *err, int64_t err_len);

typedef enum { SIFT3D_INTERP_LINEAR = 0, SIFT3D_INTERP_NEAREST = 1 } sift3d_interp;
int sift3d_resample_affine(int device, const float *src, int64_t nx, int64_t ny, int64_t nz, float *dst, int64_t ox, int64_t oy,
                           int64_t oz, const float map[12], int interp, float fill, double *kernel_ms, char *err, int64_t err_len);
int sift3d_resample_affine_dev(sift3d_ctx *ctx, const float *d_src, int64_t nx, int64_t ny, int64_t nz, float *d_dst, int64_t ox,
                               int64_t oy, int64_t oz, const float map[12], int interp, float fill);
void sift3d_similarity_matrix(const sift3d_similarity *t, float m[16]);
int sift3d_read_similarity(const char *path, float m[16]);
int sift3d_resample_map(const float moving_to_fixed[16], const float fixed_vox2key[16], const float moving_vox2key[16], float map[12]);
void sift3d_key_vox2key(const float voxel[3], const float world[16], float m[16]);

typedef struct {
    int64_t n[3];
    float origin[3];
    float spacing;
    int64_t capacity;
    float *disp;
} sift3d_field;

typedef struct {
    float spacing;
    float radius;
    float lambda;
    float search_radius;
// ... 323 lines not shown
```

Before: 20.69 million keypoints/s.

## Sort candidate keys with index permutation and fuse scan, record map and group counts

The candidate radix sort now carries a 32-bit index permutation instead of the 16-byte value payload. The keypoint kernel gathers values through that permutation, and for single-chunk runs the sort is moved to a side stream so it overlaps keypoint work. The rocprim exclusive scan, the record-map kernel and the group-count kernel are replaced by one single-pass decoupled-lookback scanmap kernel that uses epoch-tagged tile state and a ticket counter. This cuts sort traffic and kernel launches, at the cost of a more intricate scan protocol and extra event synchronisation.

```diff
diff --git a/3d_sift_cuda_amd/__init__.py b/3d_sift_cuda_amd/__init__.py
--- a/3d_sift_cuda_amd/__init__.py
+++ b/3d_sift_cuda_amd/__init__.py
@@ -110,6 +110,8 @@
     _sig(L.sift3d_set_volume_dev, I, P, P, I64, I64, I64)
     _sig(L.sift3d_set_volume_resized, I, P, P, I64, I64, I64, I)
     _sig(L.sift3d_reserve, I, P, I64)
+    _sig(L.sift3d_record_map, I, P, P, P, P, I64, I, I, P, P, I64, P, P, P)
+    _sig(L.sift3d_candidate_order, I, P, P, I64, P)
     _sig(L.sift3d_set_volume_begin, I, P, I64, I64, I64, I)
     _sig(L.sift3d_set_volume_planes, I, P, P, I64, I64)
     _sig(L.sift3d_set_volume_end, I, P)
@@ -1611,6 +1613,26 @@
     def reserve(self, n_extrema):
         self._chk(self._L.sift3d_reserve(self._h, int(n_extrema)), "sift3d_reserve")
 
+    def record_map(self, nrec, perm, keys, first_record=0, cand_off=0, group_counts=False):
+        nrec = np.ascontiguousarray(nrec, np.int32)
+        perm = np.ascontiguousarray(perm, np.uint32)
+        keys = np.ascontiguousarray(keys, np.uint64)
+        n, cap = len(nrec), int(nrec.sum()) if len(nrec) else 0
+        rec_kp, rec_frame = np.full(cap, -7, np.int32), np.full(cap, -7, np.int32)
+        end, nkp = C.c_int32(0), C.c_int64(0)
+        counts = np.zeros(GROUPS, np.int32) if group_counts else None
+        self._chk(self._L.sift3d_record_map(self._h, nrec.ctypes.data, perm.ctypes.data, keys.ctypes.data, n, int(first_record), int(cand_off),
+                                            rec_kp.ctypes.data, rec_frame.ctypes.data, cap, C.byref(end), C.byref(nkp),
+                                            None if counts is None else counts.ctypes.data), "sift3d_record_map")
+        return rec_kp, rec_frame, end.value, nkp.value, counts
+
+    def candidate_order(self):
+        n = C.c_int64(0)
+        self._chk(self._L.sift3d_candidate_order(self._h, None, 0, C.byref(n)), "sift3d_candidate_order")
+        order = np.zeros(max(n.value, 1), np.uint32)
+        self._chk(self._L.sift3d_candidate_order(self._h, order.ctypes.data, len(order), C.byref(n)), "sift3d_candidate_order")
+        return order[:n.value]
+
     def set_volume_in_runs(self, vol, runs, resize=0):
         vol = _f32(vol)
         nz, ny, nx = vol.shape
diff --git a/3d_sift_cuda_amd/csrc/api_context.hip b/3d_sift_cuda_amd/csrc/api_context.hip
--- a/3d_sift_cuda_amd/csrc/api_context.hip
+++ b/3d_sift_cuda_amd/csrc/api_context.hip
@@ -48,6 +48,7 @@
     hipFree(c->keys_b);
     hipFree(c->vals_a);
     hipFree(c->vals_b);
+    hipFree(c->perm);
     hipFree(c->d_count);
     hipFree(c->surv);
     hipFree(c->surv2);
@@ -56,14 +57,14 @@
     hipFree(c->list2_counts);
     hipFree(c->surv_counts);
     hipFree(c->sort_tmp);
-    hipFree(c->scan_tmp);
+    hipFree(c->scan_state);
+    hipFree(c->scan_ticket);
     hipFree(c->d_levels);
     hipFree(c->kps);
     hipFree(c->patch0);
     hipFree(c->sampler_tokens);
     hipFree(c->d_rec_base);
     hipFree(c->nrec);
-    hipFree(c->offs);
     hipFree(c->rec_kp);
     hipFree(c->rec_frame);
     if (c->h_recs) hipHostFree(c->h_recs);
@@ -91,20 +92,23 @@
 {
     unsigned long long *ka = nullptr, *kb = nullptr;
     sift3d_cval *va = nullptr, *vb = nullptr;
+    unsigned *pm = nullptr;
     void *tmp = nullptr;
     const size_t tmp_bytes = sift3d_sort_temp_bytes(cap) + 256;
     const bool ok = hipMalloc((void **)&ka, sizeof(unsigned long long) * (size_t)cap) == hipSuccess &&
                     hipMalloc((void **)&kb, sizeof(unsigned long long) * (size_t)cap) == hipSuccess &&
                     hipMalloc((void **)&va, sizeof(sift3d_cval) * (size_t)cap) == hipSuccess &&
-                    hipMalloc((void **)&vb, sizeof(sift3d_cval) * (size_t)cap) == hipSuccess && hipMalloc(&tmp, tmp_bytes) == hipSuccess;
+                    hipMalloc((void **)&vb, sizeof(sift3d_cval) * (size_t)cap) == hipSuccess &&
+                    hipMalloc((void **)&pm, sizeof(unsigned) * (size_t)cap) == hipSuccess && hipMalloc(&tmp, tmp_bytes) == hipSuccess;
     if (!ok) {
         (void)hipGetLastError();
-        hipFree(ka); hipFree(kb); hipFree(va); hipFree(vb); hipFree(tmp);
+        hipFree(ka); hipFree(kb); hipFree(va); hipFree(vb); hipFree(pm); hipFree(tmp);
         return SIFT3D_ERR_MEMORY;
     }
-    hipFree(c->keys_a); hipFree(c->keys_b); hipFree(c->vals_a); hipFree(c->vals_b); hipFree(c->sort_tmp);
+    hipFree(c->keys_a); hipFree(c->keys_b); hipFree(c->vals_a); hipFree(c->vals_b); hipFree(c->perm); hipFree(c->sort_tmp);
     c->keys_a = ka; c->keys_b = kb;
     c->vals_a = va; c->vals_b = vb;
+    c->perm = pm;
     c->sort_tmp = tmp;
     c->sort_tmp_bytes = tmp_bytes;
     c->cand_cap = cap;
@@ -120,7 +124,7 @@
             hipStreamDestroy(st);
         }
     hipEvent_t events[] = {c->ev_ex2[0], c->ev_ex2[1], c->ev_reset, c->ev_desc, c->ev_oct[0], c->ev_oct[1], c->ev_fence[0], c->ev_fence[1],
-                           c->ev_split[0], c->ev_split[1], c->ev_split[2]};
+                           c->ev_split[0], c->ev_split[1], c->ev_split[2], c->ev_sort[0], c->ev_sort[1]};
     for (hipEvent_t e : events)
         if (e) hipEventDestroy(e);
     for (hipEvent_t e : c->ev_kpc)
@@ -155,7 +159,7 @@
     hipStream_t *streams[] = {&c->ex_stream, &c->ex_stream2, &c->kp_stream};
     for (hipStream_t *st : streams) ok = ok && hipStreamCreateWithFlags(st, hipStreamNonBlocking) == hipSuccess;
     hipEvent_t *events[] = {&c->ev_ex2[0], &c->ev_ex2[1], &c->ev_reset, &c->ev_desc, &c->ev_oct[0], &c->ev_oct[1], &c->ev_fence[0], &c->ev_fence[1],
-                            &c->ev_split[0], &c->ev_split[1], &c->ev_split[2]};
+                            &c->ev_split[0], &c->ev_split[1], &c->ev_split[2], &c->ev_sort[0], &c->ev_sort[1]};
     for (hipEvent_t *e : events) ok = ok && hipEventCreateWithFlags(e, hipEventDisableTiming) == hipSuccess;
     for (hipEvent_t &e : c->ev_kpc) ok = ok && hipEventCreateWithFlags(&e, hipEventDisableTiming) == hipSuccess;
     ok = ok && hipHostMalloc((void **)&c->h_cnt0, sizeof(unsigned long long) * (16 + SIFT3D_KP_MAX_CHUNKS), hipHostMallocDefault) == hipSuccess;
@@ -179,6 +183,8 @@
     ok = ok && hipMalloc((void **)&c->sampler_tokens, sizeof(int) * SIFT3D_CU_SLOTS) == hipSuccess &&
          hipMemsetAsync(c->sampler_tokens, 0, sizeof(int) * SIFT3D_CU_SLOTS, c->stream) == hipSuccess;
     ok = ok && hipMalloc((void **)&c->d_rec_base, sizeof(int) * (SIFT3D_KP_MAX_CHUNKS + 1)) == hipSuccess;
+    ok = ok && hipMalloc((void **)&c->scan_ticket, sizeof(unsigned)) == hipSuccess &&
+         hipMemsetAsync(c->scan_ticket, 0, sizeof(unsigned), c->stream) == hipSuccess;
     ok = ok && alloc_cands(c, c->capN / 32 + 8192) == SIFT3D_OK;
     c->surv_cap = c->capN / 8 + 65536;
     ok = ok && hipMalloc((void **)&c->surv, sizeof(sift3d_survivor) * (size_t)c->surv_cap) == hipSuccess;
diff --git a/3d_sift_cuda_amd/csrc/api_ops.hip b/3d_sift_cuda_amd/csrc/api_ops.hip
--- a/3d_sift_cuda_amd/csrc/api_ops.hip
+++ b/3d_sift_cuda_amd/csrc/api_ops.hip
@@ -416,12 +416,19 @@
             if (rc) return rc;
             continue;
         }
-        if (cnt[0] > 0)
-            HIPCHK(c, sift3d_sort_candidates(c->stream, c->sort_tmp, c->sort_tmp_bytes, c->keys_a, c->keys_b, c->vals_a, c->vals_b, (int64_t)cnt[0]));
         *count_out = (int64_t)cnt[0];
         return SIFT3D_OK;
     }
     return set_err(c, SIFT3D_ERR_MEMORY, "extrema buffers could not be grown");
+}
+
+int cand_sorted_values(sift3d_ctx *c, int64_t n)
+{
+    if (n <= 0) return SIFT3D_OK;
+    if (n > c->cand_cap) return set_err(c, SIFT3D_ERR_ARG, "cand_sorted_values: %lld entries asked of a list of %lld", (long long)n, (long long)c->cand_cap);
+    HIPCHK(c, sift3d_sort_candidates(c->stream, c->sort_tmp, c->sort_tmp_bytes, c->keys_a, c->keys_b, c->perm, n));
+    HIPCHK(c, sift3d_gather_values(c->stream, c->vals_a, c->perm, n, c->vals_b));
+    return SIFT3D_OK;
 }
 
 extern "C" int sift3d_extrema(sift3d_ctx *c, const float *d_prev, const float *d_cur, const float *d_next, int64_t nx,
@@ -444,6 +451,7 @@
     rc = cand_reset(c);
     if (!rc) rc = cand_append(c, {c->D[0], c->D[1], d_next ? c->D[2] : nullptr, nx, ny, nz, 0, (int)nz, 0}, cand_where(), true);
     if (!rc) rc = cand_finalize(c, &cnt);
+    if (!rc) rc = cand_sorted_values(c, cnt);
     if (rc) return rc;
     std::vector<unsigned long long> keys((size_t)cnt);
     std::vector<sift3d_cval> vals((size_t)cnt);
diff --git a/3d_sift_cuda_amd/csrc/api_pipeline.hip b/3d_sift_cuda_amd/csrc/api_pipeline.hip
--- a/3d_sift_cuda_amd/csrc/api_pipeline.hip
+++ b/3d_sift_cuda_amd/csrc/api_pipeline.hip
@@ -233,20 +233,21 @@
     if (ncand > c->kps_cap) {
         HIPCHK(c, hipStreamSynchronize(c->stream));
         HIPCHK(c, hipStreamSynchronize(c->kp_stream));
-        hipFree(c->kps); hipFree(c->nrec); hipFree(c->offs); hipFree(c->scan_tmp); hipFree(c->patch0);
+        hipFree(c->kps); hipFree(c->nrec); hipFree(c->scan_state); hipFree(c->patch0);
         hipFree(c->rec_kp); hipFree(c->rec_frame);
         c->kps = nullptr;
         c->patch0 = nullptr;
-        c->nrec = c->offs = c->rec_kp = c->rec_frame = nullptr;
-        c->scan_tmp = nullptr;
+        c->nrec = c->rec_kp = c->rec_frame = nullptr;
+        c->scan_state = nullptr;
         c->kps_cap = 0;
         const int64_t cap = ncand + ncand / 2 + 1024, rcap = cap * (1 + SIFT3D_MAX_FRAMES);
-        c->scan_tmp_bytes = sift3d_scan_temp_bytes(cap) + 256;
+        const size_t state_bytes = sizeof(unsigned long long) * (size_t)sift3d_scanmap_tiles(cap);
         HIPCHK(c, hipMalloc((void **)&c->kps, sizeof(sift3d_dkp) * (size_t)cap));
         HIPCHK(c, hipMalloc((void **)&c->patch0, sizeof(float) * SIFT3D_PATCH_VOX * (size_t)cap));
         HIPCHK(c, hipMalloc((void **)&c->nrec, sizeof(int) * (size_t)cap));
-        HIPCHK(c, hipMalloc((void **)&c->offs, sizeof(int) * (size_t)cap));
-        HIPCHK(c, hipMalloc(&c->scan_tmp, c->scan_tmp_bytes));
+        HIPCHK(c, hipMalloc((void **)&c->scan_state, state_bytes));
+        HIPCHK(c, hipMemsetAsync(c->scan_state, 0, state_bytes, c->stream));
+        HIPCHK(c, hipStreamSynchronize(c->stream));
         HIPCHK(c, hipMalloc((void **)&c->rec_kp, sizeof(int) * (size_t)rcap));
         HIPCHK(c, hipMalloc((void **)&c->rec_frame, sizeof(int) * (size_t)rcap));
         c->kps_cap = cap;
@@ -280,6 +281,8 @@
     std::vector<unsigned long long> keys((size_t)ncand);
     std::vector<sift3d_cval> vals((size_t)ncand);
     if (ncand) {
+        const int rc = cand_sorted_values(c, ncand);
+        if (rc) return rc;
         HIPCHK(c, hipMemcpyAsync(keys.data(), c->keys_b, sizeof(unsigned long long) * (size_t)ncand, hipMemcpyDeviceToHost, c->stream));
         HIPCHK(c, hipMemcpyAsync(vals.data(), c->vals_b, sizeof(sift3d_cval) * (size_t)ncand, hipMemcpyDeviceToHost, c->stream));
     }
@@ -387,28 +390,50 @@
     return SIFT3D_OK;
 }
 
-static int describe_queue_chunk(sift3d_ctx *c, int i, int64_t a, int64_t b, hipStream_t ks, const float *taps3)
+static int describe_sort(sift3d_ctx *c, hipStream_t ss, int64_t list, int64_t at, int64_t n)
+{
+    HIPCHK(c, sift3d_sort_candidates(ss, c->sort_tmp, c->sort_tmp_bytes, c->keys_a + list, c->keys_b + at, c->perm + at, n));
+    return SIFT3D_OK;
+}
+
+static hipStream_t sort_stream_for(const sift3d_ctx *c, hipStream_t ks) { return (c->timing == 1 || c->timing == 3) ? ks : c->ex_stream; }
+
+static int describe_queue_chunk(sift3d_ctx *c, int i, int64_t a, int64_t b, hipStream_t ks, const float *taps3, int64_t list, int64_t at,
+                                hipStream_t ss)
 {
     int *h_end = reinterpret_cast<int *>(c->h_cnt0 + 8);
     c->kp.first[i] = a;
     c->kp.first[i + 1] = b;
     h_end[i] = 0;
+    if (ss) {
+        int rc = describe_sort(c, ss, list, at, b - a);
+        if (rc) return rc;
+        if (ss != ks) HIPCHK(c, hipEventRecord(c->ev_sort[1], ss));
+    }
     {
         sift3d_kp_params q = c->kp.p;
-        q.patch0 = c->patch0 + (size_t)a * SIFT3D_PATCH_VOX;
+        q.patch0 = c->patch0 + (size_t)at * SIFT3D_PATCH_VOX;
         stage_scope sc(c, SIFT3D_STAGE_KEYPOINT, 0.0, 0, b - a, ks);
-        HIPCHK(c, sift3d_launch_keypointsA(ks, q, c->keys_b + a, c->vals_b + a, b - a, c->kps + a, c->nrec + a, taps3));
-    }
-    HIPCHK(c, sift3d_scan_counts(ks, c->scan_tmp, c->scan_tmp_bytes, c->nrec + a, c->offs + a, b - a));
-    HIPCHK(c, sift3d_launch_recmap(ks, c->nrec + a, c->offs + a, b - a, (int)a, c->d_rec_base + i, c->rec_kp, c->rec_frame, c->d_count + 3));
-    HIPCHK(c, hipMemcpyAsync(&h_end[i], c->d_rec_base + i + 1, sizeof(int), hipMemcpyDeviceToHost, ks));
+        HIPCHK(c, sift3d_launch_keypointsA(ks, q, c->keys_a + list, c->vals_a + list, ss ? nullptr : c->perm + a, b - a, c->kps + at,
+                                           c->nrec + at, taps3));
+    }
+    if (ss && ss != ks) HIPCHK(c, hipStreamWaitEvent(ks, c->ev_sort[1], 0));
+    int *group_counts = nullptr;
     if (c->place.counts && i == 0) {
         int rc = ensure_place_buffers(c);
         if (rc) return rc;
         HIPCHK(c, hipMemsetAsync(c->place.d_counts, 0, sizeof(int) * SIFT3D_GROUPS, ks));
-        HIPCHK(c, sift3d_launch_group_counts(ks, c->keys_b + a, c->nrec + a, b - a, c->place.d_counts));
+        group_counts = c->place.d_counts;
+    }
+    if (c->scan_epoch >= SIFT3D_SCANMAP_EPOCHS) {
+        HIPCHK(c, hipMemsetAsync(c->scan_state, 0, sizeof(unsigned long long) * (size_t)sift3d_scanmap_tiles(c->kps_cap), ks));
+        c->scan_epoch = 0;
+    }
+    HIPCHK(c, sift3d_launch_scanmap(ks, c->nrec + at, c->perm + a, c->keys_b + a, b - a, (int)at, c->d_rec_base + i, c->rec_kp, c->rec_frame,
+                                    c->d_count + 3, group_counts, c->scan_state, c->scan_ticket, ++c->scan_epoch));
+    HIPCHK(c, hipMemcpyAsync(&h_end[i], c->d_rec_base + i + 1, sizeof(int), hipMemcpyDeviceToHost, ks));
+    if (group_counts)
         HIPCHK(c, hipMemcpyAsync(c->place.h_counts, c->place.d_counts, sizeof(int) * SIFT3D_GROUPS, hipMemcpyDeviceToHost, ks));
-    }
     HIPCHK(c, hipEventRecord(c->ev_kpc[i], ks));
     return SIFT3D_OK;
 }
@@ -428,12 +453,91 @@
     kp_params_of(c, desc_mode, eig_thres, size_factor, c->kp.p);
     const int nch = kp_chunks_for(c, ncand);
     c->kp.nchunks = nch;
+    hipStream_t ss = nullptr;
+    if (nch == 1) {
+        ss = sort_stream_for(c, c->stream);
+        if (ss != c->stream) {
+            HIPCHK(c, hipEventRecord(c->ev_sort[0], c->stream));
+            HIPCHK(c, hipStreamWaitEvent(ss, c->ev_sort[0], 0));
+        }
+    } else {
+        rc = describe_sort(c, c->stream, 0, 0, ncand);
+        if (rc) return rc;
+    }
     HIPCHK(c, hipMemsetAsync(c->d_count + 3, 0, sizeof(unsigned long long), c->stream));
     HIPCHK(c, hipMemsetAsync(c->d_rec_base, 0, sizeof(int), c->stream));
     for (int i = 0; i < nch; i++) {
-        rc = describe_queue_chunk(c, i, ncand * i / nch, ncand * (i + 1) / nch, c->stream, taps3);
-        if (rc) return rc;
-    }
+        rc = describe_queue_chunk(c, i, ncand * i / nch, ncand * (i + 1) / nch, c->stream, taps3, 0, 0, ss);
+        if (rc) return rc;
+    }
+    return SIFT3D_OK;
+}
+
+extern "C" int sift3d_record_map(sift3d_ctx *c, const int32_t *nrec, const uint32_t *perm, const uint64_t *keys, int64_t n, int32_t first_record,
+                                 int32_t cand_off, int32_t *rec_kp, int32_t *rec_frame, int64_t rec_cap, int32_t *end_record,
+                                 int64_t *n_keypoints, int32_t *group_counts)
+{
+    if (!c || !nrec || !perm || !keys || n <= 0 || n > INT32_MAX || first_record < 0 || !rec_kp || !rec_frame || !end_record || !n_keypoints)
+        return set_err(c, SIFT3D_ERR_ARG, "sift3d_record_map: bad arguments");
+    int64_t total = 0;
+    std::vector<bool> seen((size_t)n, false);
+    for (int64_t i = 0; i < n; i++) {
+        if (perm[i] >= (uint64_t)n || seen[perm[i]]) return set_err(c, SIFT3D_ERR_ARG, "sift3d_record_map: perm is not a permutation of 0 .. n - 1");
+        seen[perm[i]] = true;
+        if (nrec[i] < 0 || nrec[i] > 1 + SIFT3D_MAX_FRAMES) return set_err(c, SIFT3D_ERR_ARG, "sift3d_record_map: a count outside 0 .. %d", 1 + SIFT3D_MAX_FRAMES);
+        total += nrec[i];
+    }
+    if (total > rec_cap) return set_err(c, SIFT3D_ERR_CAPACITY, "sift3d_record_map: %lld records, room for %lld", (long long)total, (long long)rec_cap);
+    HIPCHK(c, hipSetDevice(c->device));
+    HIPCHK(c, hipStreamSynchronize(c->stream));
+    if (n > c->cand_cap && alloc_cands(c, n + n / 4 + 4096) != SIFT3D_OK)
+        return set_err(c, SIFT3D_ERR_MEMORY, "candidate buffer could not be grown to %lld entries", (long long)n);
+    int rc = ensure_kp_buffers(c, n, 0);
+    if (rc) return rc;
+    if (group_counts) {
+        rc = ensure_place_buffers(c);
+        if (rc) return rc;
+        HIPCHK(c, hipMemsetAsync(c->place.d_counts, 0, sizeof(int) * SIFT3D_GROUPS, c->stream));
+    }
+    if (first_record + total > c->recs_cap) return set_err(c, SIFT3D_ERR_CAPACITY, "sift3d_record_map: first record %d leaves no room for %lld", first_record, (long long)total);
+    HIPCHK(c, hipMemcpyAsync(c->nrec, nrec, sizeof(int) * (size_t)n, hipMemcpyHostToDevice, c->stream));
+    HIPCHK(c, hipMemcpyAsync(c->perm, perm, sizeof(unsigned) * (size_t)n, hipMemcpyHostToDevice, c->stream));
+    HIPCHK(c, hipMemcpyAsync(c->keys_b, keys, sizeof(unsigned long long) * (size_t)n, hipMemcpyHostToDevice, c->stream));
+    HIPCHK(c, hipMemcpyAsync(c->d_rec_base, &first_record, sizeof(int), hipMemcpyHostToDevice, c->stream));
+    HIPCHK(c, hipMemsetAsync(c->d_count + 3, 0, sizeof(unsigned long long), c->stream));
+    if (c->scan_epoch >= SIFT3D_SCANMAP_EPOCHS) {
+        HIPCHK(c, hipMemsetAsync(c->scan_state, 0, sizeof(unsigned long long) * (size_t)sift3d_scanmap_tiles(c->kps_cap), c->stream));
+        c->scan_epoch = 0;
+    }
+    HIPCHK(c, sift3d_launch_scanmap(c->stream, c->nrec, c->perm, c->keys_b, n, cand_off, c->d_rec_base, c->rec_kp, c->rec_frame, c->d_count + 3,
+                                    group_counts ? c->place.d_counts : nullptr, c->scan_state, c->scan_ticket, ++c->scan_epoch));
+    unsigned long long nkp = 0;
+    HIPCHK(c, hipMemcpyAsync(end_record, c->d_rec_base + 1, sizeof(int), hipMemcpyDeviceToHost, c->stream));
+    HIPCHK(c, hipMemcpyAsync(&nkp, c->d_count + 3, sizeof(nkp), hipMemcpyDeviceToHost, c->stream));
+    if (total > 0) {
+        HIPCHK(c, hipMemcpyAsync(rec_kp, c->rec_kp + first_record, sizeof(int) * (size_t)total, hipMemcpyDeviceToHost, c->stream));
+        HIPCHK(c, hipMemcpyAsync(rec_frame, c->rec_frame + first_record, sizeof(int) * (size_t)total, hipMemcpyDeviceToHost, c->stream));
+    }
+    if (group_counts)
+        HIPCHK(c, hipMemcpyAsync(group_counts, c->place.d_counts, sizeof(int) * SIFT3D_GROUPS, hipMemcpyDeviceToHost, c->stream));
+    HIPCHK(c, hipStreamSynchronize(c->stream));
+    *n_keypoints = (int64_t)nkp;
+    return SIFT3D_OK;
+}
+
+extern "C" int sift3d_candidate_order(sift3d_ctx *c, uint32_t *order, int64_t cap, int64_t *n_out)
+{
+    if (!c || !n_out || (cap > 0 && !order)) return set_err(c, SIFT3D_ERR_ARG, "sift3d_candidate_order: bad arguments");
+    const int64_t n = c->kp.ncand;
+    *n_out = n;
+    if (n <= 0 || !order) return SIFT3D_OK;
+    if (cap < n) return set_err(c, SIFT3D_ERR_CAPACITY, "sift3d_candidate_order: %lld entries", (long long)n);
+    HIPCHK(c, hipSetDevice(c->device));
+    HIPCHK(c, hipMemcpyAsync(order, c->perm, sizeof(unsigned) * (size_t)n, hipMemcpyDeviceToHost, c->stream));
+    HIPCHK(c, hipStreamSynchronize(c->stream));
+    if (c->kp.split)
+        for (int i = 1; i < c->kp.nchunks; i++)
+            for (int64_t j = c->kp.first[i]; j < c->kp.first[i + 1]; j++) order[j] += (uint32_t)c->kp.first[i];
     return SIFT3D_OK;
 }
 
@@ -500,7 +604,7 @@
 #ifdef SIFT3D_DEV
 extern "C" int sift3d_dev_overlap_probe(sift3d_ctx *c, int kslice, int dslice, double *out_ms)
 {
-    if (!c || !out_ms || kslice < 1 || dslice < 1 || c->kp.ncand <= 0 || c->kp.nrec <= 0) return SIFT3D_ERR_ARG;
+    if (!c || !out_ms || kslice < 1 || dslice < 1 || c->kp.ncand <= 0 || c->kp.nrec <= 0 || c->kp.split) return SIFT3D_ERR_ARG;
     HIPCHK(c, hipSetDevice(c->device));
     float taps3[SIFT3D_MAX_TAPS];
     sift3d_gauss_taps(0.5f, 0.01f, taps3);
@@ -513,7 +617,7 @@
     auto launch_k = [&](hipStream_t st, int64_t a, int64_t n) -> hipError_t {
         sift3d_kp_params q = c->kp.p;
         q.patch0 = c->patch0 + (size_t)a * SIFT3D_PATCH_VOX;
-        return sift3d_launch_keypointsA(st, q, c->keys_b + a, c->vals_b + a, n, c->kps + a, c->nrec + a, taps3);
+        return sift3d_launch_keypointsA(st, q, c->keys_a + a, c->vals_a + a, nullptr, n, c->kps + a, c->nrec + a, taps3);
     };
     auto launch_d = [&](hipStream_t st, int64_t b, int64_t m) -> hipError_t {
         return sift3d_launch_descriptors(st, c->kp.p, c->kps, c->rec_kp + b, c->rec_frame + b, m, c->d_hrecs + b, c->d_hgroup + b, c->kp.taps5);
@@ -587,15 +691,50 @@
     return rc;
 }
 
+struct split_first {
+    bool ok = false;
+    unsigned long long mark = 0;
+    int64_t nA = 0;
+    int nch = 0;
+    float taps3[SIFT3D_MAX_TAPS];
+};
+static int split_tail_first(sift3d_ctx *c, const std::vector<sift3d_level> &levels, bool levels_on_device, int desc_mode, float eig_thres,
+                            float size_factor, split_first &f)
+{
+    const unsigned long long *const h_split = c->h_cnt0 + 8 + SIFT3D_KP_MAX_CHUNKS;
+    hipStream_t ks = c->kp_stream;
+    f.nA = (int64_t)h_split[0];
+    f.mark = h_split[2];
+    if (h_split[2] > 0 || f.nA > c->cand_split_at) return SIFT3D_OK;
+    int rc = describe_begin(c, levels.size(), f.taps3);
+    if (rc) return rc;
+    rc = ensure_kp_buffers(c, f.nA + f.nA / 8 + 4096, f.nA);
+    if (rc) return rc;
+    kp_params_of(c, desc_mode, eig_thres, size_factor, c->kp.p);
+    c->kp.split = true;
+    if (!levels_on_device)
+        HIPCHK(c, hipMemcpyAsync(c->d_levels, levels.data(), sizeof(sift3d_level) * levels.size(), hipMemcpyHostToDevice, ks));
+    hipStream_t ss = sort_stream_for(c, ks);
+    if (f.nA > 0) {
+        if (ss != ks) HIPCHK(c, hipStreamWaitEvent(ss, c->ev_split[2], 0));
+        rc = describe_queue_chunk(c, f.nch++, 0, f.nA, ks, f.taps3, 0, 0, ss);
+        if (rc) return rc;
+    }
+    c->kp.nchunks = f.nch;
+    f.ok = true;
+    return SIFT3D_OK;
+}
+
 static int finish_split_tail(sift3d_ctx *c, const std::vector<sift3d_level> &levels, bool levels_on_device, int desc_mode, float eig_thres,
                              float size_factor, int64_t *n_out, bool *done)
 {
     *done = false;
+    split_first f;
     unsigned long long *const h_split = c->h_cnt0 + 8 + SIFT3D_KP_MAX_CHUNKS;
     const int64_t capA = c->cand_split_at, capB = c->cand_cap - capA;
     hipStream_t ks = c->kp_stream;
-    float taps3[SIFT3D_MAX_TAPS];
     auto fall_back = [&](unsigned long long overflow_mark) -> int {
+        HIPCHK(c, hipStreamSynchronize(c->ex_stream));
         HIPCHK(c, hipStreamSynchronize(ks));
         HIPCHK(c, hipStreamSynchronize(c->stream));
         if (overflow_mark > 0) {
@@ -607,29 +746,19 @@
     h_split[3] = h_split[5] = h_split[7] = 0;
     HIPCHK(c, hipMemcpyAsync(h_split + 3, c->d_count, sizeof(unsigned long long) * 5, hipMemcpyDeviceToHost, c->stream));
     HIPCHK(c, hipEventSynchronize(c->ev_split[2]));
-    const int64_t nA = (int64_t)h_split[0];
-    if (h_split[2] > 0 || nA > capA) return fall_back(h_split[2]);
-    int rc = describe_begin(c, levels.size(), taps3);
-    if (rc) return rc;
-    rc = ensure_kp_buffers(c, nA + nA / 8 + 4096, nA);
-    if (rc) return rc;
-    kp_params_of(c, desc_mode, eig_thres, size_factor, c->kp.p);
-    c->kp.split = true;
-    if (!levels_on_device)
-        HIPCHK(c, hipMemcpyAsync(c->d_levels, levels.data(), sizeof(sift3d_level) * levels.size(), hipMemcpyHostToDevice, ks));
-    int nch = 0;
-    if (nA > 0) {
-        HIPCHK(c, sift3d_sort_candidates(ks, c->sort_tmp, c->sort_tmp_bytes, c->keys_a, c->keys_b, c->vals_a, c->vals_b, nA));
-        rc = describe_queue_chunk(c, nch++, 0, nA, ks, taps3);
-        if (rc) return rc;
-    }
+    int rc = split_tail_first(c, levels, levels_on_device, desc_mode, eig_thres, size_factor, f);
+    if (rc) return rc;
+    if (!f.ok) return fall_back(f.mark);
+    const int64_t nA = f.nA;
+    const float *taps3 = f.taps3;
+    hipStream_t ss = sort_stream_for(c, ks);
+    int nch = f.nch;
     c->kp.nchunks = nch;
     HIPCHK(c, hipStreamSynchronize(c->stream));
     const int64_t nB = (int64_t)h_split[7];
     if (h_split[5] > 0 || nB > capB || nA + nB > c->kps_cap || (int64_t)h_split[3] != nA) return fall_back(h_split[5]);
     if (nB > 0) {
-        HIPCHK(c, sift3d_sort_candidates(ks, c->sort_tmp, c->sort_tmp_bytes, c->keys_a + capA, c->keys_b + nA, c->vals_a + capA, c->vals_b + nA, nB));
-        rc = describe_queue_chunk(c, nch++, nA, nA + nB, ks, taps3);
+        rc = describe_queue_chunk(c, nch++, nA, nA + nB, ks, taps3, capA, nA, ss);
         if (rc) return rc;
     }
     c->kp.nchunks = nch;
diff --git a/3d_sift_cuda_amd/csrc/kernels_keypoint.hip b/3d_sift_cuda_amd/csrc/kernels_keypoint.hip
--- a/3d_sift_cuda_amd/csrc/kernels_keypoint.hip
+++ b/3d_sift_cuda_amd/csrc/kernels_keypoint.hip
@@ -640,13 +640,13 @@
               "the splat parameters span A and C");
 
 __global__ __launch_bounds__(KP_NT, 7) void keypoint_kernel(sift3d_kp_params p, const unsigned long long *__restrict__ keys,
-                                                      const sift3d_cval *__restrict__ vals, long long ncand,
-                                                      sift3d_dkp *__restrict__ kps, int *__restrict__ nrec_out,
+                                                      const sift3d_cval *__restrict__ vals, const unsigned *__restrict__ pick,
+                                                      long long ncand, sift3d_dkp *__restrict__ kps, int *__restrict__ nrec_out,
                                                       sift3d_taps taps3)
 {
     __shared__ __attribute__((aligned(16))) kpA_smem sm;
-    const long long k = blockIdx.x;
-    if (k >= ncand) return;
+    if (blockIdx.x >= ncand) return;
+    const long long k = pick ? (long long)pick[blockIdx.x] : (long long)blockIdx.x;
     const int lane = threadIdx.x;
     if (lane < 3) sm.taps[lane] = taps3.f[lane];
     const unsigned long long key = keys[k];
@@ -1106,54 +1106,135 @@
     }
 }
 
-__global__ void group_count_kernel(const unsigned long long *__restrict__ keys, const int *__restrict__ nrec, long long ncand, int *__restrict__ counts)
-{
-    const long long k = (long long)blockIdx.x * blockDim.x + threadIdx.x;
-    if (k >= ncand) return;
-    const int n = nrec[k];
-    if (n <= 0) return;
-    int g = (int)(keys[k] >> SIFT3D_KEY_LVL_SHIFT) * 2 + (int)((keys[k] >> SIFT3D_KEY_MAX_SHIFT) & 1ull);
-    if (g < 0 || g >= SIFT3D_GROUPS - 1) g = SIFT3D_GROUPS - 1;
-    atomicAdd(counts + g, n);
-}
-
-hipError_t sift3d_launch_group_counts(hipStream_t s, const unsigned long long *keys, const int *nrec, int64_t ncand, int *counts)
-{
-    if (ncand <= 0) return hipSuccess;
-    hipLaunchKernelGGL(group_count_kernel, dim3((unsigned)((ncand + 255) / 256)), dim3(256), 0, s, keys, nrec, (long long)ncand, counts);
-    return hipGetLastError();
-}
-
-__global__ void recmap_kernel(const int *__restrict__ nrec, const int *__restrict__ offs, long long ncand, int cand_off,
-                              int *rec_base, int *__restrict__ rec_kp, int *__restrict__ rec_frame, unsigned long long *kp_count)
-{
-    const long long k = (long long)blockIdx.x * blockDim.x + threadIdx.x;
-    if (k >= ncand) return;
-    const int n = nrec[k], o = rec_base[0] + offs[k];
-    if (k == ncand - 1) rec_base[1] = o + n;
-    if (n > 0) atomicAdd(kp_count, 1ull);
-    for (int f = 0; f < n; f++) {
-        rec_kp[o + f] = cand_off + (int)k;
-        rec_frame[o + f] = f - 1;
+#define SCANMAP_NT 256
+#define SCANMAP_ITEMS 2
+#define SCANMAP_TILE (SCANMAP_NT * SCANMAP_ITEMS)
+#define SCANMAP_SPINS (1 << 20)
+#define SCANMAP_AGG 1ull
+#define SCANMAP_PREFIX 2ull
+
+__global__ __launch_bounds__(SCANMAP_NT) void scanmap_kernel(const int *__restrict__ nrec, const unsigned *__restrict__ perm,
+                                                             const unsigned long long *__restrict__ keys, long long ncand, int cand_off,
+                                                             int *rec_base, int *__restrict__ rec_kp, int *__restrict__ rec_frame,
+                                                             unsigned long long *kp_count, int *group_counts,
+                                                             unsigned long long *state, unsigned *ticket, unsigned epoch)
+{
+    __shared__ unsigned s_tile;
+    __shared__ int s_wave[SCANMAP_NT / 64];
+    __shared__ int s_base;
+    const int tid = threadIdx.x, lane = tid & 63, wave = tid >> 6;
+    if (tid == 0) {
+        s_tile = atomicAdd(ticket, 1u);
+        if (s_tile == gridDim.x - 1) __hip_atomic_store(ticket, 0u, __ATOMIC_RELAXED, __HIP_MEMORY_SCOPE_AGENT);
+    }
+    __syncthreads();
+    const long long tile = s_tile;
+    const unsigned long long tag = (unsigned long long)epoch << 34;
+
+    int n[SCANMAP_ITEMS], src[SCANMAP_ITEMS];
+    int mine = 0, kept = 0;
+    for (int j = 0; j < SCANMAP_ITEMS; j++) {
+        const long long i = tile * SCANMAP_TILE + (long long)tid * SCANMAP_ITEMS + j;
+        n[j] = 0;
+        src[j] = 0;
+        if (i < ncand) {
+            src[j] = (int)perm[i];
+            const int v = nrec[src[j]];
+            n[j] = v < 0 ? 0 : (v > 1 + SIFT3D_MAX_FRAMES ? 1 + SIFT3D_MAX_FRAMES : v);
+        }
+        mine += n[j];
+        kept += n[j] > 0;
+    }
+    int incl = mine;
+    for (int d = 1; d < 64; d <<= 1) {
+        const int up = __shfl_up(incl, d, 64);
+        if (lane >= d) incl += up;
+    }
+    if (lane == 63) s_wave[wave] = incl;
+    for (int d = 32; d > 0; d >>= 1) kept += __shfl_xor(kept, d, 64);
+    if (lane == 0 && kept > 0) atomicAdd(kp_count, (unsigned long long)kept);
+    __syncthreads();
+    int before = 0, total = 0;
+    for (int w = 0; w < SCANMAP_NT / 64; w++) {
+        if (w < wave) before += s_wave[w];
+        total += s_wave[w];
+    }
+    if (wave == 0) {
+        long long sum = 0;
+        bool ok = true;
+        if (lane == 0)
+            __hip_atomic_store(state + tile, tag | ((tile == 0 ? SCANMAP_PREFIX : SCANMAP_AGG) << 32) | (unsigned)total, __ATOMIC_RELAXED,
+                               __HIP_MEMORY_SCOPE_AGENT);
+        for (long long hi = tile - 1; hi >= 0 && ok; hi -= 64) {
+            const long long t = hi - lane;
+            unsigned long long v = tag | (SCANMAP_PREFIX << 32);
+            int spins = 0;
+            for (;;) {
+                if (t >= 0) v = __hip_atomic_load(state + t, __ATOMIC_RELAXED, __HIP_MEMORY_SCOPE_AGENT);
+                const bool there = (v >> 34) == epoch && ((v >> 32) & 3ull) != 0;
+                if (__all(there)) break;
+                if (++spins >= SCANMAP_SPINS) {
+                    ok = false;
+                    break;
+                }
+                __builtin_amdgcn_s_sleep(2);
+            }
+            if (!ok) break;
+            const unsigned long long known = __ballot(((v >> 32) & 3ull) == SCANMAP_PREFIX);
+            const int stop = known ? __ffsll((long long)known) - 1 : 63;
+            long long part = lane <= stop ? (long long)(unsigned)v : 0;
+            for (int d = 32; d > 0; d >>= 1) part += __shfl_xor(part, d, 64);
+            sum += part;
+            if (known) break;
+        }
+        if (lane == 0) {
+            if (ok && tile > 0)
+                __hip_atomic_store(state + tile, tag | (SCANMAP_PREFIX << 32) | (unsigned)(sum + total), __ATOMIC_RELAXED, __HIP_MEMORY_SCOPE_AGENT);
+            if (!ok) atomicExch(rec_base + 1, -1);
+            s_base = ok ? (int)sum : -1;
+        }
+    }
+    __syncthreads();
+    if (s_base < 0) return;
+    int o = rec_base[0] + s_base + before + incl - mine;
+    for (int j = 0; j < SCANMAP_ITEMS; j++) {
+        const long long i = tile * SCANMAP_TILE + (long long)tid * SCANMAP_ITEMS + j;
+        if (i >= ncand) break;
+        for (int f = 0; f < n[j]; f++) {
+            rec_kp[o + f] = cand_off + src[j];
+            rec_frame[o + f] = f - 1;
+        }
+        if (group_counts && n[j] > 0) {
+            int g = (int)(keys[i] >> SIFT3D_KEY_LVL_SHIFT) * 2 + (int)((keys[i] >> SIFT3D_KEY_MAX_SHIFT) & 1ull);
+            if (g < 0 || g >= SIFT3D_GROUPS - 1) g = SIFT3D_GROUPS - 1;
+            atomicAdd(group_counts + g, n[j]);
+        }
+        o += n[j];
+        if (i == ncand - 1) rec_base[1] = o;
     }
 }
 
 hipError_t sift3d_launch_keypointsA(hipStream_t s, const sift3d_kp_params &p, const unsigned long long *keys,
-                                    const sift3d_cval *vals, int64_t ncand, sift3d_dkp *kps, int *nrec, const float *taps3)
+                                    const sift3d_cval *vals, const unsigned *pick, int64_t ncand, sift3d_dkp *kps, int *nrec,
+                                    const float *taps3)
 {
     if (ncand <= 0) return hipSuccess;
     sift3d_taps t;
     for (int i = 0; i < 17; i++) t.f[i] = i < 3 ? taps3[i] : 0.0f;
-    hipLaunchKernelGGL(keypoint_kernel, dim3((unsigned)ncand), dim3(KP_NT), 0, s, p, keys, vals, (long long)ncand, kps, nrec, t);
+    hipLaunchKernelGGL(keypoint_kernel, dim3((unsigned)ncand), dim3(KP_NT), 0, s, p, keys, vals, pick, (long long)ncand, kps, nrec, t);
     return hipGetLastError();
 }
 
-hipError_t sift3d_launch_recmap(hipStream_t s, const int *nrec, const int *offs, int64_t ncand, int cand_off, int *rec_base,
-                                int *rec_kp, int *rec_frame, unsigned long long *kp_count)
+int64_t sift3d_scanmap_tiles(int64_t ncand) { return ncand > 0 ? (ncand + SCANMAP_TILE - 1) / SCANMAP_TILE : 0; }
+
+hipError_t sift3d_launch_scanmap(hipStream_t s, const int *nrec, const unsigned *perm, const unsigned long long *keys, int64_t ncand,
+                                 int cand_off, int *rec_base, int *rec_kp, int *rec_frame, unsigned long long *kp_count,
+                                 int *group_counts, unsigned long long *state, unsigned *ticket, unsigned epoch)
 {
     if (ncand <= 0) return hipSuccess;
-    hipLaunchKernelGGL(recmap_kernel, dim3((unsigned)((ncand + 255) / 256)), dim3(256), 0, s, nrec, offs, (long long)ncand,
-                       cand_off, rec_base, rec_kp, rec_frame, kp_count);
+    if (epoch < 1 || epoch > SIFT3D_SCANMAP_EPOCHS) return hipErrorInvalidValue;
+    hipLaunchKernelGGL(scanmap_kernel, dim3((unsigned)sift3d_scanmap_tiles(ncand)), dim3(SCANMAP_NT), 0, s, nrec, perm, keys,
+                       (long long)ncand, cand_off, rec_base, rec_kp, rec_frame, kp_count, group_counts, state, ticket, epoch);
     return hipGetLastError();
 }
 
diff --git a/3d_sift_cuda_amd/csrc/pipeline.h b/3d_sift_cuda_amd/csrc/pipeline.h
--- a/3d_sift_cuda_amd/csrc/pipeline.h
+++ b/3d_sift_cuda_amd/csrc/pipeline.h
@@ -124,7 +124,9 @@
     float *d_taps;
     unsigned long long *keys_a, *keys_b;
     sift3d_cval *vals_a, *vals_b;
+    unsigned *perm;
     int64_t cand_cap;
+    hipEvent_t ev_sort[2];
     unsigned long long *d_count;
     int64_t cand_split_at;
     sift3d_survivor *surv;
@@ -137,14 +139,15 @@
     int surv_div;
     void *sort_tmp;
     size_t sort_tmp_bytes;
-    void *scan_tmp;
-    size_t scan_tmp_bytes;
+    unsigned long long *scan_state;
+    unsigned *scan_ticket;
+    unsigned scan_epoch;
     sift3d_level *d_levels;
     sift3d_dkp *kps;
     float *patch0;
     int *sampler_tokens;
     int *d_rec_base;
-    int *nrec, *offs;
+    int *nrec;
     int64_t kps_cap;
     int *rec_kp, *rec_frame;
     int64_t recs_cap;
@@ -241,6 +244,7 @@
                              const cand_where &w);
 int cand_count_queue(sift3d_ctx *c);
 int cand_finalize(sift3d_ctx *c, int64_t *count_out);
+int cand_sorted_values(sift3d_ctx *c, int64_t n);
 int describe_queue(sift3d_ctx *c, const std::vector<sift3d_level> &levels, int64_t ncand, int desc_mode, float eig_thres, float size_factor,
                    bool levels_on_device);
 void describe_want_group_counts(sift3d_ctx *c, bool on);
diff --git a/3d_sift_cuda_amd/csrc/sift3d_internal.h b/3d_sift_cuda_amd/csrc/sift3d_internal.h
--- a/3d_sift_cuda_amd/csrc/sift3d_internal.h
+++ b/3d_sift_cuda_amd/csrc/sift3d_internal.h
@@ -141,7 +141,6 @@
     int desc_seg;
     const int *rec_shift;
 };
-hipError_t sift3d_launch_group_counts(hipStream_t s, const unsigned long long *keys, const int *nrec, int64_t ncand, int *counts);
 #define SIFT3D_CU_SLOTS 2048
 #define SIFT3D_MAX_FRAMES 11
 struct sift3d_dkp {
@@ -154,17 +153,20 @@
     unsigned info;
 };
 hipError_t sift3d_launch_keypointsA(hipStream_t s, const sift3d_kp_params &p, const unsigned long long *keys,
-                                    const sift3d_cval *vals, int64_t ncand, sift3d_dkp *kps, int *nrec, const float *taps3);
-hipError_t sift3d_launch_recmap(hipStream_t s, const int *nrec, const int *offs, int64_t ncand, int cand_off, int *rec_base,
-                                int *rec_kp, int *rec_frame, unsigned long long *kp_count);
+                                    const sift3d_cval *vals, const unsigned *pick, int64_t ncand, sift3d_dkp *kps, int *nrec,
+                                    const float *taps3);
+#define SIFT3D_SCANMAP_EPOCHS 0x3fffffffu
+int64_t sift3d_scanmap_tiles(int64_t ncand);
+hipError_t sift3d_launch_scanmap(hipStream_t s, const int *nrec, const unsigned *perm, const unsigned long long *keys, int64_t ncand,
+                                 int cand_off, int *rec_base, int *rec_kp, int *rec_frame, unsigned long long *kp_count,
+                                 int *group_counts, unsigned long long *state, unsigned *ticket, unsigned epoch);
 hipError_t sift3d_launch_descriptors(hipStream_t s, const sift3d_kp_params &p, const sift3d_dkp *kps, const int *rec_kp,
                                      const int *rec_frame, int64_t nrec, sift3d_feature *recs, int *rec_group,
                                      const float *taps5);
 size_t sift3d_sort_temp_bytes(int64_t n);
 hipError_t sift3d_sort_candidates(hipStream_t s, void *temp, size_t temp_bytes, const unsigned long long *keys_in,
-                                  unsigned long long *keys_out, const sift3d_cval *vals_in, sift3d_cval *vals_out, int64_t n);
-size_t sift3d_scan_temp_bytes(int64_t n);
-hipError_t sift3d_scan_counts(hipStream_t s, void *temp, size_t temp_bytes, const int *in, int *out, int64_t n);
+                                  unsigned long long *keys_out, unsigned *perm, int64_t n);
+hipError_t sift3d_gather_values(hipStream_t s, const sift3d_cval *vals_in, const unsigned *perm, int64_t n, sift3d_cval *vals_out);
 
 hipError_t sift3d_launch_knn_norms(hipStream_t s, const signed char *v, int64_t n, int *norms, unsigned long long *stats);
 hipError_t sift3d_launch_knn(hipStream_t s, const signed char *db, const int *db_norm, int64_t n_db, const signed char *q, const int *q_norm,
diff --git a/3d_sift_cuda_amd/csrc/sort_scan.hip b/3d_sift_cuda_amd/csrc/sort_scan.hip
--- a/3d_sift_cuda_amd/csrc/sort_scan.hip
+++ b/3d_sift_cuda_amd/csrc/sort_scan.hip
@@ -10,28 +10,29 @@
 {
     size_t bytes = 0;
     (void)rocprim::radix_sort_pairs(nullptr, bytes, (const unsigned long long *)nullptr, (unsigned long long *)nullptr,
-                                    (const float4 *)nullptr, (float4 *)nullptr, (size_t)n, 0, SORT_END_BIT, (hipStream_t)0);
+                                    rocprim::counting_iterator<unsigned>(0u), (unsigned *)nullptr, (size_t)n, 0, SORT_END_BIT, (hipStream_t)0);
     return bytes;
 }
 
 hipError_t sift3d_sort_candidates(hipStream_t s, void *temp, size_t temp_bytes, const unsigned long long *keys_in,
-                                  unsigned long long *keys_out, const sift3d_cval *vals_in, sift3d_cval *vals_out, int64_t n)
+                                  unsigned long long *keys_out, unsigned *perm, int64_t n)
 {
     if (n <= 0) return hipSuccess;
-    return rocprim::radix_sort_pairs(temp, temp_bytes, keys_in, keys_out, (const float4 *)vals_in, (float4 *)vals_out,
-                                     (size_t)n, 0, SORT_END_BIT, s);
+    return rocprim::radix_sort_pairs(temp, temp_bytes, keys_in, keys_out, rocprim::counting_iterator<unsigned>(0u), perm, (size_t)n, 0,
+                                     SORT_END_BIT, s);
 }
 
-size_t sift3d_scan_temp_bytes(int64_t n)
+__global__ void gather_values_kernel(const sift3d_cval *__restrict__ vals_in, const unsigned *__restrict__ perm, long long n,
+                                     sift3d_cval *__restrict__ vals_out)
 {
-    size_t bytes = 0;
-    (void)rocprim::exclusive_scan(nullptr, bytes, (const int *)nullptr, (int *)nullptr, 0, (size_t)n, rocprim::plus<int>(),
-                                  (hipStream_t)0);
-    return bytes;
+    const long long i = (long long)blockIdx.x * blockDim.x + threadIdx.x;
+    if (i >= n) return;
+    reinterpret_cast<float4 *>(vals_out)[i] = reinterpret_cast<const float4 *>(vals_in)[perm[i]];
 }
 
-hipError_t sift3d_scan_counts(hipStream_t s, void *temp, size_t temp_bytes, const int *in, int *out, int64_t n)
+hipError_t sift3d_gather_values(hipStream_t s, const sift3d_cval *vals_in, const unsigned *perm, int64_t n, sift3d_cval *vals_out)
 {
     if (n <= 0) return hipSuccess;
-    return rocprim::exclusive_scan(temp, temp_bytes, in, out, 0, (size_t)n, rocprim::plus<int>(), s);
+    hipLaunchKernelGGL(gather_values_kernel, dim3((unsigned)((n + 255) / 256)), dim3(256), 0, s, vals_in, perm, (long long)n, vals_out);
+    return hipGetLastError();
 }
diff --git a/include/sift3d.h b/include/sift3d.h
--- a/include/sift3d.h
+++ b/include/sift3d.h
@@ -145,6 +145,11 @@
                                float size_factor, const int32_t **group_counts, int64_t *n_records);
 int sift3d_describe_dev_place(sift3d_ctx *ctx, sift3d_feature *list, const int32_t *shift, const sift3d_feature **own_view,
                               const int32_t **group_view, int64_t *n_out);
+
+int sift3d_record_map(sift3d_ctx *ctx, const int32_t *nrec, const uint32_t *perm, const uint64_t *keys, int64_t n, int32_t first_record,
+                      int32_t cand_off, int32_t *rec_kp, int32_t *rec_frame, int64_t rec_cap, int32_t *end_record,
+                      int64_t *n_keypoints, int32_t *group_counts);
+int sift3d_candidate_order(sift3d_ctx *ctx, uint32_t *order, int64_t cap, int64_t *n);
 int sift3d_host_register(void *p, int64_t bytes);
 int sift3d_host_unregister(void *p);
 
```

Result: no change. 20.66 million keypoints/s (-0.1%).
